# MicroYY/VoxelHashing

Hardware: AMD Instinct MI355X
Metric: depth frames/sec integrate+raycast @640x480, 4 cm voxel; HBM GB/s vs peak (higher is better)
Workload: dtype f32

## Files before the change

### include/vh_api.h

```cpp
#ifndef VH_API_H
#define VH_API_H

#include "vh_types.h"

#ifdef __cplusplus
extern "C" {
#endif

typedef void* vhStream_t;

const char* vh_version(void);
const char* vh_error_string(int code);
const char* vh_last_error_message(void);

int vh_malloc(void** devPtr, size_t bytes);
int vh_free(void* devPtr);
int vh_malloc_host(void** hostPtr, size_t bytes);
int vh_free_host(void* hostPtr);
int vh_memcpy_h2d(void* dst, const void* src, size_t bytes, vhStream_t stream);
int vh_memcpy_d2h(void* dst, const void* src, size_t bytes, vhStream_t stream);
int vh_memset(void* dst, int value, size_t bytes, vhStream_t stream);
int vh_time_next_launch(void* startEvent, void* stopEvent);
int vh_stream_create(vhStream_t* out);
int vh_stream_destroy(vhStream_t stream);
int vh_stream_synchronize(vhStream_t stream);
int vh_device_synchronize(void);

int vh_hash_data_alloc(VhHashData* hd, const VhHashParams* hp);
int vh_hash_data_free(VhHashData* hd);

int vh_reset(const VhHashData* hd, const VhHashParams* hp, vhStream_t stream);
int vh_reset_bucket_mutex(const VhHashData* hd, const VhHashParams* hp, vhStream_t stream);
int vh_alloc(const VhHashData* hd, const VhHashParams* hp, const VhDepthCameraData* cam,
             const VhDepthCameraParams* cp, const uint32_t* d_bitMask, int32_t lockToken, vhStream_t stream);
enum { VH_COMPACT_COUNTER_IS_ZERO = 1 };
int vh_compactify(const VhHashData* hd, const VhHashParams* hp, const VhDepthCameraParams* cp,
                  uint32_t* numOccupied, uint32_t flags, vhStream_t stream);
int vh_integrate(const VhHashData* hd, const VhHashParams* hp, const VhDepthCameraData* cam,
                 const VhDepthCameraParams* cp, vhStream_t stream);
int vh_starve(const VhHashData* hd, const VhHashParams* hp, vhStream_t stream);
int vh_gc_identify(const VhHashData* hd, const VhHashParams* hp, const VhDepthCameraParams* cp, vhStream_t stream);
int vh_gc_free(const VhHashData* hd, const VhHashParams* hp, int32_t lockToken, vhStream_t stream);
int vh_bind_input_depth_color_textures(const VhDepthCameraData* cam);

enum { VH_FUSED_GC = 1, VH_FUSED_STARVE = 2 };
int vh_integrate_fused(const VhHashData* hd, const VhHashParams* hp, const VhDepthCameraData* cam,
                       const VhDepthCameraParams* cp, uint32_t flags, int32_t lockToken, uint32_t* d_countMirror,
                       uint32_t mirrorTag, const void* d_packedFrame, vhStream_t stream);
int vh_alloc_job(VhFrameJob* job, vhStream_t stream);
int vh_compactify_job(VhFrameJob* job, vhStream_t stream);

int vh_render(const VhHashData* hd, const VhHashParams* hp, const VhRayCastData* rd,
              const VhDepthCameraParams* cp, const VhRayCastParams* rp, vhStream_t stream);
int vh_ray_interval_clear(uint32_t* d_tileHeads, uint32_t width, uint32_t height, vhStream_t stream);
int vh_ray_interval_splat(const VhHashData* hd, const VhHashParams* hp, const VhDepthCameraParams* cp, const VhRayCastParams* rp,
                          uint32_t* d_tileHeads, VhTileBlock* d_tileBlocks, uint32_t tileCapacity, uint32_t* d_schedule, uint32_t phase,
                          uint32_t* d_longestList, vhStream_t stream);
size_t vh_render_schedule_bytes(uint32_t width, uint32_t height);
uint32_t vh_render_split_tiles(uint32_t width, uint32_t height);
int vh_render_intervals(const VhHashData* hd, const VhHashParams* hp, const VhRayCastData* rd, const VhDepthCameraParams* cp,
                        const VhRayCastParams* rp, uint32_t* d_tileHeads, const VhTileBlock* d_tileBlocks, uint32_t tileCapacity,
                        uint32_t* d_schedule, uint32_t phase, vhStream_t stream);
int vh_compute_normals(float* d_output4, const float* d_input4, uint32_t width, uint32_t height, vhStream_t stream);
int vh_render_intervals_co(const VhHashData* hd, const VhHashParams* hp, const VhRayCastData* rd, const VhDepthCameraParams* cp,
                           const VhRayCastParams* rp, uint32_t* d_tileHeads, const VhTileBlock* d_tileBlocks, uint32_t tileCapacity,
                           uint32_t* d_schedule, uint32_t phase, VhFrameJob* job, vhStream_t stream);
int vh_compute_normals_co(float* d_output4, const float* d_input4, uint32_t width, uint32_t height, VhFrameJob* job, vhStream_t stream);
int vh_compute_normals_co2(float* d_output4, const float* d_input4, uint32_t width, uint32_t height, VhFrameJob* job,
                           const VhRayCastParams* nextView, uint32_t* d_tileHeads, VhTileBlock* d_tileBlocks, uint32_t tileCapacity,
                           uint32_t* d_schedule, uint32_t phase, uint32_t* d_longestList, vhStream_t stream);

int vh_publish_words(const uint32_t* d_src0, const uint32_t* d_src1, uint32_t* d_mapped, uint32_t tag, vhStream_t stream);

int vh_stream_out_pass1(const VhHashData* hd, const VhHashParams* hp, uint32_t threadsPerPart, uint32_t start,
                        float radius, const float camPos[3], uint32_t* d_outputCounter, VhSDFBlockDesc* d_output,
                        uint32_t outputCapacity, int32_t lockToken, vhStream_t stream);
int vh_stream_out_probe(const VhHashData* hd, const VhHashParams* hp, uint32_t threadsPerPart, uint32_t start, float radius,
                        const float camPos[3], uint32_t* d_counter, uint32_t* d_mapped, uint32_t tag, vhStream_t stream);
int vh_stream_out_pass2(const VhHashData* hd, const VhHashParams* hp, const VhSDFBlockDesc* d_descs,
                        VhVoxel* d_output, uint32_t nSDFBlocks, vhStream_t stream);
int vh_stream_out_device(const VhHashData* hd, const VhHashParams* hp, uint32_t threadsPerPart, uint32_t start, float radius,
                         const float camPos[3], uint32_t* d_outputCounter, VhSDFBlockDesc* d_descs, VhVoxel* d_blocks,
                         uint32_t mostBlocks, int32_t lockToken, uint32_t* d_bitMask, vhStream_t stream);
int vh_publish_count(const uint32_t* d_counter, uint32_t* d_mapped, uint32_t tag, vhStream_t stream);
int vh_stream_in_device(const VhHashData* hd, const VhHashParams* hp, uint32_t n, const VhSDFBlockDesc* d_descs, const VhVoxel* d_blocks,
                        int32_t lockToken, uint32_t* d_failed, uint32_t* d_bitMask, uint32_t chunkBit, uint32_t* d_mapped, uint32_t tag,
                        vhStream_t stream);
int vh_stream_in_pass1(const VhHashData* hd, const VhHashParams* hp, uint32_t n, uint32_t heapCountPrev,
                       const VhSDFBlockDesc* d_descs, int32_t lockToken, vhStream_t stream);
int vh_stream_in_pass1_report(const VhHashData* hd, const VhHashParams* hp, uint32_t n, uint32_t heapCountPrev,
                              const VhSDFBlockDesc* d_descs, int32_t lockToken, uint32_t* d_failed, vhStream_t stream);
int vh_stream_in_pass2(const VhHashData* hd, const VhHashParams* hp, uint32_t n, uint32_t heapCountPrev,
                       const VhSDFBlockDesc* d_descs, const VhVoxel* d_blocks, vhStream_t stream);

int vh_synth_frame(const double* h_spheres, int nSpheres, int inside, const float camToWorld[16],
                   const VhDepthCameraParams* cp, float* d_depth, float* d_color4, vhStream_t stream);
enum { VH_OP_ALLOC = 0, VH_OP_DELETE = 1, VH_OP_INSERT = 2, VH_OP_LOOKUP = 3, VH_OP_NEW_PASS = 4 };
int vh_debug_hash_ops(const VhHashData* hd, const VhHashParams* hp, const int32_t* d_ops, int32_t* d_results,
                      uint32_t n, vhStream_t stream);

int vh_debug_check_fast_math(float divisor, uint32_t modulus, uint32_t n, uint32_t seed, uint32_t* d_mismatches, vhStream_t stream);

int vh_debug_check_refined_division(uint32_t n, uint32_t seed, uint32_t* d_mismatches, vhStream_t stream);
int vh_debug_valu_probe(uint32_t mode, uint32_t wavesPerSimd, uint32_t iters, uint32_t* d_stamps, uint32_t* numWaves, vhStream_t stream);

typedef struct VhSceneRep VhSceneRep;
typedef struct VhRayCast VhRayCast;
typedef struct VhChunkGrid VhChunkGrid;

int vh_scene_rep_create(const VhHashParams* hp, const VhSceneOptions* opt, vhStream_t stream, VhSceneRep** out);
void vh_scene_rep_destroy(VhSceneRep* s);
int vh_scene_rep_integrate(VhSceneRep* s, const float rigidTransform[16], const VhDepthCameraData* cam,
                           const VhDepthCameraParams* cp, const uint32_t* d_bitMask);
int vh_scene_rep_set_last_rigid_transform_and_compactify(VhSceneRep* s, const float rigidTransform[16],
                                                         const VhDepthCameraParams* cp);
int vh_scene_rep_reset(VhSceneRep* s);
int vh_scene_rep_get_hash_data(VhSceneRep* s, VhHashData* out);
int vh_scene_rep_get_hash_params(VhSceneRep* s, VhHashParams* out);
int vh_scene_rep_get_heap_free_count(VhSceneRep* s, uint32_t* out);
int vh_scene_rep_get_num_occupied_blocks(VhSceneRep* s, uint32_t* out);
int vh_scene_rep_debug_hash(VhSceneRep* s, uint32_t report[4]);
int vh_scene_rep_get_state(VhSceneRep* s, uint32_t* out);
int vh_scene_rep_get_timings(VhSceneRep* s, double out[4]);
int vh_scene_rep_set_options(VhSceneRep* s, const VhSceneOptions* opt);

int vh_scene_rep_integrate_ahead(VhSceneRep* s, const float rigidTransform[16], const VhDepthCameraData* cam,
                                 const VhDepthCameraParams* cp, const uint32_t* d_bitMask, VhFrameJob** job);
int vh_scene_rep_integrate_finish(VhSceneRep* s, const VhDepthCameraData* cam, const VhDepthCameraParams* cp);

int vh_raycast_create(const VhRayCastParams* rp, vhStream_t stream, VhRayCast** out);
void vh_raycast_destroy(VhRayCast* r);
int vh_raycast_render(VhRayCast* r, const VhHashData* hd, const VhHashParams* hp,
                      const VhDepthCameraParams* cp, const float lastRigidTransform[16]);
int vh_raycast_render_co(VhRayCast* r, const VhHashData* hd, const VhHashParams* hp,
                         const VhDepthCameraParams* cp, const float lastRigidTransform[16], VhFrameJob* job);
int vh_raycast_get_data(VhRayCast* r, VhRayCastData* out);
int vh_raycast_get_params(VhRayCast* r, VhRayCastParams* out);
int vh_raycast_get_timings(VhRayCast* r, double out[4]);
int vh_raycast_get_event_pair_overhead(VhRayCast* r, double* ms);
int vh_raycast_set_timing(VhRayCast* r, int enabled);
int vh_raycast_set_timing_stride(VhRayCast* r, int enabled, uint32_t stride);
int vh_raycast_set_interval_splatting(VhRayCast* r, int enabled);

int vh_chunk_grid_create(VhSceneRep* s, const float voxelExtents[3], const int32_t gridDimensions[3],
                         const int32_t minGridPos[3], uint32_t initialChunkListSize, int streamingEnabled,
                         uint32_t streamOutParts, VhChunkGrid** out);
void vh_chunk_grid_destroy(VhChunkGrid* g);
int vh_chunk_grid_stream_out_to_cpu_pass0_gpu(VhChunkGrid* g, const float posCamera[3], float radius, int useParts, int multiThreaded);
int vh_chunk_grid_stream_out_to_cpu_pass1_cpu(VhChunkGrid* g, int multiThreaded);
int vh_chunk_grid_stream_in_to_gpu_pass0_cpu(VhChunkGrid* g, const float posCamera[3], float radius, int useParts, int multiThreaded);
int vh_chunk_grid_stream_in_to_gpu_pass1_gpu(VhChunkGrid* g, int multiThreaded);
int vh_chunk_grid_stream_out_to_cpu(VhChunkGrid* g, const float posCamera[3], float radius, int useParts, uint32_t* nStreamedBlocks);
int vh_chunk_grid_stream_in_to_gpu(VhChunkGrid* g, const float posCamera[3], float radius, int useParts, uint32_t* nStreamedBlocks);
int vh_chunk_grid_stream_out_to_cpu_all(VhChunkGrid* g);
int vh_chunk_grid_stream_in_to_gpu_all(VhChunkGrid* g, const float posCamera[3], float radius, int useParts, uint32_t* nStreamedBlocks);
int vh_chunk_grid_get_bit_mask_gpu(VhChunkGrid* g, const uint32_t** d_bitMask);
int vh_chunk_grid_reset(VhChunkGrid* g);
int vh_chunk_grid_debug_check_for_duplicates(VhChunkGrid* g);
int vh_chunk_grid_get_statistics(VhChunkGrid* g, uint32_t out[3]);
int vh_chunk_grid_get_num_failed_inserts(VhChunkGrid* g, uint32_t* out);
int vh_chunk_grid_download_host_blocks(VhChunkGrid* g, VhSDFBlockDesc* descs, VhVoxel* blocks, uint32_t capacity, uint32_t* n);
int vh_chunk_grid_save_to_file(VhChunkGrid* g, const char* filename, const float camPos[3], float radius);
int vh_chunk_grid_load_from_file(VhChunkGrid* g, const char* filename, const float camPos[3], float radius);

typedef struct VhReconstruction VhReconstruction;
void vh_reconstruction_default_options(VhReconstructionOptions* out);
int vh_reconstruction_create(VhSceneRep* scene, VhRayCast* rayCast, VhChunkGrid* chunkGrid ,
                             const VhDepthCameraParams* cp, const VhReconstructionOptions* opt, VhReconstruction** out);
void vh_reconstruction_destroy(VhReconstruction* r);
int vh_reconstruction_run(VhReconstruction* r, const VhSequenceFrame* frames, uint32_t n);
int vh_reconstruction_run_ahead(VhReconstruction* r, const VhSequenceFrame* frames, uint32_t n, const VhSequenceFrame* next);
int vh_reconstruction_synchronize(VhReconstruction* r);
int vh_reconstruction_get_stats(VhReconstruction* r, VhReconstructionStats* out);
int vh_reconstruction_debug_fail_render(VhReconstruction* r, uint32_t nthRenderFromNow);
int vh_reconstruction_reset(VhReconstruction* r);

int vh_convert_color_raw_to_float4(float* d_output4, const uint8_t* d_inputRGBX, uint32_t width, uint32_t height, vhStream_t stream);
int vh_upload_frame(const float* hostDepth, const uint8_t* hostRGBX, float* d_depth, float* d_color4, uint32_t width, uint32_t height, vhStream_t stream);
int vh_resample_float_map(float* d_output, uint32_t outputWidth, uint32_t outputHeight, const float* d_input,
                          uint32_t inputWidth, uint32_t inputHeight, vhStream_t stream);
int vh_resample_float4_map(float* d_output4, uint32_t outputWidth, uint32_t outputHeight, const float* d_input4,
                           uint32_t inputWidth, uint32_t inputHeight, vhStream_t stream);
// ... 157 lines not shown
```

### include/vh_types.h

```cpp
#ifndef VH_TYPES_H
#define VH_TYPES_H

#include <stdint.h>

#ifdef __cplusplus
extern "C" {
#endif

#define VH_SDF_BLOCK_SIZE 8
#define VH_SDF_BLOCK_VOXELS 512
#define VH_HASH_BUCKET_SIZE 10
#define VH_LOCK_ENTRY (-1)
#define VH_FREE_ENTRY (-2)
#define VH_NO_OFFSET 0

typedef struct VhHashEntry {
    int32_t pos[3];
    int32_t ptr;
    uint32_t offset;
    uint32_t _pad[3];
} VhHashEntry;

typedef struct VhVoxel {
    float sdf;
    uint8_t color[3];
    uint8_t weight;
} VhVoxel;

typedef struct VhHashParams {
    float m_rigidTransform[16];
    float m_rigidTransformInverse[16];

    uint32_t m_hashNumBuckets;
    uint32_t m_hashBucketSize;
    uint32_t m_hashMaxCollisionLinkedListSize;
    uint32_t m_numSDFBlocks;

    int32_t m_SDFBlockSize;
    float m_virtualVoxelSize;
    uint32_t m_numOccupiedBlocks;

    float m_maxIntegrationDistance;
    float m_truncScale;
    float m_truncation;
    uint32_t m_integrationWeightSample;
    uint32_t m_integrationWeightMax;

    float m_streamingVoxelExtents[3];
    int32_t m_streamingGridDimensions[3];
    int32_t m_streamingMinGridPos[3];
    uint32_t m_streamingInitialChunkListSize;
    uint32_t m_dummy[2];
} VhHashParams;

typedef struct VhDepthCameraParams {
    float fx, fy, mx, my;
    uint32_t m_imageWidth;
    uint32_t m_imageHeight;
    float m_sensorDepthWorldMin;
    float m_sensorDepthWorldMax;
} VhDepthCameraParams;

typedef struct VhRayCastParams {
    float m_viewMatrix[16];
    float m_viewMatrixInverse[16];
    float m_intrinsics[16];
    float m_intrinsicsInverse[16];

    uint32_t m_width;
    uint32_t m_height;

    uint32_t m_numOccupiedSDFBlocks;
    uint32_t m_maxNumVertices;
    int32_t m_splatMinimum;

    float m_minDepth;
    float m_maxDepth;
    float m_rayIncrement;
    float m_thresSampleDist;
    float m_thresDist;
    uint8_t m_useGradients;
    uint8_t _pad0[3];

    uint32_t dummy0;
} VhRayCastParams;

typedef struct VhHashData {
    uint32_t* d_heap;
    uint32_t* d_heapCounter;
    int32_t* d_hashDecision;
    int32_t* d_hashDecisionPrefix;
    VhHashEntry* d_hash;
    VhHashEntry* d_hashCompactified;
    int32_t* d_hashCompactifiedCounter;
    VhVoxel* d_SDFBlocks;
    int32_t* d_hashBucketMutex;
    uint8_t m_bIsOnGPU;
    uint8_t _pad0[7];
    uint32_t* d_bucketCount;
    uint32_t* d_bucketBits;
    uint32_t* d_state;
} VhHashData;

enum {
    VH_STATE_HEAP_UNDERFLOW = 0,
    VH_STATE_INSERT_FAILED = 1,
    VH_STATE_ALLOC_LOCK_LOST = 2,
    VH_STATE_RIDER_GAVE_UP = 3,
    VH_STATE_WORDS = 16
};

typedef struct VhDepthCameraData {
    const float* d_depthData;
    const float* d_colorData;
} VhDepthCameraData;

typedef struct VhRayCastData {
    float* d_depth;
    float* d_depth4;
    float* d_normals;
    float* d_colors;
} VhRayCastData;

#define VH_TILE_LIST_CAPACITY 64
#define VH_TILE_LIST_CAPACITY_LARGE 128
typedef struct VhTileBlock {
    int32_t pos[3];
    int32_t ptr;
} VhTileBlock;

typedef struct VhSDFBlockDesc {
    int32_t pos[3];
    int32_t ptr;
} VhSDFBlockDesc;

typedef struct VhMarchingCubesParams {
    uint32_t m_boxEnabled;
    float m_minCorner[3];
    uint32_t m_maxNumTriangles;
    float m_maxCorner[3];
    uint32_t m_sdfBlockSize;
    uint32_t m_hashNumBuckets;
    uint32_t m_hashBucketSize;
    float m_threshMarchingCubes;
    float m_threshMarchingCubes2;
    float dummy[3];
} VhMarchingCubesParams;

typedef struct VhVertex {
    float p[3];
    float c[3];
} VhVertex;
typedef struct VhTriangle {
    VhVertex v0, v1, v2;
} VhTriangle;

typedef struct VhMarchingCubesData {
    VhMarchingCubesParams* d_params;
    uint32_t* d_numOccupiedBlocks;
    uint32_t* d_occupiedBlocks;
    uint32_t* d_numTriangles;
    VhTriangle* d_triangles;
    uint8_t m_bIsOnGPU;
} VhMarchingCubesData;

typedef struct VhSceneOptions {
    uint8_t s_offlineProcessing;
    uint8_t s_garbageCollectionEnabled;
    uint8_t s_timingsDetailledEnabled;
    uint8_t s_useReferenceLaunchSequence;
    uint32_t s_garbageCollectionStarve;
    uint32_t s_streamingOutParts;
} VhSceneOptions;

typedef struct VhFrameJob {
    VhHashData hashData;
    VhHashParams hashParams;
    VhDepthCameraData cam;
    VhDepthCameraParams cp;
    const uint32_t* d_bitMask;
    void* d_packedFrame;
    int32_t lockToken;
    uint8_t allocLaunched, compactifyLaunched, pad0[2];
    uint32_t frameNumber;
    uint32_t tableEpoch;
// ... 191 lines not shown
```

### voxelhashing_amd/csrc/vh_device.hpp

```cpp
#pragma once

#include <hip/hip_runtime.h>
#include <stdint.h>

#include "../../include/vh_types.h"

namespace vhd {

struct F3 { float x, y, z; };
struct I3 { int x, y, z; };

#define VHD __device__ __forceinline__

VHD float minf() { return __int_as_float((int)0xff800000u); }
VHD float pinf() { return __int_as_float((int)0x7f800000u); }

VHD F3 mk3(float x, float y, float z) { F3 r; r.x = x; r.y = y; r.z = z; return r; }
VHD I3 mki3(int x, int y, int z) { I3 r; r.x = x; r.y = y; r.z = z; return r; }
VHD float dot3(F3 a, F3 b) { return a.x * b.x + a.y * b.y + a.z * b.z; }

VHD int f2i(float v) { return __float2int_rz(v); }
VHD uint8_t f2uc(float v) { return (uint8_t)__float2int_rz(fminf(fmaxf(v, 0.0f), 255.0f)); }

VHD int signi(float v) { return (0.0f < v) - (v < 0.0f); }
// ... 82 lines not shown
{
    const uint32_t q0 = __umulhi(k.m, n);
    const uint32_t t = ((n - q0) >> 1) + q0;
    const uint32_t q = t >> k.sh;
    return n - q * k.d;
}
VHD uint32_t hash_pos_fast(HashMod k, I3 p)
{
    const uint32_t p0 = 73856093u, p1 = 19349669u, p2 = 83492791u;
    return umod_fast(((uint32_t)p.x * p0) ^ ((uint32_t)p.y * p1) ^ ((uint32_t)p.z * p2), k);
}


VHD F3 depth_to_skeleton(const VhDepthCameraParams& cp, uint32_t ux, uint32_t uy, float depth)
{
    const float x = ((float)ux - cp.mx) / cp.fx;
    const float y = ((float)uy - cp.my) / cp.fy;
    return mk3(depth * x, depth * y, depth);
}
VHD float cam_to_proj_z(const VhDepthCameraParams& cp, float z)
{
    return (z - cp.m_sensorDepthWorldMin) / (cp.m_sensorDepthWorldMax - cp.m_sensorDepthWorldMin);
}
VHD float proj_to_cam_z(const VhDepthCameraParams& cp, float z)
{
    return z * (cp.m_sensorDepthWorldMax - cp.m_sensorDepthWorldMin) + cp.m_sensorDepthWorldMin;
}
VHD bool in_frustum_approx(const VhDepthCameraParams& cp, const float* viewMatrixInverse, F3 pos)
{
    F3 pc = mat_mul_p(viewMatrixInverse, pos);
    float px = pc.x * cp.fx / pc.z + cp.mx;
    float py = pc.y * cp.fy / pc.z + cp.my;
    float wm1 = (float)cp.m_imageWidth - 1.0f, hm1 = (float)cp.m_imageHeight - 1.0f;
    float x = (2.0f * px - wm1) / wm1;
    float y = (hm1 - 2.0f * py) / hm1;
    float z = cam_to_proj_z(cp, pc.z);
    const float s = 0.95f;
    x *= s; y *= s; z *= s;
    return !(x < -1.0f || x > 1.0f || y < -1.0f || y > 1.0f || z < 0.0f || z > 1.0f);
}
VHD bool block_in_frustum(const VhHashParams& hp, const VhDepthCameraParams& cp, I3 blk)
{
    F3 pw = block_to_world(hp.m_virtualVoxelSize, blk);
    float off = hp.m_virtualVoxelSize * 0.5f * ((float)VH_SDF_BLOCK_SIZE - 1.0f);
    pw.x += off; pw.y += off; pw.z += off;
    return in_frustum_approx(cp, hp.m_rigidTransformInverse, pw);
}


VHD int4 load_quad(const VhHashEntry* e) { return *reinterpret_cast<const int4*>(e); }
VHD void store_quad(VhHashEntry* e, int4 q) { *reinterpret_cast<int4*>(e) = q; }
VHD bool quad_matches(int4 q, I3 p) { return q.x == p.x && q.y == p.y && q.z == p.z && q.w != VH_FREE_ENTRY; }

VHD void delete_hash_entry(VhHashEntry* e)
{
    e->offset = 0;
    store_quad(e, make_int4(0, 0, 0, VH_FREE_ENTRY));
}
VHD void copy_entry(VhHashEntry* dst, const VhHashEntry* src)
{
    int4 q = load_quad(src);
    uint32_t o = src->offset;
    dst->offset = o;
    store_quad(dst, q);
}

VHD void bucket_inc(const VhHashData& hd, uint32_t slotIdx)
{
    uint32_t b = slotIdx / VH_HASH_BUCKET_SIZE;
    uint32_t old = atomicAdd(&hd.d_bucketCount[b], 1u);
    if (old == 0u) atomicOr(&hd.d_bucketBits[b >> 5], 1u << (b & 31));
}
VHD void bucket_dec(const VhHashData& hd, uint32_t slotIdx)
{
    uint32_t b = slotIdx / VH_HASH_BUCKET_SIZE;
    uint32_t old = atomicSub(&hd.d_bucketCount[b], 1u);
    if (old == 1u) atomicAnd(&hd.d_bucketBits[b >> 5], ~(1u << (b & 31)));
}
VHD bool bucket_maybe_occupied(const VhHashData& hd, uint32_t h)
{
    return (hd.d_bucketBits[h >> 5] >> (h & 31)) & 1u;
}

VHD uint32_t consume_heap(const VhHashData& hd, uint32_t numSDFBlocks, bool& ok)
{
    uint32_t addr = atomicSub(&hd.d_heapCounter[0], 1u);
    if (addr >= numSDFBlocks) {
        atomicAdd(&hd.d_heapCounter[0], 1u);
        atomicAdd(&hd.d_state[VH_STATE_HEAP_UNDERFLOW], 1u);
        ok = false;
        return 0;
    }
    ok = true;
    return hd.d_heap[addr];
}
VHD void append_heap(const VhHashData& hd, uint32_t blockId)
{
    uint32_t addr = atomicAdd(&hd.d_heapCounter[0], 1u);
    hd.d_heap[addr + 1] = blockId;
}

VHD int lookup_ptr(const VhHashData& hd, const VhHashParams& hp, I3 blk)
{
    const uint32_t ne = hp.m_hashNumBuckets * VH_HASH_BUCKET_SIZE;
    const uint32_t h = hash_pos(hp.m_hashNumBuckets, blk);
    if (!bucket_maybe_occupied(hd, h)) return VH_FREE_ENTRY;
    const uint32_t base = h * VH_HASH_BUCKET_SIZE;
#pragma unroll 1
    for (uint32_t j = 0; j < VH_HASH_BUCKET_SIZE; j++) {
        int4 q = load_quad(&hd.d_hash[base + j]);
        if (quad_matches(q, blk)) return q.w;
    }
    const uint32_t idxLast = base + VH_HASH_BUCKET_SIZE - 1;
    uint32_t i = idxLast;
    uint32_t maxIter = 0;
#pragma unroll 1
    while (maxIter < hp.m_hashMaxCollisionLinkedListSize) {
        int4 q = load_quad(&hd.d_hash[i]);
        if (quad_matches(q, blk)) return q.w;
        if (q.w == VH_FREE_ENTRY && i != idxLast) {
            __builtin_amdgcn_fence(__ATOMIC_ACQUIRE, "agent");
            q = load_quad(&hd.d_hash[i]);
            if (quad_matches(q, blk)) return q.w;
        }
        uint32_t off = hd.d_hash[i].offset;
        if (off == 0) break;
        i = (idxLast + off) % ne;
        maxIter++;
    }
    return VH_FREE_ENTRY;
}

VHD int alloc_block(const VhHashData& hd, const VhHashParams& hp, I3 pos, int32_t lockToken)
{
    const uint32_t ne = hp.m_hashNumBuckets * VH_HASH_BUCKET_SIZE;
    uint32_t h = hash_pos(hp.m_hashNumBuckets, pos);
    const uint32_t base = h * VH_HASH_BUCKET_SIZE;

    int firstEmpty = -1;
    const uint32_t idxLast = base + VH_HASH_BUCKET_SIZE - 1;
    const uint32_t maxLoop = hp.m_hashMaxCollisionLinkedListSize;
    uint32_t i = idxLast;
    uint32_t maxIter = 0;
    if (!bucket_maybe_occupied(hd, h)) {
        firstEmpty = (int)base;
    } else {
        int4 qs[VH_HASH_BUCKET_SIZE];
#pragma unroll
        for (uint32_t j = 0; j < VH_HASH_BUCKET_SIZE; j++) qs[j] = load_quad(&hd.d_hash[base + j]);
        uint32_t off = hd.d_hash[idxLast].offset;
#pragma unroll
        for (uint32_t j = 0; j < VH_HASH_BUCKET_SIZE; j++) {
            if (quad_matches(qs[j], pos)) return 0;
            if (firstEmpty == -1 && qs[j].w == VH_FREE_ENTRY) firstEmpty = (int)(base + j);
        }
#pragma unroll 1
        while (maxIter < maxLoop) {
            if (off == 0) break;
            i = (idxLast + off) % ne;
            maxIter++;
            if (!(maxIter < maxLoop)) break;
            int4 q = load_quad(&hd.d_hash[i]);
            if (quad_matches(q, pos)) return 0;
            off = hd.d_hash[i].offset;
        }
    }

    if (firstEmpty != -1) {
        int prev = atomicExch(&hd.d_hashBucketMutex[h], lockToken);
        if (prev != lockToken) {
            bool ok;
            uint32_t blk = consume_heap(hd, hp.m_numSDFBlocks, ok);
            if (!ok) return 3;
            VhHashEntry* e = &hd.d_hash[firstEmpty];
            e->offset = VH_NO_OFFSET;
            store_quad(e, make_int4(pos.x, pos.y, pos.z, (int)(blk * VH_SDF_BLOCK_VOXELS)));
            bucket_inc(hd, (uint32_t)firstEmpty);
            return 1;
        }
        atomicAdd(&hd.d_state[VH_STATE_ALLOC_LOCK_LOST], 1u);
        return 2;
    }

    int offset = 0;
    maxIter = 0;
#pragma unroll 1
    while (maxIter < maxLoop) {
        offset++;
        i = (idxLast + (uint32_t)offset) % ne;
        if ((offset % VH_HASH_BUCKET_SIZE) == 0) continue;
        int4 q = load_quad(&hd.d_hash[i]);
        if (q.w == VH_FREE_ENTRY) {
            int prev = atomicExch(&hd.d_hashBucketMutex[h], lockToken);
            if (prev != lockToken) {
                uint32_t lastOffset = hd.d_hash[idxLast].offset;
                uint32_t h2 = i / VH_HASH_BUCKET_SIZE;
                prev = atomicExch(&hd.d_hashBucketMutex[h2], lockToken);
                if (prev != lockToken) {
                    bool ok;
                    uint32_t blk = consume_heap(hd, hp.m_numSDFBlocks, ok);
                    if (!ok) return 3;
                    VhHashEntry* e = &hd.d_hash[i];
                    e->offset = lastOffset;
                    store_quad(e, make_int4(pos.x, pos.y, pos.z, (int)(blk * VH_SDF_BLOCK_VOXELS)));
                    __threadfence();
                    hd.d_hash[idxLast].offset = (uint32_t)offset;
                    bucket_inc(hd, i);
                    return 1;
                }
            }
            atomicAdd(&hd.d_state[VH_STATE_ALLOC_LOCK_LOST], 1u);
            return 2;
        }
        maxIter++;
    }
    return 3;
}

VHD bool insert_hash_entry(const VhHashData& hd, const VhHashParams& hp, I3 pos, int ptr, int32_t lockToken)
{
    const uint32_t ne = hp.m_hashNumBuckets * VH_HASH_BUCKET_SIZE;
    const uint32_t h = hash_pos(hp.m_hashNumBuckets, pos);
    const uint32_t base = h * VH_HASH_BUCKET_SIZE;
#pragma unroll 1
    for (uint32_t j = 0; j < VH_HASH_BUCKET_SIZE; j++) {
        VhHashEntry* e = &hd.d_hash[base + j];
        int prev = atomicCAS(&e->ptr, VH_FREE_ENTRY, VH_LOCK_ENTRY);
        if (prev == VH_FREE_ENTRY) {
            e->offset = 0;
            store_quad(e, make_int4(pos.x, pos.y, pos.z, ptr));
            bucket_inc(hd, base + j);
            return true;
        }
    }
    const uint32_t idxLast = base + VH_HASH_BUCKET_SIZE - 1;
    int prevLock = atomicExch(&hd.d_hashBucketMutex[h], lockToken);
    if (prevLock == lockToken) return false;
    uint32_t maxIter = 0;
    int offset = 0;
#pragma unroll 1
    while (maxIter < hp.m_hashMaxCollisionLinkedListSize) {
        offset++;
        uint32_t i = (idxLast + (uint32_t)offset) % ne;
        if ((offset % VH_HASH_BUCKET_SIZE) == 0) continue;
        VhHashEntry* e = &hd.d_hash[i];
        int prev = atomicCAS(&e->ptr, VH_FREE_ENTRY, VH_LOCK_ENTRY);
        if (prev == VH_FREE_ENTRY) {
            e->offset = hd.d_hash[idxLast].offset;
            store_quad(e, make_int4(pos.x, pos.y, pos.z, ptr));
            hd.d_hash[idxLast].offset = (uint32_t)offset;
            bucket_inc(hd, i);
            return true;
        }
        maxIter++;
    }
    return false;
}

VHD bool delete_hash_entry_element(const VhHashData& hd, const VhHashParams& hp, I3 blk, int32_t lockToken)
{
    const uint32_t ne = hp.m_hashNumBuckets * VH_HASH_BUCKET_SIZE;
    const uint32_t h = hash_pos(hp.m_hashNumBuckets, blk);
    const uint32_t base = h * VH_HASH_BUCKET_SIZE;

#pragma unroll 1
    for (uint32_t j = 0; j < VH_HASH_BUCKET_SIZE; j++) {
        const uint32_t i = base + j;
        int4 q = load_quad(&hd.d_hash[i]);
        if (quad_matches(q, blk)) {
            uint32_t off = hd.d_hash[i].offset;
            if (off != 0) {
                int prev = atomicExch(&hd.d_hashBucketMutex[h], lockToken);
                if (prev == lockToken) return false;
                append_heap(hd, (uint32_t)q.w / VH_SDF_BLOCK_VOXELS);
                uint32_t nextIdx = (i + off) % ne;
                copy_entry(&hd.d_hash[i], &hd.d_hash[nextIdx]);
                delete_hash_entry(&hd.d_hash[nextIdx]);
                bucket_dec(hd, nextIdx);
                return true;
            } else {
                append_heap(hd, (uint32_t)q.w / VH_SDF_BLOCK_VOXELS);
                delete_hash_entry(&hd.d_hash[i]);
                bucket_dec(hd, i);
                return true;
            }
        }
    }
    const uint32_t idxLast = base + VH_HASH_BUCKET_SIZE - 1;
    uint32_t prevIdx = idxLast;
    uint32_t i = (idxLast + hd.d_hash[idxLast].offset) % ne;
    uint32_t maxIter = 0;
#pragma unroll 1
    while (maxIter < hp.m_hashMaxCollisionLinkedListSize) {
        int4 q = load_quad(&hd.d_hash[i]);
        uint32_t off = hd.d_hash[i].offset;
        if (quad_matches(q, blk)) {
            int prev = atomicExch(&hd.d_hashBucketMutex[h], lockToken);
            if (prev == lockToken) return false;
            append_heap(hd, (uint32_t)q.w / VH_SDF_BLOCK_VOXELS);
            delete_hash_entry(&hd.d_hash[i]);
            bucket_dec(hd, i);
            hd.d_hash[prevIdx].offset = off;
            return true;
        }
        if (off == 0) return false;
        prevIdx = i;
        i = (idxLast + off) % ne;
        maxIter++;
    }
    return false;
}

VHD bool delete_hash_entry_element_wave(const VhHashData& hd, const VhHashParams& hp, I3 blk, int32_t lockToken, uint32_t lane)
{
    const uint32_t h = hash_pos(hp.m_hashNumBuckets, blk);
    const uint32_t i = h * VH_HASH_BUCKET_SIZE + lane;
    int4 q = make_int4(0, 0, 0, VH_FREE_ENTRY);
    uint32_t off = 0u;
    if (lane < VH_HASH_BUCKET_SIZE) { q = load_quad(&hd.d_hash[i]); off = hd.d_hash[i].offset; }
    const bool match = lane < VH_HASH_BUCKET_SIZE && quad_matches(q, blk);
    const unsigned long long m = __ballot(match);
    bool ok = false;
    if (m == 0ull || __ballot(match && off != 0u) != 0ull) {
        if (lane == 0u) ok = delete_hash_entry_element(hd, hp, blk, lockToken);
    } else if (match) {
        const uint32_t addr = atomicAdd(&hd.d_heapCounter[0], 1u);
        const uint32_t old = atomicSub(&hd.d_bucketCount[h], 1u);
        hd.d_heap[addr + 1] = (uint32_t)q.w / VH_SDF_BLOCK_VOXELS;
        delete_hash_entry(&hd.d_hash[i]);
        if (old == 1u) atomicAnd(&hd.d_bucketBits[h >> 5], ~(1u << (h & 31)));
        ok = true;
    }
    return __ballot(ok) != 0ull;
}


struct Vox {
    float sdf;
    uint32_t cw;
    VHD uint32_t weight() const { return cw >> 24; }
    VHD uint32_t r() const { return cw & 0xffu; }
    VHD uint32_t g() const { return (cw >> 8) & 0xffu; }
    VHD uint32_t b() const { return (cw >> 16) & 0xffu; }
};
VHD Vox unpack_vox(uint2 w) { Vox v; v.sdf = __uint_as_float(w.x); v.cw = w.y; return v; }
VHD uint2 pack_vox(Vox v) { return make_uint2(__float_as_uint(v.sdf), v.cw); }
VHD uint32_t pack_cw(uint32_t r, uint32_t g, uint32_t b, uint32_t w) { return r | (g << 8) | (b << 16) | (w << 24); }

VHD Vox combine_voxel(const VhHashParams& hp, Vox v0, Vox v1)
{
    Vox out;
    const uint32_t a = v0.cw & 0x00ffffffu, c = v1.cw & 0x00ffffffu;
    const uint32_t rgb = (a | c) - (((a ^ c) >> 1) & 0x7f7f7f7fu);
    float w0 = (float)v0.weight(), w1 = (float)v1.weight();
    out.sdf = (v0.sdf * w0 + v1.sdf * w1) / (w0 + w1);
    uint32_t w = min(hp.m_integrationWeightMax, v0.weight() + v1.weight());
    out.cw = rgb | ((w & 0xffu) << 24);
    return out;
}

}
```

### voxelhashing_amd/csrc/vh_host.cpp

```cpp
#include <hip/hip_runtime.h>

#include <array>
#include <climits>
#include <cstring>
#include <string>
#include <unordered_set>
#include <vector>

#include "../../include/vh.hpp"
#include "vh_host_util.hpp"
#include "vh_stage_timer.hpp"

namespace {

inline void check(int code, const char* what)
{
    if (code != 0) throw vh::Error(code, std::string(what) + ": " + vh_error_string(code));
}
inline void checkHip(hipError_t e, const char* what)
{
    if (e != hipSuccess) throw vh::Error(-(int)e, std::string(what) + ": " + hipGetErrorString(e));
}

}
// ... 50 lines not shown
}
int vh_free_host(void* hostPtr)
{
    if (!hostPtr) return VH_ERR_BAD_ARGUMENT;
    VH_HIP(hipHostFree(hostPtr));
    return VH_OK;
}
int vh_memcpy_h2d(void* dst, const void* src, size_t bytes, vhStream_t stream)
{
    if (!dst || !src) return VH_ERR_BAD_ARGUMENT;
    VH_HIP(hipMemcpyAsync(dst, src, bytes, hipMemcpyHostToDevice, (hipStream_t)stream));
    VH_HIP(hipStreamSynchronize((hipStream_t)stream));
    return VH_OK;
}
int vh_memcpy_d2h(void* dst, const void* src, size_t bytes, vhStream_t stream)
{
    if (!dst || !src) return VH_ERR_BAD_ARGUMENT;
    VH_HIP(hipMemcpyAsync(dst, src, bytes, hipMemcpyDeviceToHost, (hipStream_t)stream));
    VH_HIP(hipStreamSynchronize((hipStream_t)stream));
    return VH_OK;
}
int vh_memset(void* dst, int value, size_t bytes, vhStream_t stream)
{
    if (!dst) return VH_ERR_BAD_ARGUMENT;
    VH_HIP(hipMemsetAsync(dst, value, bytes, (hipStream_t)stream));
    return VH_OK;
}
int vh_time_next_launch(void* startEvent, void* stopEvent)
{
    if (!startEvent || !stopEvent) return VH_ERR_BAD_ARGUMENT;
    t_launchStart = (hipEvent_t)startEvent;
    t_launchStop = (hipEvent_t)stopEvent;
    return VH_OK;
}
int vh_stream_create(vhStream_t* out)
{
    if (!out) return VH_ERR_BAD_ARGUMENT;
    hipStream_t s = nullptr;
    VH_HIP(hipStreamCreateWithFlags(&s, hipStreamNonBlocking));
    *out = (vhStream_t)s;
    return VH_OK;
}
int vh_stream_destroy(vhStream_t stream)
{
    if (!stream) return VH_ERR_BAD_ARGUMENT;
    VH_HIP(hipStreamDestroy((hipStream_t)stream));
    return VH_OK;
}
int vh_stream_synchronize(vhStream_t stream)
{
    VH_HIP(hipStreamSynchronize((hipStream_t)stream));
    return VH_OK;
}
int vh_device_synchronize(void)
{
    VH_HIP(hipDeviceSynchronize());
    return VH_OK;
}

int vh_hash_data_alloc(VhHashData* hd, const VhHashParams* hp)
{
    if (!hd || !hp || hp->m_hashNumBuckets == 0 || hp->m_numSDFBlocks == 0) return VH_ERR_BAD_ARGUMENT;
    if (hp->m_hashBucketSize != VH_HASH_BUCKET_SIZE || hp->m_SDFBlockSize != VH_SDF_BLOCK_SIZE) return VH_ERR_BAD_ARGUMENT;
    if ((uint64_t)hp->m_numSDFBlocks * VH_SDF_BLOCK_VOXELS > (uint64_t)INT_MAX) return VH_ERR_BAD_ARGUMENT;
    if ((uint64_t)hp->m_hashNumBuckets * VH_HASH_BUCKET_SIZE > (uint64_t)UINT_MAX / 2) return VH_ERR_BAD_ARGUMENT;
    std::memset(hd, 0, sizeof(*hd));
    const size_t nb = hp->m_hashNumBuckets, ne = nb * VH_HASH_BUCKET_SIZE, nblk = hp->m_numSDFBlocks;
    int err = 0;
#define VH_ALLOC(field, bytes)                                              \
    if (!err) {                                                             \
        hipError_t e_ = hipMalloc((void**)&hd->field, (bytes));             \
        if (e_ != hipSuccess) { hd->field = nullptr; err = -(int)e_; }      \
    }
    VH_ALLOC(d_heap, sizeof(uint32_t) * nblk)
    VH_ALLOC(d_heapCounter, sizeof(uint32_t))
    VH_ALLOC(d_hash, sizeof(VhHashEntry) * ne)
    VH_ALLOC(d_hashDecision, sizeof(int32_t) * ne)
    VH_ALLOC(d_hashDecisionPrefix, sizeof(int32_t) * ne)
    VH_ALLOC(d_hashCompactified, sizeof(VhHashEntry) * ne)
    VH_ALLOC(d_hashCompactifiedCounter, sizeof(int32_t))
    VH_ALLOC(d_SDFBlocks, sizeof(VhVoxel) * nblk * VH_SDF_BLOCK_VOXELS)
    VH_ALLOC(d_hashBucketMutex, sizeof(int32_t) * nb)
    VH_ALLOC(d_bucketCount, sizeof(uint32_t) * nb)
    VH_ALLOC(d_bucketBits, sizeof(uint32_t) * ((nb + 31) / 32))
    VH_ALLOC(d_state, sizeof(uint32_t) * VH_STATE_WORDS)
#undef VH_ALLOC
    if (err) {
        vh_hash_data_free(hd);
        return err;
    }
    hd->m_bIsOnGPU = 1;
    return VH_OK;
}

int vh_hash_data_free(VhHashData* hd)
{
    if (!hd) return VH_ERR_BAD_ARGUMENT;
    void* ptrs[] = { hd->d_heap, hd->d_heapCounter, hd->d_hash, hd->d_hashDecision, hd->d_hashDecisionPrefix,
                     hd->d_hashCompactified, hd->d_hashCompactifiedCounter, hd->d_SDFBlocks, hd->d_hashBucketMutex,
                     hd->d_bucketCount, hd->d_bucketBits, hd->d_state };
    for (void* p : ptrs)
        if (p) (void)hipFree(p);
    std::memset(hd, 0, sizeof(*hd));
    return VH_OK;
}

}


namespace vh {

mat4f mat4f::identity()
{
    mat4f r;
    for (int i = 0; i < 16; i++) r.m[i] = (i % 5 == 0) ? 1.0f : 0.0f;
    return r;
}

mat4f mat4f::getInverse() const
{
    static const signed char T[16][6][4] = {
        { {+1,5,10,15}, {-1,5,11,14}, {-1,9,6,15}, {+1,9,7,14}, {+1,13,6,11}, {-1,13,7,10} },
        { {-1,1,10,15}, {+1,1,11,14}, {+1,9,2,15}, {-1,9,3,14}, {-1,13,2,11}, {+1,13,3,10} },
        { {+1,1,6,15}, {-1,1,7,14}, {-1,5,2,15}, {+1,5,3,14}, {+1,13,2,7}, {-1,13,3,6} },
        { {-1,1,6,11}, {+1,1,7,10}, {+1,5,2,11}, {-1,5,3,10}, {-1,9,2,7}, {+1,9,3,6} },
        { {-1,4,10,15}, {+1,4,11,14}, {+1,8,6,15}, {-1,8,7,14}, {-1,12,6,11}, {+1,12,7,10} },
        { {+1,0,10,15}, {-1,0,11,14}, {-1,8,2,15}, {+1,8,3,14}, {+1,12,2,11}, {-1,12,3,10} },
        { {-1,0,6,15}, {+1,0,7,14}, {+1,4,2,15}, {-1,4,3,14}, {-1,12,2,7}, {+1,12,3,6} },
        { {+1,0,6,11}, {-1,0,7,10}, {-1,4,2,11}, {+1,4,3,10}, {+1,8,2,7}, {-1,8,3,6} },
        { {+1,4,9,15}, {-1,4,11,13}, {-1,8,5,15}, {+1,8,7,13}, {+1,12,5,11}, {-1,12,7,9} },
        { {-1,0,9,15}, {+1,0,11,13}, {+1,8,1,15}, {-1,8,3,13}, {-1,12,1,11}, {+1,12,3,9} },
        { {+1,0,5,15}, {-1,0,7,13}, {-1,4,1,15}, {+1,4,3,13}, {+1,12,1,7}, {-1,12,3,5} },
        { {-1,0,5,11}, {+1,0,7,9}, {+1,4,1,11}, {-1,4,3,9}, {-1,8,1,7}, {+1,8,3,5} },
        { {-1,4,9,14}, {+1,4,10,13}, {+1,8,5,14}, {-1,8,6,13}, {-1,12,5,10}, {+1,12,6,9} },
        { {+1,0,9,14}, {-1,0,10,13}, {-1,8,1,14}, {+1,8,2,13}, {+1,12,1,10}, {-1,12,2,9} },
        { {-1,0,5,14}, {+1,0,6,13}, {+1,4,1,14}, {-1,4,2,13}, {-1,12,1,6}, {+1,12,2,5} },
        { {+1,0,5,10}, {-1,0,6,9}, {-1,4,1,10}, {+1,4,2,9}, {+1,8,1,6}, {-1,8,2,5} },
    };
    float inv[16];
    for (int n = 0; n < 16; n++) {
        float acc = 0.0f;
        for (int t = 0; t < 6; t++) {
            const float p = m[T[n][t][1]] * m[T[n][t][2]] * m[T[n][t][3]];
            if (t == 0) acc = (T[n][t][0] > 0) ? p : -p;
            else acc = (T[n][t][0] > 0) ? acc + p : acc - p;
        }
        inv[n] = acc;
    }
    const float det = m[0] * inv[0] + m[1] * inv[4] + m[2] * inv[8] + m[3] * inv[12];
    const float detr = 1.0f / det;
    mat4f r;
    for (int n = 0; n < 16; n++) r.m[n] = inv[n] * detr;
    return r;
}

mat4f mat4f::operator*(const mat4f& o) const
{
    mat4f r;
    for (int i = 0; i < 4; i++)
        for (int j = 0; j < 4; j++)
            r.m[4 * i + j] = m[4 * i + 0] * o.m[j] + m[4 * i + 1] * o.m[4 + j] + m[4 * i + 2] * o.m[8 + j] + m[4 * i + 3] * o.m[12 + j];
    return r;
}

vec3f mat4f::transformPoint(const vec3f& v) const
{
    vec3f r;
// ... 564 lines not shown
```

### voxelhashing_amd/csrc/vh_kernels.hip

```cpp
#include <hip/hip_runtime.h>

#include <cstring>

#include "../../include/vh_api.h"
#include "vh_device.hpp"
#include "vh_host_util.hpp"

using namespace vhd;

namespace {

constexpr int kWave = 64;

VHD uint32_t lane_id() { return threadIdx.x & (kWave - 1); }
VHD uint64_t lanemask_lt() { return (1ull << lane_id()) - 1ull; }


__global__ __launch_bounds__(256) void k_reset_heap(uint32_t* heap, uint32_t* heapCounter, uint32_t n)
{
    const uint32_t idx = blockIdx.x * blockDim.x + threadIdx.x;
    if (idx == 0) heapCounter[0] = n - 1;
    if (idx < n) heap[idx] = n - idx - 1;
}

__global__ __launch_bounds__(256) void k_reset_hash(VhHashEntry* a, VhHashEntry* b, uint32_t ne)
{
    const uint64_t idx = (uint64_t)blockIdx.x * blockDim.x + threadIdx.x;
    if (idx < 2ull * ne) {
        const int4 v = (idx & 1) ? make_int4(0, 0, 0, 0) : make_int4(0, 0, 0, VH_FREE_ENTRY);
        reinterpret_cast<int4*>(a)[idx] = v;
        reinterpret_cast<int4*>(b)[idx] = v;
    }
}

__global__ __launch_bounds__(256) void k_fill_i32(int32_t* p, int32_t v, uint32_t n)
{
    const uint32_t idx = blockIdx.x * blockDim.x + threadIdx.x;
    if (idx < n) p[idx] = v;
}


VHD bool block_streamed_out(const VhHashParams& hp, I3 blk, const uint32_t* bitMask)
{
    if (!bitMask) return false;
    F3 pw = block_to_world(hp.m_virtualVoxelSize, blk);
    F3 p = mk3(pw.x / hp.m_streamingVoxelExtents[0], pw.y / hp.m_streamingVoxelExtents[1], pw.z / hp.m_streamingVoxelExtents[2]);
    I3 c = mki3(f2i(p.x + (float)signi(p.x) * 0.5f), f2i(p.y + (float)signi(p.y) * 0.5f), f2i(p.z + (float)signi(p.z) * 0.5f));
    I3 q = mki3(c.x - hp.m_streamingMinGridPos[0], c.y - hp.m_streamingMinGridPos[1], c.z - hp.m_streamingMinGridPos[2]);
    uint32_t index = (uint32_t)(q.z * hp.m_streamingGridDimensions[0] * hp.m_streamingGridDimensions[1] +
                                q.y * hp.m_streamingGridDimensions[0] + q.x);
    return (bitMask[index >> 5] & (1u << (index & 31))) != 0u;
}

VHD uint2 pack_pixel(const VhHashParams& hp, const VhDepthCameraParams& cp, float depth, bool hasColor, float4 c)
{
    uint32_t cw = 0u;
    if (hasColor && c.x != minf() && depth != minf() && depth < hp.m_maxIntegrationDistance) {
        const float depthZeroOne = cam_to_proj_z(cp, depth);
        const float weightUpdate = fmaxf((float)hp.m_integrationWeightSample * 1.5f * (1.0f - depthZeroOne), 1.0f);
        cw = pack_cw(f2uc(255.0f * c.x), f2uc(255.0f * c.y), f2uc(255.0f * c.z), f2uc(weightUpdate));
    }
    return make_uint2(__float_as_uint(depth), cw);
}

VHD void alloc_tile(const VhHashData& hd, const VhHashParams& hp, const VhDepthCameraData& cam, const VhDepthCameraParams& cp,
                    const uint32_t* bitMask, int32_t lockToken, HashMod hm, uint2* packed, uint32_t tile)
{
    const uint32_t lane = lane_id();
    const uint32_t W = cp.m_imageWidth, H = cp.m_imageHeight;
    const uint32_t tilesX = (W + 7) / 8, tilesY = (H + 7) / 8;
    if (tile >= tilesX * tilesY) return;
    const uint32_t x = (tile % tilesX) * 8 + (lane & 7), y = (tile / tilesX) * 8 + (lane >> 3);
    const float vs = hp.m_virtualVoxelSize;

    bool active = (x < W) && (y < H);
    float d = active ? cam.d_depthData[y * W + x] : minf();
    if (packed && active) {
        float4 c = make_float4(minf(), minf(), minf(), minf());
        if (cam.d_colorData) c = reinterpret_cast<const float4*>(cam.d_colorData)[y * W + x];
        packed[y * W + x] = pack_pixel(hp, cp, d, cam.d_colorData != nullptr, c);
    }
    if (d == minf() || d == 0.0f) active = false;
    if (d >= hp.m_maxIntegrationDistance) active = false;
    const float t = get_truncation(hp, d);
    const float minDepth = fminf(hp.m_maxIntegrationDistance, d - t);
    const float maxDepth = fminf(hp.m_maxIntegrationDistance, d + t);
    if (minDepth >= maxDepth) active = false;
    if (!__any(active)) return;

    const F3 rayMin = mat_mul_p(hp.m_rigidTransform, depth_to_skeleton(cp, x, y, minDepth));
    const F3 rayMax = mat_mul_p(hp.m_rigidTransform, depth_to_skeleton(cp, x, y, maxDepth));
    const F3 rayDir = normalize3(mk3(rayMax.x - rayMin.x, rayMax.y - rayMin.y, rayMax.z - rayMin.z));

    const float rvs = 1.0f / vs;
    I3 id = vvp_to_block(mki3(world_to_vvp1_rb(rayMin.x, vs, rvs), world_to_vvp1_rb(rayMin.y, vs, rvs), world_to_vvp1_rb(rayMin.z, vs, rvs)));
    const I3 idEnd = vvp_to_block(mki3(world_to_vvp1_rb(rayMax.x, vs, rvs), world_to_vvp1_rb(rayMax.y, vs, rvs), world_to_vvp1_rb(rayMax.z, vs, rvs)));

    const F3 step = mk3((float)signi(rayDir.x), (float)signi(rayDir.y), (float)signi(rayDir.z));
    const I3 cl = mki3(f2i(fmaxf(0.0f, fminf(step.x, 1.0f))), f2i(fmaxf(0.0f, fminf(step.y, 1.0f))), f2i(fmaxf(0.0f, fminf(step.z, 1.0f))));
    F3 boundaryPos = block_to_world(vs, mki3(id.x + cl.x, id.y + cl.y, id.z + cl.z));
    const float half = 0.5f * vs;
    boundaryPos.x -= half; boundaryPos.y -= half; boundaryPos.z -= half;
    F3 tMax = mk3((boundaryPos.x - rayMin.x) / rayDir.x, (boundaryPos.y - rayMin.y) / rayDir.y, (boundaryPos.z - rayMin.z) / rayDir.z);
    F3 tDelta = mk3((step.x * (float)VH_SDF_BLOCK_SIZE * vs) / rayDir.x, (step.y * (float)VH_SDF_BLOCK_SIZE * vs) / rayDir.y,
                    (step.z * (float)VH_SDF_BLOCK_SIZE * vs) / rayDir.z);
    const I3 idBound = mki3(f2i((float)idEnd.x + step.x), f2i((float)idEnd.y + step.y), f2i((float)idEnd.z + step.z));

    if (rayDir.x == 0.0f) { tMax.x = pinf(); tDelta.x = pinf(); }
    if (boundaryPos.x - rayMin.x == 0.0f) { tMax.x = pinf(); tDelta.x = pinf(); }
    if (rayDir.y == 0.0f) { tMax.y = pinf(); tDelta.y = pinf(); }
    if (boundaryPos.y - rayMin.y == 0.0f) { tMax.y = pinf(); tDelta.y = pinf(); }
    if (rayDir.z == 0.0f) { tMax.z = pinf(); tDelta.z = pinf(); }
    if (boundaryPos.z - rayMin.z == 0.0f) { tMax.z = pinf(); tDelta.z = pinf(); }

    uint32_t iter = 0;
    while (__any(active)) {
        bool want = active;
        if (want) {
            const int4 q0 = load_quad(&hd.d_hash[hash_pos_fast(hm, id) * VH_HASH_BUCKET_SIZE]);
            want = !quad_matches(q0, id);
        }
        if (want) want = block_in_frustum(hp, cp, id) && !block_streamed_out(hp, id, bitMask);
        uint64_t pending = __ballot(want);
        bool leads = false;
        while (pending) {
            const int leader = __ffsll((unsigned long long)pending) - 1;
            const int bx = __builtin_amdgcn_readlane(id.x, leader);
            const int by = __builtin_amdgcn_readlane(id.y, leader);
            const int bz = __builtin_amdgcn_readlane(id.z, leader);
            const bool same = want && id.x == bx && id.y == by && id.z == bz;
            pending &= ~__ballot(same);
            leads = leads || (int)lane == leader;
        }
        if (leads) alloc_block(hd, hp, id, lockToken);
        if (active) {
            if (tMax.x < tMax.y && tMax.x < tMax.z) {
                id.x = f2i((float)id.x + step.x);
                if (id.x == idBound.x) active = false;
                tMax.x += tDelta.x;
            } else if (tMax.z < tMax.y) {
                id.z = f2i((float)id.z + step.z);
                if (id.z == idBound.z) active = false;
                tMax.z += tDelta.z;
            } else {
                id.y = f2i((float)id.y + step.y);
                if (id.y == idBound.y) active = false;
                tMax.y += tDelta.y;
            }
            iter++;
            if (iter >= 1024u) active = false;
        }
    }
}

__global__ __launch_bounds__(512) void k_alloc(VhHashData hd, VhHashParams hp, VhDepthCameraData cam,
                                               VhDepthCameraParams cp, const uint32_t* bitMask, int32_t lockToken, HashMod hm, uint2* packed)
{
    if (blockIdx.x == 0 && threadIdx.x == 0) hd.d_hashCompactifiedCounter[0] = 0;
    alloc_tile(hd, hp, cam, cp, bitMask, lockToken, hm, packed, blockIdx.x * (blockDim.x / kWave) + (threadIdx.x / kWave));
}


VHD int cvt_rz(float v)
{
    int r;
    asm("v_cvt_i32_f32 %0, %1" : "=v"(r) : "v"(v));
    return r;
}

constexpr uint32_t kIntegrateTile = 32;
constexpr uint32_t kIntegrateTileRows = 29;
constexpr uint32_t kIntegrateTileStride = 34;


constexpr uint32_t VH_BOX_STAGED = 1u, VH_BOX_CERTIFIED = 2u;
struct BlockBox {
    uint32_t x0, y0, w, h, flags;
};
VHD uint32_t frame_tag(const VhHashParams& hp, const VhDepthCameraParams& cp)
{
    uint32_t t = 0x9E3779B9u;
#pragma unroll
    for (int i = 0; i < 12; i++) t = (t ^ __float_as_uint(hp.m_rigidTransformInverse[i])) * 0x01000193u + (t >> 15);
    const uint32_t more[7] = { __float_as_uint(hp.m_virtualVoxelSize), __float_as_uint(cp.fx), __float_as_uint(cp.fy), __float_as_uint(cp.mx),
                               __float_as_uint(cp.my), cp.m_imageWidth, cp.m_imageHeight };
#pragma unroll
    for (int i = 0; i < 7; i++) t = (t ^ more[i]) * 0x01000193u + (t >> 15);
    return (t & 0x7fffffffu) | 1u;
}
VHD uint32_t rider_tag(uint32_t frameNumber) { return 0x80000000u | frameNumber; }
struct BoxCorners {
    int bx0, bx1, by0, by1;
    float cz;
    bool fine;
};
VHD BoxCorners box_no_corner()
{
    BoxCorners a;
    a.bx0 = 0x7fffffff; a.bx1 = (int)0x80000000; a.by0 = 0x7fffffff; a.by1 = (int)0x80000000;
    a.cz = pinf();
    a.fine = true;
    return a;
}
VHD void box_add_corner(const VhHashParams& hp, const VhDepthCameraParams& cp, int ex, int ey, int ez, uint32_t c, BoxCorners& a)
{
    const I3 pc = mki3(ex * VH_SDF_BLOCK_SIZE + ((c & 1u) ? 7 : 0), ey * VH_SDF_BLOCK_SIZE + ((c & 2u) ? 7 : 0), ez * VH_SDF_BLOCK_SIZE + ((c & 4u) ? 7 : 0));
    const F3 pf = mat_mul_p(hp.m_rigidTransformInverse, vvp_to_world(hp.m_virtualVoxelSize, pc));
    const float rz = __builtin_amdgcn_rcpf(pf.z);
    const int cx = cvt_rz((pf.x * cp.fx * rz + cp.mx) + 0.5f), cy = cvt_rz((pf.y * cp.fy * rz + cp.my) + 0.5f);
    a.bx0 = min(a.bx0, cx); a.bx1 = max(a.bx1, cx);
    a.by0 = min(a.by0, cy); a.by1 = max(a.by1, cy);
    a.cz = fminf(a.cz, pf.z);
    a.fine = a.fine && pf.z >= 0x1p-20f && pf.z <= 0x1p20f && fabsf(pf.x * cp.fx) <= 0x1p60f && fabsf(pf.y * cp.fy) <= 0x1p60f;
}
VHD BlockBox box_of_corners(const VhDepthCameraParams& cp, const BoxCorners& a)
{
    const bool inFront = a.cz > 1e-3f;
    const bool sane = a.bx0 > -(1 << 30) && a.bx1 < (1 << 30) && a.by0 > -(1 << 30) && a.by1 < (1 << 30);
    const int x0i = max(a.bx0 - 1, 0) & ~1, x1i = min(a.bx1 + 1, (int)cp.m_imageWidth - 1);
    const int y0i = max(a.by0 - 1, 0), y1i = min(a.by1 + 1, (int)cp.m_imageHeight - 1);
    const bool staged = inFront && sane && x0i <= x1i && y0i <= y1i && (x1i - x0i) < (int)kIntegrateTile && (y1i - y0i) < (int)kIntegrateTileRows &&
                        (cp.m_imageWidth & 1u) == 0u && cp.m_imageWidth <= 0xffffu && cp.m_imageHeight <= 0xffffu;
    BlockBox b;
    b.x0 = staged ? (uint32_t)x0i : 0u;
    b.y0 = staged ? (uint32_t)y0i : 0u;
    b.w = staged ? (uint32_t)(x1i - x0i + 1) : 0u;
    b.h = staged ? (uint32_t)(y1i - y0i + 1) : 0u;
    b.flags = (staged ? VH_BOX_STAGED : 0u) | (a.fine ? VH_BOX_CERTIFIED : 0u);
    return b;
}
VHD BlockBox block_box(const VhHashParams& hp, const VhDepthCameraParams& cp, int ex, int ey, int ez)
{
    BoxCorners a = box_no_corner();
#pragma unroll
    for (uint32_t c = 0; c < 8u; c++) box_add_corner(hp, cp, ex, ey, ez, c, a);
    return box_of_corners(cp, a);
}
VHD BlockBox block_box_by_eight_lanes(const VhHashParams& hp, const VhDepthCameraParams& cp, int ex, int ey, int ez)
{
    BoxCorners a = box_no_corner();
    box_add_corner(hp, cp, ex, ey, ez, lane_id() & 7u, a);
    int fine = a.fine ? 1 : 0;
#pragma unroll
    for (int o = 1; o < 8; o <<= 1) {
        a.bx0 = min(a.bx0, __shfl_xor(a.bx0, o)); a.bx1 = max(a.bx1, __shfl_xor(a.bx1, o));
        a.by0 = min(a.by0, __shfl_xor(a.by0, o)); a.by1 = max(a.by1, __shfl_xor(a.by1, o));
        a.cz = fminf(a.cz, __shfl_xor(a.cz, o));
        fine &= __shfl_xor(fine, o);
    }
    a.fine = fine != 0;
    return box_of_corners(cp, a);
}
VHD uint4 pack_box(uint32_t offset, const BlockBox& b, uint32_t tag) { return make_uint4(offset, b.x0 | (b.y0 << 16), b.w | (b.h << 8) | (b.flags << 16), tag); }

constexpr uint32_t kCompactQueue = 768;
struct CompactShared {
    int4 q[kCompactQueue];
    uint32_t off[kCompactQueue];
    uint32_t n, base, nBuckets;
    uint16_t buckets[256 * 32];
};
template <bool COHERENT> VHD void list_store(VhHashEntry* o, const int4 q, const uint4 box)
{
    if (COHERENT) {
        uint64_t* const w = reinterpret_cast<uint64_t*>(o);
        __hip_atomic_store(w + 0, (uint64_t)(uint32_t)q.x | ((uint64_t)(uint32_t)q.y << 32), __ATOMIC_RELAXED, __HIP_MEMORY_SCOPE_AGENT);
        __hip_atomic_store(w + 1, (uint64_t)(uint32_t)q.z | ((uint64_t)(uint32_t)q.w << 32), __ATOMIC_RELAXED, __HIP_MEMORY_SCOPE_AGENT);
        __hip_atomic_store(w + 2, (uint64_t)box.x | ((uint64_t)box.y << 32), __ATOMIC_RELAXED, __HIP_MEMORY_SCOPE_AGENT);
        __builtin_amdgcn_fence(__ATOMIC_RELEASE, "workgroup");
        __hip_atomic_store(w + 3, (uint64_t)box.z | ((uint64_t)box.w << 32), __ATOMIC_RELAXED, __HIP_MEMORY_SCOPE_AGENT);
    } else {
        *(reinterpret_cast<uint4*>(o) + 1) = box;
        store_quad(o, q);
    }
}
template <bool COHERENT> VHD int4 list_quad(const VhHashEntry* e)
{
    if (COHERENT) {
        const uint64_t* const w = reinterpret_cast<const uint64_t*>(e);
        const uint64_t a = __hip_atomic_load(w + 0, __ATOMIC_RELAXED, __HIP_MEMORY_SCOPE_AGENT), b = __hip_atomic_load(w + 1, __ATOMIC_RELAXED, __HIP_MEMORY_SCOPE_AGENT);
        return make_int4((int)(uint32_t)a, (int)(uint32_t)(a >> 32), (int)(uint32_t)b, (int)(uint32_t)(b >> 32));
    }
    return load_quad(e);
}
template <bool COHERENT> VHD uint4 list_box(const VhHashEntry* e)
{
    if (COHERENT) {
        const uint64_t* const w = reinterpret_cast<const uint64_t*>(e);
        const uint64_t a = __hip_atomic_load(w + 2, __ATOMIC_RELAXED, __HIP_MEMORY_SCOPE_AGENT), b = __hip_atomic_load(w + 3, __ATOMIC_RELAXED, __HIP_MEMORY_SCOPE_AGENT);
        return make_uint4((uint32_t)a, (uint32_t)(a >> 32), (uint32_t)b, (uint32_t)(b >> 32));
    }
    return *(reinterpret_cast<const uint4*>(e) + 1);
}

template <bool COHERENT = false>
__device__ void compactify_group(const VhHashData& hd, const VhHashParams& hp, const VhDepthCameraParams& cp, uint32_t wordIdx, CompactShared& sh, const uint32_t riderTag = 0u)
{
    const uint32_t nWords = (hp.m_hashNumBuckets + 31) / 32;
    const uint32_t tag = COHERENT ? riderTag : frame_tag(hp, cp);
    const uint32_t lane = lane_id();
#if defined(VH_KNOCKOUT) && VH_KNOCKOUT == 42
    uint32_t phase[6];
    phase[0] = (uint32_t)__builtin_amdgcn_s_memrealtime();
#define VH_COMPACT_PHASE(I) phase[I] = (uint32_t)__builtin_amdgcn_s_memrealtime();
#define VH_COMPACT_PHASES_OUT { __syncthreads(); if (threadIdx.x == 0) { uint4* const at = reinterpret_cast<uint4*>(hd.d_hashCompactified) + (hp.m_hashNumBuckets * VH_HASH_BUCKET_SIZE) / 2u + 8192u + 2u * (wordIdx / 256u); \
        at[0] = make_uint4(phase[0], phase[1], phase[2], 0x5743u); at[1] = make_uint4(phase[3], phase[4], (uint32_t)__builtin_amdgcn_s_memrealtime(), sh.n | (sh.nBuckets << 16)); } }
#else
#define VH_COMPACT_PHASE(I)
#define VH_COMPACT_PHASES_OUT
#endif
    if (threadIdx.x == 0) { sh.n = 0u; sh.nBuckets = 0u; }
    __syncthreads();
    uint32_t bits = (wordIdx < nWords) ? hd.d_bucketBits[wordIdx] : 0u;
    {
        const uint32_t mine = (uint32_t)__popc(bits);
        uint32_t incl = mine;
#pragma unroll
        for (uint32_t d = 1; d < kWave; d <<= 1) {
            const uint32_t t = (uint32_t)__shfl_up((int)incl, d);
            if (lane >= d) incl += t;
        }
        const uint32_t total = (uint32_t)__shfl((int)incl, kWave - 1);
        uint32_t at = 0;
        if (lane == 0 && total != 0u) at = atomicAdd(&sh.nBuckets, total);
        at = (uint32_t)__shfl((int)at, 0) + incl - mine;
        while (bits != 0u) {
            sh.buckets[at++] = (uint16_t)(threadIdx.x * 32u + (uint32_t)(__ffs((int)bits) - 1));
            bits &= bits - 1u;
        }
    }
    __syncthreads();
    VH_COMPACT_PHASE(1)
    const uint32_t nSlots = sh.nBuckets * VH_HASH_BUCKET_SIZE;
    const uint64_t firstBucket = (uint64_t)(wordIdx - threadIdx.x) * 32u;
    constexpr uint32_t kInFlight = 4;
    for (uint32_t s0 = threadIdx.x; s0 < nSlots; s0 += 256u * kInFlight) {
        int4 qs[kInFlight];
        uint32_t offs[kInFlight];
#pragma unroll
        for (uint32_t j = 0; j < kInFlight; j++) {
            const uint32_t slot = s0 + 256u * j;
            qs[j] = make_int4(0, 0, 0, VH_FREE_ENTRY);
            offs[j] = 0;
            if (slot < nSlots) {
                const VhHashEntry* e = &hd.d_hash[(firstBucket + sh.buckets[slot / VH_HASH_BUCKET_SIZE]) * VH_HASH_BUCKET_SIZE + slot % VH_HASH_BUCKET_SIZE];
                qs[j] = load_quad(e);
                offs[j] = e->offset;
            }
        }
#pragma unroll
        for (uint32_t j = 0; j < kInFlight; j++) {
            const int4 q = qs[j];
            const bool keep = q.w != VH_FREE_ENTRY && block_in_frustum(hp, cp, mki3(q.x, q.y, q.z));
            const uint64_t kept = __ballot(keep);
            if (kept == 0ull) continue;
            uint32_t at = 0;
            if (lane == 0) at = atomicAdd(&sh.n, (uint32_t)__popcll(kept));
            at = (uint32_t)__shfl((int)at, 0) + (uint32_t)__popcll(kept & lanemask_lt());
            if (keep) {
                if (at < kCompactQueue) {
                    sh.q[at] = q;
                    sh.off[at] = offs[j];
                } else {
                    VhHashEntry* o = &hd.d_hashCompactified[(uint32_t)atomicAdd(hd.d_hashCompactifiedCounter, 1)];
                    list_store<COHERENT>(o, q, pack_box(offs[j], block_box(hp, cp, q.x, q.y, q.z), tag));
                }
            }
        }
    }
    __syncthreads();
    VH_COMPACT_PHASE(2)
    const uint32_t n = min(sh.n, kCompactQueue);
    if (n == 0u) return;
    uint32_t place = 0;
    if (threadIdx.x == 0) place = (uint32_t)atomicAdd(hd.d_hashCompactifiedCounter, (int)n);
    if (COHERENT) {
        if (threadIdx.x == 0) sh.base = place;
        __syncthreads();
        VH_COMPACT_PHASE(3)
        const uint32_t base = sh.base;
        for (uint32_t i = threadIdx.x; i < n; i += blockDim.x) list_store<true>(&hd.d_hashCompactified[base + i], sh.q[i], make_uint4(sh.off[i], 0u, 0u, tag));
        VH_COMPACT_PHASE(4)
        VH_COMPACT_PHASES_OUT
        return;
    }
    constexpr uint32_t kBoxRounds = 2;
    uint4 boxes[kBoxRounds];
    const uint32_t mine = threadIdx.x >> 3;
#pragma unroll
    for (uint32_t r = 0; r < kBoxRounds; r++) {
        const uint32_t i = min(r * 32u + mine, n - 1u);
        if (r * 32u < n) {
            const int4 q = sh.q[i];
            boxes[r] = pack_box(sh.off[i], block_box_by_eight_lanes(hp, cp, q.x, q.y, q.z), tag);
        }
    }
    if (threadIdx.x == 0) sh.base = place;
    __syncthreads();
    VH_COMPACT_PHASE(3)
    const uint32_t base = sh.base;
#pragma unroll
    for (uint32_t r = 0; r < kBoxRounds; r++) {
        const uint32_t i = r * 32u + mine;
        if (i < n && (threadIdx.x & 7u) == 0u) list_store<COHERENT>(&hd.d_hashCompactified[base + i], sh.q[i], boxes[r]);
    }
    for (uint32_t r = kBoxRounds; r * 32u < n; r++) {
        const uint32_t i = r * 32u + mine;
        const int4 q = sh.q[min(i, n - 1u)];
        const BlockBox b = block_box_by_eight_lanes(hp, cp, q.x, q.y, q.z);
        if (i < n && (threadIdx.x & 7u) == 0u) list_store<COHERENT>(&hd.d_hashCompactified[base + i], q, pack_box(sh.off[i], b, tag));
    }
    VH_COMPACT_PHASE(4)
    VH_COMPACT_PHASES_OUT
}

__global__ __launch_bounds__(256) void k_compactify(VhHashData hd, VhHashParams hp, VhDepthCameraParams cp)
{
    __shared__ CompactShared sh;
    compactify_group(hd, hp, cp, blockIdx.x * blockDim.x + threadIdx.x, sh);
}


VHD Vox integrate_voxel(const VhHashParams& hp, const VhDepthCameraParams& cp, const VhDepthCameraData& cam, I3 pi, Vox stored)
{
    F3 pf = mat_mul_p(hp.m_rigidTransformInverse, vvp_to_world(hp.m_virtualVoxelSize, pi));
    const uint32_t sx = (uint32_t)f2i((pf.x * cp.fx / pf.z + cp.mx) + 0.5f);
    const uint32_t sy = (uint32_t)f2i((pf.y * cp.fy / pf.z + cp.my) + 0.5f);
    if (sx < cp.m_imageWidth && sy < cp.m_imageHeight) {
        const uint32_t pix = sy * cp.m_imageWidth + sx;
        const float depth = cam.d_depthData[pix];
        float cr = minf(), cg = minf(), cb = minf();
        if (cam.d_colorData) {
            const float4 c = reinterpret_cast<const float4*>(cam.d_colorData)[pix];
            cr = c.x; cg = c.y; cb = c.z;
        }
        if (cr != minf() && depth != minf()) {
            if (depth < hp.m_maxIntegrationDistance) {
                const float depthZeroOne = cam_to_proj_z(cp, depth);
                float sdf = depth - pf.z;
                const float truncation = get_truncation(hp, depth);
                if (sdf > -truncation) {
                    if (sdf >= 0.0f) sdf = fminf(truncation, sdf);
                    else sdf = fmaxf(-truncation, sdf);
                    const float weightUpdate = fmaxf((float)hp.m_integrationWeightSample * 1.5f * (1.0f - depthZeroOne), 1.0f);
                    Vox curr;
                    curr.sdf = sdf;
                    if (cam.d_colorData) curr.cw = pack_cw(f2uc(255.0f * cr), f2uc(255.0f * cg), f2uc(255.0f * cb), f2uc(weightUpdate));
                    else curr.cw = pack_cw(0, 255, 0, f2uc(weightUpdate));
                    return combine_voxel(hp, stored, curr);
                }
            }
        }
    }
    return stored;
}

VHD Vox starve_voxel(Vox v)
{
    uint32_t w = v.weight();
    w = (w > 0u) ? w - 1u : 0u;
    v.cw = (v.cw & 0x00ffffffu) | (w << 24);
    return v;
}

VHD void block_min_max(float& minSdf, uint32_t& maxW, float* sMin, uint32_t* sMax)
{
#pragma unroll
    for (int o = 32; o > 0; o >>= 1) {
        minSdf = fminf(minSdf, __shfl_xor(minSdf, o));
        maxW = max(maxW, (uint32_t)__shfl_xor((int)maxW, o));
    }
    const uint32_t wave = threadIdx.x / kWave;
    if (lane_id() == 0) { sMin[wave] = minSdf; sMax[wave] = maxW; }
    __syncthreads();
    float m = sMin[0];
    uint32_t w = sMax[0];
    for (uint32_t i = 1; i < blockDim.x / kWave; i++) { m = fminf(m, sMin[i]); w = max(w, sMax[i]); }
    minSdf = m; maxW = w;
}

VHD float gc_key(Vox v) { return (v.weight() == 0u) ? pinf() : fabsf(v.sdf); }

template <bool FUSED>
__global__ __launch_bounds__(256) void k_integrate(VhHashData hd, VhHashParams hp, VhDepthCameraData cam,
                                                   VhDepthCameraParams cp, uint32_t flags, int32_t lockToken, uint32_t* countMirror)
{
    __shared__ float sMin[4];
    __shared__ uint32_t sMax[4];
    __shared__ int sFreed;

    const uint32_t count = FUSED ? (uint32_t)hd.d_hashCompactifiedCounter[0] : hp.m_numOccupiedBlocks;
    if (FUSED && countMirror && blockIdx.x == 0 && threadIdx.x == 0) *countMirror = count;
    const uint32_t t = threadIdx.x;
    const int lx = (int)((2u * t) & 7u), ly = (int)(((2u * t) & 63u) >> 3), lz = (int)((2u * t) >> 6);

    for (uint32_t b = blockIdx.x; b < count; b += gridDim.x) {
        const int4 q = load_quad(&hd.d_hashCompactified[b]);
        const int ex = __builtin_amdgcn_readfirstlane(q.x), ey = __builtin_amdgcn_readfirstlane(q.y);
        const int ez = __builtin_amdgcn_readfirstlane(q.z), ptr = __builtin_amdgcn_readfirstlane(q.w);

        uint4* vp = reinterpret_cast<uint4*>(&hd.d_SDFBlocks[(uint32_t)ptr]) + t;
        const uint4 raw = *vp;
// ... 439 lines not shown
            const bool decide = (minSdf >= thr) || (maxW == 0u);
            if (lane == 0) hd.d_hashDecision[b] = decide ? 1 : 0;
            if (__builtin_amdgcn_readfirstlane(decide ? 1 : 0) != 0) freed = free_block_cold<KERNARG_OFFSET>(ex, ey, ez, lane);
        }
        if (freed) {
#pragma unroll
            for (int j = 0; j < 4; j++) vp[j * kWave] = make_uint4(0u, 0u, 0u, 0u);
        } else if (!wrote) {
#pragma unroll
            for (int j = 0; j < 4; j++) vp[j * kWave] = raw[j];
        }
        if (!hasNext) break;
        b = bNext;
    }
#if defined(VH_KNOCKOUT) && VH_KNOCKOUT == 9
    if (wFirst == 0u && lane == 0u) {
        const uint64_t c = __builtin_amdgcn_s_memtime() - stampC0, r = __builtin_amdgcn_s_memrealtime() - stampR0;
        hd.d_state[8] = (uint32_t)c; hd.d_state[9] = (uint32_t)r; hd.d_state[10] = (count + nActive - 1u) / nActive; hd.d_state[11] = nActive;
    }
    if (lane == 0u) {
        const uint32_t hwid = __builtin_amdgcn_s_getreg((31 << 11) | 4), xcc = __builtin_amdgcn_s_getreg((31 << 11) | 20);
        reinterpret_cast<uint4*>(hd.d_hashCompactified)[nEntries / 2u + 3u * wFirst] =
            make_uint4((uint32_t)stampR0, (uint32_t)__builtin_amdgcn_s_memrealtime(), hwid, xcc);
        reinterpret_cast<uint4*>(hd.d_hashCompactified)[nEntries / 2u + 3u * wFirst + 1u] = make_uint4(stamps[0], stamps[1], stamps[2], stamps[3]);
        reinterpret_cast<uint4*>(hd.d_hashCompactified)[nEntries / 2u + 3u * wFirst + 2u] = make_uint4(stamps[4], stamps[5], 0u, 0u);
    }
#endif
}

template <bool PACKED>
__global__ __launch_bounds__(256)
void k_integrate_fused(FusedArgs args)
{
    __shared__ FusedShared<PACKED> sh;
    integrate_fused_body<PACKED, 0u>(args, blockIdx.x, gridDim.x, sh);
}

__global__ __launch_bounds__(256) void k_starve(VhHashData hd, VhHashParams hp)
{
    const uint32_t b = blockIdx.x;
    if (b >= hp.m_numOccupiedBlocks) return;
    const int ptr = __builtin_amdgcn_readfirstlane(load_quad(&hd.d_hashCompactified[b]).w);
    uint4* vp = reinterpret_cast<uint4*>(&hd.d_SDFBlocks[(uint32_t)ptr]) + threadIdx.x;
    uint4 raw = *vp;
    Vox v0 = starve_voxel(unpack_vox(make_uint2(raw.x, raw.y))), v1 = starve_voxel(unpack_vox(make_uint2(raw.z, raw.w)));
    raw.y = v0.cw; raw.w = v1.cw;
    *vp = raw;
}

__global__ __launch_bounds__(256) void k_gc_identify(VhHashData hd, VhHashParams hp, VhDepthCameraParams cp)
{
    __shared__ float sMin[4];
    __shared__ uint32_t sMax[4];
    const uint32_t b = blockIdx.x;
    if (b >= hp.m_numOccupiedBlocks) return;
    const int ptr = __builtin_amdgcn_readfirstlane(load_quad(&hd.d_hashCompactified[b]).w);
    const uint4 raw = *(reinterpret_cast<const uint4*>(&hd.d_SDFBlocks[(uint32_t)ptr]) + threadIdx.x);
    const Vox v0 = unpack_vox(make_uint2(raw.x, raw.y)), v1 = unpack_vox(make_uint2(raw.z, raw.w));
    float minSdf = fminf(gc_key(v0), gc_key(v1));
    uint32_t maxW = max(v0.weight(), v1.weight());
    block_min_max(minSdf, maxW, sMin, sMax);
    if (threadIdx.x == 0) {
        const float thr = get_truncation(hp, cp.m_sensorDepthWorldMax);
        hd.d_hashDecision[b] = ((minSdf >= thr) || (maxW == 0u)) ? 1 : 0;
    }
}

__global__ __launch_bounds__(256) void k_gc_free(VhHashData hd, VhHashParams hp, int32_t lockToken)
{
    __shared__ int sFreed;
    const uint32_t b = blockIdx.x;
    if (b >= hp.m_numOccupiedBlocks) return;
    if (hd.d_hashDecision[b] == 0) return;
    const int4 q = load_quad(&hd.d_hashCompactified[b]);
    if (threadIdx.x == 0) sFreed = delete_hash_entry_element(hd, hp, mki3(q.x, q.y, q.z), lockToken) ? 1 : 0;
    __syncthreads();
    if (sFreed) {
        const int ptr = __builtin_amdgcn_readfirstlane(q.w);
        *(reinterpret_cast<uint4*>(&hd.d_SDFBlocks[(uint32_t)ptr]) + threadIdx.x) = make_uint4(0u, 0u, 0u, 0u);
    }
}


constexpr uint32_t kSplatWordsPerGroup = 32;
constexpr uint32_t kSplatQueue = 128;

VHD void divmod_small(uint32_t i, uint32_t nx, float rnx, uint32_t& q, uint32_t& r)
{
    q = (uint32_t)((float)i * rnx);
    int rem = (int)i - (int)(q * nx);
    if (rem < 0) { q--; rem += (int)nx; }
    if (rem >= (int)nx) { q++; rem -= (int)nx; }
    r = (uint32_t)rem;
}

constexpr uint32_t kCostSample = 6;
constexpr uint32_t kCostClasses = 32;
constexpr uint32_t kCostClassWidth = 8;
#ifndef VH_SPLIT_TILES
#define VH_SPLIT_TILES 256
#endif
constexpr uint32_t kSplitTiles = VH_SPLIT_TILES;
constexpr uint32_t kSplitMinTiles = 1024;
__host__ __device__ inline uint32_t split_tiles(uint32_t nTiles)
{
#ifndef VH_SPLIT_DIV
#define VH_SPLIT_DIV 16
#endif
    const uint32_t n = (nTiles / VH_SPLIT_DIV) & ~1u;
    return nTiles >= kSplitMinTiles ? (n < kSplitTiles ? n : kSplitTiles) : 0u;
}

constexpr uint32_t kSchedGroups = 8;
__host__ __device__ inline uint32_t sched_groups(uint32_t nTiles) { return nTiles >= kSplitMinTiles ? kSchedGroups : 1u; }

__device__ void schedule_tiles(uint32_t* sched, uint32_t* feedback, uint32_t nTiles, uint32_t phase, uint32_t numCUs, uint32_t part, uint32_t parts,
                               uint32_t* sCount )
{
    const uint32_t* cls = sched + 4;
    uint2* slots = reinterpret_cast<uint2*>(sched + 4 + 4u * ((nTiles + 3u) / 4u));
    const uint32_t nSplit = split_tiles(nTiles);
    if (threadIdx.x == 0 && part == 0u) {
        sched[0] = phase;
        if (feedback) *feedback = sched[1];
        sched[1] = 0u;
    }
    constexpr uint32_t kSub = 8, kBins = kCostClasses * kSub;
    static_assert(kBins == 4u * kWave, "the scan below gives four bins to each lane of one wave");
    for (uint32_t i = threadIdx.x; i < 2u * kBins; i += blockDim.x) sCount[i] = 0u;
    __syncthreads();
    const uint32_t sub = threadIdx.x % kSub;
    constexpr uint32_t kBatch = 5;
    const uint32_t nQuads = (nTiles + 3u) / 4u;
    const uint4* cls4 = reinterpret_cast<const uint4*>(cls);
    const uint32_t myQuads = part < nQuads ? (nQuads - part + parts - 1u) / parts : 0u;
    uint32_t nShare[kSchedGroups];
#pragma unroll
    for (uint32_t w = 0; w < kSchedGroups; w++) {
        const uint32_t nq = (w < parts && w < nQuads) ? (nQuads - w + parts - 1u) / parts : 0u;
        nShare[w] = 4u * nq - ((nq != 0u && (nQuads - 1u) % parts == w) ? 4u * nQuads - nTiles : 0u);
    }
    for (uint32_t q0 = threadIdx.x; q0 < myQuads; q0 += blockDim.x * kBatch) {
        uint4 c[kBatch];
#pragma unroll
        for (uint32_t j = 0; j < kBatch; j++) {
            const uint32_t q = q0 + j * blockDim.x;
            c[j] = q < myQuads ? cls4[q * parts + part] : make_uint4(0u, 0u, 0u, 0u);
        }
#pragma unroll
        for (uint32_t j = 0; j < kBatch; j++) {
            const uint32_t t = ((q0 + j * blockDim.x) * parts + part) * 4u;
            if (t + 0u < nTiles) atomicAdd(&sCount[min(c[j].x, kCostClasses - 1u) * kSub + sub], 1u);
            if (t + 1u < nTiles) atomicAdd(&sCount[min(c[j].y, kCostClasses - 1u) * kSub + sub], 1u);
            if (t + 2u < nTiles) atomicAdd(&sCount[min(c[j].z, kCostClasses - 1u) * kSub + sub], 1u);
            if (t + 3u < nTiles) atomicAdd(&sCount[min(c[j].w, kCostClasses - 1u) * kSub + sub], 1u);
        }
    }
    __syncthreads();
    if (threadIdx.x < kWave) {
        const uint32_t lane = threadIdx.x;
        uint32_t n[4], mine = 0u;
#pragma unroll
        for (uint32_t j = 0; j < 4u; j++) { n[j] = sCount[kBins - 1u - (lane * 4u + j)]; mine += n[j]; }
        uint32_t incl = mine;
#pragma unroll
        for (int off = 1; off < (int)kWave; off <<= 1) {
            const uint32_t up = (uint32_t)__shfl_up((int)incl, off);
            if ((int)lane >= off) incl += up;
        }
        uint32_t start = incl - mine;
#pragma unroll
        for (uint32_t j = 0; j < 4u; j++) { sCount[kBins + kBins - 1u - (lane * 4u + j)] = start; start += n[j]; }
    }
    __syncthreads();
    const uint32_t nGroups = (nTiles + nSplit + 3u) / 4u, fullRows = nGroups / numCUs;
    for (uint32_t q0 = threadIdx.x; q0 < myQuads; q0 += blockDim.x * kBatch) {
        uint4 c[kBatch];
#pragma unroll
        for (uint32_t j = 0; j < kBatch; j++) {
            const uint32_t q = q0 + j * blockDim.x;
            c[j] = q < myQuads ? cls4[q * parts + part] : make_uint4(0u, 0u, 0u, 0u);
        }
#pragma unroll
        for (uint32_t j = 0; j < kBatch; j++) {
            const uint32_t cc[4] = { c[j].x, c[j].y, c[j].z, c[j].w };
#pragma unroll
            for (uint32_t k = 0; k < 4u; k++) {
                const uint32_t t = ((q0 + j * blockDim.x) * parts + part) * 4u + k;
                if (t < nTiles) {
                    const uint32_t mine = atomicAdd(&sCount[kBins + min(cc[k], kCostClasses - 1u) * kSub + sub], 1u);
                    uint32_t i = 0u;
#pragma unroll
                    for (uint32_t w = 0; w < kSchedGroups; w++) i += min(mine, nShare[w]) + ((w < part && nShare[w] > mine) ? 1u : 0u);
                    if (i < nSplit) {
                        const uint32_t at = (i / 2u) * 4u + (i & 1u) * 2u;
                        slots[at] = make_uint2(t | (1u << 24), phase);
                        slots[at + 1u] = make_uint2(t | (2u << 24), phase);
                    } else {
                        const uint32_t j = i + nSplit;
                        uint32_t g = j / 4u;
                        const uint32_t row = g / numCUs, col = g % numCUs;
                        if ((row & 1u) && row < fullRows && row * numCUs >= nSplit / 2u) g = row * numCUs + (numCUs - 1u - col);
                        slots[g * 4u + (j & 3u)] = make_uint2(t, phase);
                    }
                }
            }
        }
    }
}

struct SplatShared {
    uint32_t sBuckets[kSplatWordsPerGroup * 32];
    int4 sBlocks[kSplatQueue];
    uint32_t sNumBuckets, sNumBlocks;
};

__device__ void interval_splat_group(const VhHashData& hd, const VhHashParams& hp, const VhDepthCameraParams& cp, const VhRayCastParams& rp,
                                     uint4* heads, int4* lists, uint32_t cap, uint32_t* sched, uint32_t phase, uint32_t numCUs,
                                     uint32_t nSplatGroups, uint32_t* feedback, uint32_t group, SplatShared& sh)
{
    uint32_t (&sBuckets)[kSplatWordsPerGroup * 32] = sh.sBuckets;
    int4 (&sBlocks)[kSplatQueue] = sh.sBlocks;
    uint32_t& sNumBuckets = sh.sNumBuckets;
    uint32_t& sNumBlocks = sh.sNumBlocks;
    const uint32_t nWords = (hp.m_hashNumBuckets + 31) / 32;
    const uint32_t lane = lane_id(), wave = threadIdx.x / kWave;
    const int tilesX = (int)((rp.m_width + 7) / 8), tilesY = (int)((rp.m_height + 7) / 8);
    const float vs = hp.m_virtualVoxelSize;
    const float growLo = (rp.m_useGradients ? 1.75f : 1.25f) * vs, growHi = (rp.m_useGradients ? 0.75f : 0.25f) * vs;

    if (group >= nSplatGroups) {
        schedule_tiles(sched, feedback, (uint32_t)(tilesX * tilesY), phase, numCUs, group - nSplatGroups, sched_groups((uint32_t)(tilesX * tilesY)), sBuckets);
        return;
    }
    if (threadIdx.x == 0) { sNumBuckets = 0u; sNumBlocks = 0u; }
    __syncthreads();
    if (threadIdx.x < kSplatWordsPerGroup) {
        const uint32_t wordIdx = group * kSplatWordsPerGroup + threadIdx.x;
        uint32_t bits = wordIdx < nWords ? hd.d_bucketBits[wordIdx] : 0u;
        while (bits) {
            const uint32_t bucket = wordIdx * 32u + (uint32_t)(__ffs((int)bits) - 1);
            bits &= bits - 1u;
            sBuckets[atomicAdd(&sNumBuckets, 1u)] = bucket;
        }
    }
    __syncthreads();
    const uint32_t nBuckets = sNumBuckets;
    for (uint32_t b0 = 0; b0 < nBuckets; b0 += 12u) {
        const uint32_t bi = b0 + threadIdx.x / 16u, sl = threadIdx.x % 16u;
        if (threadIdx.x < 12u * 16u && bi < nBuckets && sl < VH_HASH_BUCKET_SIZE) {
            const int4 q = load_quad(&hd.d_hash[(uint64_t)sBuckets[bi] * VH_HASH_BUCKET_SIZE + sl]);
            if (q.w != VH_FREE_ENTRY) sBlocks[atomicAdd(&sNumBlocks, 1u)] = q;
        }
        __syncthreads();
        const uint32_t nBlocks = sNumBlocks;
        for (uint32_t k = wave; k < nBlocks; k += 256 / kWave) {
            const int4 q = sBlocks[k];
            const int bx = q.x, by = q.y, bz = q.z, ptr = q.w;
            const float lox = (float)(bx * VH_SDF_BLOCK_SIZE) * vs - growLo, hix = (float)(bx * VH_SDF_BLOCK_SIZE + VH_SDF_BLOCK_SIZE) * vs + growHi;
            const float loy = (float)(by * VH_SDF_BLOCK_SIZE) * vs - growLo, hiy = (float)(by * VH_SDF_BLOCK_SIZE + VH_SDF_BLOCK_SIZE) * vs + growHi;
            const float loz = (float)(bz * VH_SDF_BLOCK_SIZE) * vs - growLo, hiz = (float)(bz * VH_SDF_BLOCK_SIZE + VH_SDF_BLOCK_SIZE) * vs + growHi;
            float zmin = pinf(), zmax = minf(), xmin = pinf(), xmax = minf(), ymin = pinf(), ymax = minf();
#pragma unroll
            for (int c = 0; c < 8; c++) {
                const F3 pc = mat_mul_p(rp.m_viewMatrix, mk3((c & 1) ? hix : lox, (c & 2) ? hiy : loy, (c & 4) ? hiz : loz));
                zmin = fminf(zmin, pc.z); zmax = fmaxf(zmax, pc.z);
                const float iz = 1.0f / fmaxf(pc.z, 1e-6f);
                const float sx = pc.x * cp.fx * iz + cp.mx, sy = pc.y * cp.fy * iz + cp.my;
                xmin = fminf(xmin, sx); xmax = fmaxf(xmax, sx);
                ymin = fminf(ymin, sy); ymax = fmaxf(ymax, sy);
            }
            if (!(zmax > 0.0f)) continue;
            int tx0 = 0, ty0 = 0, tx1 = tilesX - 1, ty1 = tilesY - 1;
            if (zmin > 0.05f) {
                const float slop = 1.0f + 1e-3f * fmaxf(fmaxf(fabsf(xmin), fabsf(xmax)), fmaxf(fabsf(ymin), fabsf(ymax)));
                tx0 = (int)fminf(fmaxf(floorf((xmin - slop) * 0.125f), 0.0f), (float)tilesX);
                ty0 = (int)fminf(fmaxf(floorf((ymin - slop) * 0.125f), 0.0f), (float)tilesY);
                tx1 = (int)fminf(fmaxf(floorf((xmax + slop) * 0.125f), -1.0f), (float)(tilesX - 1));
                ty1 = (int)fminf(fmaxf(floorf((ymax + slop) * 0.125f), -1.0f), (float)(tilesY - 1));
            }
            if (tx1 < tx0 || ty1 < ty0) continue;
            const float zs = 1e-3f * fabsf(zmax) + 0.5f * vs;
            const uint32_t lo = __float_as_uint(fmaxf(zmin - zs, 0.0f)), hi = __float_as_uint(fmaxf(zmax + zs, 0.0f));
            const uint32_t nx = (uint32_t)(tx1 - tx0 + 1), n = nx * (uint32_t)(ty1 - ty0 + 1);
            const float rnx = 1.0f / (float)nx;
            constexpr uint32_t kInFlight = 4;
            for (uint32_t base = 0; base < n; base += kInFlight * kWave) {
                uint32_t t[kInFlight], slot[kInFlight];
#pragma unroll
                for (uint32_t j = 0; j < kInFlight; j++) {
                    const uint32_t i = base + j * kWave + lane;
                    uint32_t qy, qx;
                    divmod_small(i, nx, rnx, qy, qx);
                    t[j] = (uint32_t)(ty0 + (int)qy) * (uint32_t)tilesX + (uint32_t)(tx0 + (int)qx);
                    slot[j] = 0xffffffffu;
                    if (i < n) {
                        slot[j] = atomicAdd(&heads[t[j]].z, 1u);
                    }
                }
#pragma unroll
                for (uint32_t j = 0; j < kInFlight; j++) {
                    if (slot[j] < cap) {
                        lists[(size_t)t[j] * cap + slot[j]] = make_int4(bx, by, bz, ptr);
                    } else if (slot[j] != 0xffffffffu) {
                        atomicMin(&heads[t[j]].x, lo);
                        atomicMax(&heads[t[j]].y, hi);
                    }
                }
            }
        }
        __syncthreads();
        if (threadIdx.x == 0) sNumBlocks = 0u;
        __syncthreads();
    }
}

__global__ __launch_bounds__(256) void k_interval_splat(VhHashData hd, VhHashParams hp, VhDepthCameraParams cp,
                                                        VhRayCastParams rp, uint4* heads, int4* lists, uint32_t cap,
                                                        uint32_t* sched, uint32_t phase, uint32_t numCUs, uint32_t nSplatGroups, uint32_t* feedback)
{
    __shared__ SplatShared sh;
    interval_splat_group(hd, hp, cp, rp, heads, lists, cap, sched, phase, numCUs, nSplatGroups, feedback, blockIdx.x, sh);
}

__global__ __launch_bounds__(256) void k_interval_clear(uint4* heads, uint32_t n)
{
    const uint32_t i = blockIdx.x * blockDim.x + threadIdx.x;
    if (i < n) heads[i] = make_uint4(0x7f800000u, 0u, 0u, 0u);
}


struct BlockCache {
    int bx0, by0, bz0, p0;
    int bx1, by1, bz1, p1;
    bool v0, v1;
};

VHD void cache_init(BlockCache& bc)
{
    bc.v0 = bc.v1 = false;
    bc.bx0 = bc.by0 = bc.bz0 = bc.bx1 = bc.by1 = bc.bz1 = 0;
    bc.p0 = bc.p1 = VH_FREE_ENTRY;
}

VHD int cached_lookup(const VhHashData& hd, const VhHashParams& hp, HashMod hm, BlockCache& bc, int bx, int by, int bz)
{
    if (bc.v0 && bc.bx0 == bx && bc.by0 == by && bc.bz0 == bz) return bc.p0;
    if (bc.v1 && bc.bx1 == bx && bc.by1 == by && bc.bz1 == bz) return bc.p1;
    const uint32_t h = hash_pos_fast(hm, mki3(bx, by, bz));
    const uint32_t word = hd.d_bucketBits[h >> 5];
    const int4 q = load_quad(&hd.d_hash[h * VH_HASH_BUCKET_SIZE]);
    int p;
    if (quad_matches(q, mki3(bx, by, bz))) p = q.w;
    else if (!((word >> (h & 31)) & 1u)) p = VH_FREE_ENTRY;
    else p = lookup_ptr(hd, hp, mki3(bx, by, bz));
    bc.bx1 = bc.bx0; bc.by1 = bc.by0; bc.bz1 = bc.bz0; bc.p1 = bc.p0; bc.v1 = bc.v0;
    bc.bx0 = bx; bc.by0 = by; bc.bz0 = bz; bc.p0 = p; bc.v0 = true;
    return p;
}

constexpr int kPtrUnknown = -3;

struct HashLookup {
    const VhHashData& hd;
    const VhHashParams& hp;
    HashMod hm;
    BlockCache bc;
    VHD int find(int bx, int by, int bz) { return cached_lookup(hd, hp, hm, bc, bx, by, bz); }
    VHD bool first_tap(int bx, int by, int bz, int& handle)
    {
        handle = kPtrUnknown;
        return bucket_maybe_occupied(hd, hash_pos_fast(hm, mki3(bx, by, bz)));
    }
    VHD bool resolve(int, int bxa, int bya, int bza, int bxb, int byb, int bzb, uint32_t straddle, int (&p)[8])
    {
        const int p0 = find(bxa, bya, bza);
        if (p0 == VH_FREE_ENTRY) return false;
#pragma unroll
        for (int j = 0; j < 8; j++) p[j] = p0;
        if (straddle) {
            uint32_t need = 0xfeu;
#pragma unroll
            for (uint32_t j = 1; j < 8u; j++)
                if ((j & straddle) == 0u) need &= ~(1u << j);
#pragma unroll 1
            while (need) {
                const uint32_t k = (uint32_t)__ffs((int)need) - 1u;
                const int pk = find((k & 1u) ? bxb : bxa, (k & 2u) ? byb : bya, (k & 4u) ? bzb : bza);
                if (pk == VH_FREE_ENTRY) return false;
                const uint32_t km = k & straddle;
                uint32_t same = 0u;
#pragma unroll
                for (uint32_t j = 1; j < 8u; j++) {
                    const bool eq = (j & straddle) == km;
                    p[j] = eq ? pk : p[j];
                    same |= (eq ? 1u : 0u) << j;
// ... 733 lines not shown
}
#undef VH_WAVE_STAMP
#undef VH_STAT_DECL
#undef VH_STAT_ARGS
#undef VH_STAT_STORE

struct CoAlloc {
    VhHashData hd;
    VhHashParams hp;
    VhDepthCameraData cam;
    VhDepthCameraParams cp;
    const uint32_t* bitMask;
    uint2* packed;
    HashMod hm;
    int32_t lockToken;
    uint32_t firstGroup;
};

VHD bool co_alloc(const CoAlloc& job)
{
    if (job.firstGroup == 0u || blockIdx.x < job.firstGroup) return false;
    const uint32_t g = blockIdx.x - job.firstGroup;
    if (g == 0u && threadIdx.x == 0) job.hd.d_hashCompactifiedCounter[0] = 0;
    alloc_tile(job.hd, job.hp, job.cam, job.cp, job.bitMask, job.lockToken, job.hm, job.packed, g * (256u / kWave) + (threadIdx.x / kWave));
    return true;
}

#ifndef VH_RENDER_WAVES
#define VH_RENDER_WAVES 6
#endif
template <bool GRADIENTS>
__global__ __launch_bounds__(256) __attribute__((amdgpu_waves_per_eu(VH_RENDER_WAVES, VH_RENDER_WAVES)))
void k_render(VhHashData hd, VhHashParams hp, VhRayCastData rd, VhDepthCameraParams cp, VhRayCastParams rp,
              uint4* heads, const int4* lists, uint32_t cap, uint32_t* sched, uint32_t phase, CoAlloc job)
{
    __shared__ int tileTab[256 / kWave][2u * VH_TILE_LIST_CAPACITY * kTileSlotWords];
    if (co_alloc(job)) return;
    render_tile<GRADIENTS, VH_TILE_LIST_CAPACITY>(hd, hp, rd, cp, rp, heads, lists, cap, sched, phase, tileTab);
}

template <bool GRADIENTS>
__global__ __launch_bounds__(256)
void k_render_large(VhHashData hd, VhHashParams hp, VhRayCastData rd, VhDepthCameraParams cp, VhRayCastParams rp,
                    uint4* heads, const int4* lists, uint32_t cap, uint32_t* sched, uint32_t phase, CoAlloc job)
{
    __shared__ int tileTab[256 / kWave][2u * VH_TILE_LIST_CAPACITY_LARGE * kTileSlotWords];
    if (co_alloc(job)) return;
    render_tile<GRADIENTS, VH_TILE_LIST_CAPACITY_LARGE>(hd, hp, rd, cp, rp, heads, lists, cap, sched, phase, tileTab);
}

struct CoCompactify {
    VhHashData hd;
    VhHashParams hp;
    VhDepthCameraParams cp;
    uint32_t groups;
};

struct CoSplat {
    VhRayCastParams rp;
    VhDepthCameraParams cp;
    uint4* heads;
    int4* lists;
    uint32_t* sched;
    uint32_t* feedback;
    uint32_t cap, phase, numCUs, nSplatGroups;
    uint32_t groups;
};

struct CoIntegrate {
    FusedArgs args;
    uint32_t* done;
    uint32_t listExpected, listClassExpected;
    uint32_t riderTag;
    uint32_t first;
    uint32_t groups;
};
struct NormalsKernargs {
    float4* out; const float4* in; uint32_t width, height; CoCompactify job; CoSplat splat; CoIntegrate integ;
};
constexpr uint32_t kRiderFewGroups = 128;
VHD void rider_done(const CoIntegrate& integ, const uint32_t i, const uint32_t n)
{
    if (integ.groups == 0u) return;
    __builtin_amdgcn_fence(__ATOMIC_RELEASE, "workgroup");
    __syncthreads();
    if (threadIdx.x < kWave) {
        uint32_t* const words = integ.done;
        const uint32_t padded = (n + VH_RIDER_DONE_COUNTERS - 1u) / VH_RIDER_DONE_COUNTERS * VH_RIDER_DONE_COUNTERS;
        const uint32_t add = (i + VH_RIDER_DONE_COUNTERS >= n && i + VH_RIDER_DONE_COUNTERS < padded) ? 2u : 1u;
        uint32_t last = 0;
        if (threadIdx.x == 0) {
            if (n <= kRiderFewGroups) {
                last = __hip_atomic_fetch_add(&words[2u * VH_RIDER_DONE_COUNTERS * 32u], 1u, __ATOMIC_RELAXED, __HIP_MEMORY_SCOPE_AGENT) + 1u == integ.listExpected ? 1u : 0u;
            } else {
                const uint32_t before = __hip_atomic_fetch_add(&words[(VH_RIDER_DONE_COUNTERS + i % VH_RIDER_DONE_COUNTERS) * 32u], add, __ATOMIC_RELAXED, __HIP_MEMORY_SCOPE_AGENT);
                if (before + add == integ.listClassExpected)
                    last = __hip_atomic_fetch_add(&words[2u * VH_RIDER_DONE_COUNTERS * 32u], 1u, __ATOMIC_RELAXED, __HIP_MEMORY_SCOPE_AGENT) + 1u == integ.listExpected ? 1u : 0u;
            }
        }
        last = (uint32_t)__shfl((int)last, 0);
        if (last && threadIdx.x < (uint32_t)VH_RIDER_DONE_COUNTERS)
            __hip_atomic_store(&words[threadIdx.x * 32u], integ.listExpected, __ATOMIC_RELAXED, __HIP_MEMORY_SCOPE_AGENT);
    }
}

struct PassRiderShared {
    FusedShared<false> fused;
    int4 q;
    uint32_t have, count;
};
template <uint32_t KERNARG_OFFSET>
VHD void pass_rider_group(const CoIntegrate& integ, const uint32_t group, PassRiderShared& sh)
{
    const FusedArgs& args = integ.args;
    const VhHashEntry* const list = args.hd.d_hashCompactified;
    const uint32_t nEntries = args.hp.m_hashNumBuckets * VH_HASH_BUCKET_SIZE;
    const float thr = get_truncation(args.hp, args.cp.m_sensorDepthWorldMax);
    if (threadIdx.x < kWave) {
        uint32_t have = 0u;
        if (group < nEntries) {
            const uint32_t* const flag = integ.done + (blockIdx.x % VH_RIDER_DONE_COUNTERS) * 32u;
            const uint64_t* const tagWord = reinterpret_cast<const uint64_t*>(&list[group]) + 3;
            for (uint32_t polls = 0; polls < (1u << 22); polls++) {
                const uint64_t w = __hip_atomic_load(tagWord, __ATOMIC_RELAXED, __HIP_MEMORY_SCOPE_AGENT);
                const uint32_t f = __hip_atomic_load(flag, __ATOMIC_RELAXED, __HIP_MEMORY_SCOPE_AGENT);
                if ((uint32_t)(w >> 32) == integ.riderTag) { have = 1u; break; }
                if ((int32_t)(f - integ.listExpected) >= 0) break;
                __builtin_amdgcn_s_sleep(2);
            }
        }
        int4 q = make_int4(0, 0, 0, 0);
        if (have) q = list_quad<true>(&list[group]);
        if (threadIdx.x == 0) { sh.q = q; sh.have = have; }
    }
    __syncthreads();
    const bool early = sh.have != 0u;
    if (early) integrate_block_by_workgroup<true, KERNARG_OFFSET>(args, sh.fused, sh.q, group, thr);
    if (threadIdx.x < kWave) {
        uint32_t count = 0u;
        if (rider_wait(integ.done, integ.listExpected)) count = (uint32_t)__hip_atomic_load(args.hd.d_hashCompactifiedCounter, __ATOMIC_RELAXED, __HIP_MEMORY_SCOPE_AGENT);
        else if (threadIdx.x == 0) atomicAdd(&args.hd.d_state[VH_STATE_RIDER_GAVE_UP], 1u);
        if (threadIdx.x == 0) sh.count = count;
    }
    __syncthreads();
    const uint32_t count = sh.count;
    if (args.countMirror && group == 0u && threadIdx.x == 0) *reinterpret_cast<uint2*>(args.countMirror) = make_uint2(count, args.mirrorTag);
    for (uint32_t b = group; b < count; b += integ.groups) {
        if (b == group && early) continue;
        __syncthreads();
        integrate_block_by_workgroup<true, KERNARG_OFFSET>(args, sh.fused, list_quad<true>(&list[b]), b, thr);
    }
}

__global__ __launch_bounds__(256) void k_compute_normals(float4* out, const float4* in, uint32_t width, uint32_t height, CoCompactify job, CoSplat splat, CoIntegrate integ)
{
    __shared__ union RiderShared { SplatShared splat; CompactShared compact; PassRiderShared pass; } shared;
    SplatShared& sh = shared.splat;
    uint32_t g = blockIdx.x;
    if (integ.groups != 0u && g >= integ.first) {
        static_assert(kRiderFewGroups >= VH_RIDER_DONE_COUNTERS && VH_RIDER_DONE_COUNTERS <= kWave, "one lane per flag");
#if defined(VH_KNOCKOUT) && VH_KNOCKOUT == 42
        const uint32_t riderStamp0 = (uint32_t)__builtin_amdgcn_s_memrealtime();
        uint4* const riderStampAt = reinterpret_cast<uint4*>(job.hd.d_hashCompactified) + (job.hp.m_hashNumBuckets * VH_HASH_BUCKET_SIZE) / 2u + blockIdx.x;
#endif
        pass_rider_group<(uint32_t)(offsetof(NormalsKernargs, integ) + offsetof(CoIntegrate, args))>(integ, g - integ.first, shared.pass);
#if defined(VH_KNOCKOUT) && VH_KNOCKOUT == 42
        __syncthreads();
        if (threadIdx.x == 0) *riderStampAt = make_uint4(riderStamp0, (uint32_t)__builtin_amdgcn_s_memrealtime(), 5u, 0x5742u);
#endif
        return;
    }
#if defined(VH_KNOCKOUT) && VH_KNOCKOUT == 42
    const uint32_t stamp0 = (uint32_t)__builtin_amdgcn_s_memrealtime();
    uint4* const stampAt = reinterpret_cast<uint4*>(job.hd.d_hashCompactified) + (job.hp.m_hashNumBuckets * VH_HASH_BUCKET_SIZE) / 2u + blockIdx.x;
#define VH_GROUP_STAMP(KIND) { __syncthreads(); if (threadIdx.x == 0) *stampAt = make_uint4(stamp0, (uint32_t)__builtin_amdgcn_s_memrealtime(), (KIND), 0x5742u); }
#else
#define VH_GROUP_STAMP(KIND)
#endif
#if defined(VH_KNOCKOUT) && VH_KNOCKOUT >= 31 && VH_KNOCKOUT <= 34
    {
        const uint32_t nSchedK = splat.groups - splat.nSplatGroups;
        const bool isSched = g < nSchedK, isCompact = !isSched && g - nSchedK < job.groups, isSplat = !isSched && !isCompact && g < splat.groups + job.groups;
        if (VH_KNOCKOUT == 31 && isSched) return;
        if (VH_KNOCKOUT == 32 && (isSched || isSplat)) return;
        if (VH_KNOCKOUT == 33 && isCompact) return;
        if (VH_KNOCKOUT == 34 && !isSched && !isCompact && !isSplat) return;
    }
#endif
    const uint32_t nSched = splat.groups - splat.nSplatGroups;
    if (g >= nSched && g - nSched < job.groups) {
        g -= nSched;
        if (integ.groups != 0u) compactify_group<true>(job.hd, job.hp, job.cp, g * blockDim.x + threadIdx.x, shared.compact, integ.riderTag);
        else compactify_group<false>(job.hd, job.hp, job.cp, g * blockDim.x + threadIdx.x, shared.compact);
        VH_GROUP_STAMP(3u)
        rider_done(integ, g, job.groups);
        return;
    }
    if (g >= nSched) g -= job.groups;
    if (g < splat.groups) {
        const uint32_t group = g < nSched ? splat.nSplatGroups + g : g - nSched;
        interval_splat_group(job.hd, job.hp, splat.cp, splat.rp, splat.heads, splat.lists, splat.cap, splat.sched, splat.phase, splat.numCUs,
                             splat.nSplatGroups, splat.feedback, group, sh);
        VH_GROUP_STAMP(group >= splat.nSplatGroups ? 1u : 2u)
        return;
    }
    g -= splat.groups;
    const uint32_t idx = g * blockDim.x + threadIdx.x;
#if defined(VH_KNOCKOUT) && VH_KNOCKOUT == 42
    if (job.groups != 0u && idx < width * height) {
#else
    if (idx >= width * height) return;
    {
#endif
    const uint32_t x = idx % width, y = idx / width;
    const float mi = minf();
    float4 o = make_float4(mi, mi, mi, mi);
    if (x > 0 && x < width - 1 && y > 0 && y < height - 1) {
        const float4 CC = in[idx], PC = in[idx + width], CP = in[idx + 1], MC = in[idx - width], CM = in[idx - 1];
        if (CC.x != mi && PC.x != mi && CP.x != mi && MC.x != mi && CM.x != mi) {
            const F3 a = mk3(PC.x - MC.x, PC.y - MC.y, PC.z - MC.z), b = mk3(CP.x - CM.x, CP.y - CM.y, CP.z - CM.z);
            const F3 n = mk3(a.y * b.z - a.z * b.y, a.z * b.x - a.x * b.z, a.x * b.y - a.y * b.x);
            const float l = sqrtf(dot3(n, n));
            if (l > 0.0f) o = make_float4(n.x / -l, n.y / -l, n.z / -l, 1.0f);
        }
    }
    out[idx] = o;
    }
#if defined(VH_KNOCKOUT) && VH_KNOCKOUT == 42
    if (job.groups != 0u) VH_GROUP_STAMP(4u)
#endif
}
#undef VH_GROUP_STAMP


namespace mc_tables {
#define VH_MC_QUAL __device__ const
#include "../../include/vh_mc_tables.h"
#undef VH_MC_QUAL
}

VHD int lookup_ptr_wide(const VhHashData& hd, const VhHashParams& hp, I3 blk)
{
    const uint32_t ne = hp.m_hashNumBuckets * VH_HASH_BUCKET_SIZE;
    const uint32_t h = hash_pos(hp.m_hashNumBuckets, blk);
    if (!bucket_maybe_occupied(hd, h)) return VH_FREE_ENTRY;
    const uint32_t base = h * VH_HASH_BUCKET_SIZE, idxLast = base + VH_HASH_BUCKET_SIZE - 1;
    int4 qs[VH_HASH_BUCKET_SIZE];
#pragma unroll
    for (uint32_t j = 0; j < VH_HASH_BUCKET_SIZE; j++) qs[j] = load_quad(&hd.d_hash[base + j]);
    uint32_t off = hd.d_hash[idxLast].offset;
#pragma unroll
    for (uint32_t j = 0; j < VH_HASH_BUCKET_SIZE; j++)
        if (quad_matches(qs[j], blk)) return qs[j].w;
    uint32_t maxIter = 0;
#pragma unroll 1
    while (maxIter < hp.m_hashMaxCollisionLinkedListSize) {
        if (off == 0) break;
        const uint32_t i = (idxLast + off) % ne;
        const int4 q = load_quad(&hd.d_hash[i]);
        if (quad_matches(q, blk)) return q.w;
        off = hd.d_hash[i].offset;
        maxIter++;
    }
    return VH_FREE_ENTRY;
}

__global__ void k_mc_reset(VhMarchingCubesData d)
{
    if (threadIdx.x == 0 && blockIdx.x == 0) { d.d_numTriangles[0] = 0u; d.d_numOccupiedBlocks[0] = 0u; }
}

__global__ __launch_bounds__(256) void k_mc_pass1(VhHashData hd, VhHashParams hp, VhMarchingCubesData d)
{
    const uint32_t nWords = (hp.m_hashNumBuckets + 31) / 32;
    const uint32_t wordIdx = blockIdx.x * blockDim.x + threadIdx.x;
    uint32_t bits = (wordIdx < nWords) ? hd.d_bucketBits[wordIdx] : 0u;
// ... 906 lines not shown
        if (absDI <= prm.colorThres && sqrtf(gu * gu + gv * gv) > prm.colorGradientMin) {
            const float wC = fmaxf(0.0f, 1.0f - absDI / prm.colorThres);
            const float iz = 1.0f / pp.z, wSq = pp.z * pp.z;
            const float d0 = gu * iz, d1 = gv * iz, d2 = gu * (-pp.x / wSq) + gv * (-pp.y / wSq);
            const F3 g = mk3(d0 * prm.fx, d1 * prm.fy, d0 * prm.mx + d1 * prm.my + d2);
            const float J[6] = { g.x * phiA.x + g.y * phiA.y + g.z * phiA.z, g.x * phiB.x + g.y * phiB.y + g.z * phiB.z,
                                 g.x * phiG.x + g.y * phiG.y + g.z * phiG.z, g.x, g.y, g.z };
            rgbd_add_row(acc, J, dI, prm.weightColor * wC);
        }
    }
    const uint32_t lane = lane_id();
#pragma unroll
    for (int off = 32; off > 0; off >>= 1) {
#pragma unroll
        for (uint32_t k = 0; k < kIcpTerms; k++) {
            const float other = __shfl_down(acc[k], off);
            if ((int)lane < off) acc[k] += other;
        }
    }
    if (lane == 0u) {
#pragma unroll
        for (uint32_t k = 0; k < kIcpTerms; k++) partials[(size_t)blockIdx.x * kIcpTerms + k] = acc[k];
    }
}

__global__ __launch_bounds__(64) void k_icp_rgbd_solve(VhIcpStateRGBD* st, const float* partials, uint32_t nPartials, float angleThres, float distThres, float earlyOut)
{
    __shared__ float sTerms[kIcpTerms];
    VhIcpState& s = st->icp;
    if (s.lost || s.done) return;
    const uint32_t t = threadIdx.x;
    if (t < kIcpTerms) sTerms[t] = icp_sum_term(partials, nPartials, t);
    __syncthreads();
    if (t != 0u) return;
    double A[6][6], b[6];
    const bool nonzero = icp_system_from_terms(sTerms, A, b);
    s.sumRegError = sTerms[27];
    s.sumRegWeight = sTerms[28];
    s.numCorr = (uint32_t)sTerms[29];
    s.iterations += 1u;
    if (!nonzero) { s.lost = 1u; return; }
    double xs[6];
    s.matrixCondition = icp_solve_6x6(A, b, xs);
    float x[6];
    for (int k = 0; k < 3; k++) x[k] = st->angles[k] + (float)xs[k];
    for (int k = 0; k < 3; k++) x[3 + k] = st->translation[k] + (float)xs[3 + k];
    const float cz = cosf(x[0]), sz = sinf(x[0]), cy = cosf(x[1]), sy = sinf(x[1]), cx = cosf(x[2]), sx = sinf(x[2]);
    const float R[9] = { cz * cy, cz * sy * sx - sz * cx, cz * sy * cx + sz * sx,
                         sz * cy, sz * sy * sx + cz * cx, sz * sy * cx - cz * sx,
                         -sy, cy * sx, cy * cx };
    const float angle = angle_axis_angle(R);
    const float tnorm = sqrtf(x[3] * x[3] + x[4] * x[4] + x[5] * x[5]);
    if (!(angle <= angleThres) || !(tnorm <= distThres)) { s.lost = 1u; return; }
    const float M[16] = { R[0], R[1], R[2], x[3], R[3], R[4], R[5], x[4], R[6], R[7], R[8], x[5], 0.0f, 0.0f, 0.0f, 1.0f };
    for (int k = 0; k < 16; k++) s.delta[k] = M[k];
    rgbd_linearisation_point(st, M);
    if (fabsf(s.lastError - s.sumRegError) < earlyOut) s.done = 1u;
    s.lastError = s.sumRegError;
}


__global__ __launch_bounds__(64) void k_stream_out_pass1(VhHashData hd, VhHashParams hp, uint32_t start, float radius,
                                                         float cx, float cy, float cz, uint32_t* outCounter,
                                                         VhSDFBlockDesc* out, uint32_t capacity, int32_t lockToken)
{
    const uint32_t ne = hp.m_hashNumBuckets * VH_HASH_BUCKET_SIZE;
    const uint32_t idx = blockIdx.x * blockDim.x + threadIdx.x + start;
    if (idx >= ne) return;
    VhHashEntry* e = &hd.d_hash[idx];
    const int4 q = load_quad(e);
    const uint32_t off = e->offset;
    const I3 pos = mki3(q.x, q.y, q.z);
    const F3 pw = block_to_world(hp.m_virtualVoxelSize, pos);
    const F3 df = mk3(pw.x - cx, pw.y - cy, pw.z - cz);
    const float d = sqrtf(dot3(df, df));
    if (q.w != VH_FREE_ENTRY && d >= radius) {
        bool emit = false;
        if (off != 0u || hash_pos(hp.m_hashNumBuckets, pos) != idx / VH_HASH_BUCKET_SIZE) {
            emit = delete_hash_entry_element(hd, hp, pos, lockToken);
        } else {
            append_heap(hd, (uint32_t)q.w / VH_SDF_BLOCK_VOXELS);
            delete_hash_entry(e);
            bucket_dec(hd, idx);
            emit = true;
        }
        if (emit) {
            const uint32_t addr = atomicAdd(outCounter, 1u);
            if (addr < capacity) {
                VhSDFBlockDesc dsc;
                dsc.pos[0] = q.x; dsc.pos[1] = q.y; dsc.pos[2] = q.z; dsc.ptr = q.w;
                out[addr] = dsc;
            }
        }
    }
}

VHD uint32_t chunk_bit_of_block(const VhHashParams& hp, I3 blk)
{
    const F3 pw = block_to_world(hp.m_virtualVoxelSize, blk);
    const F3 p = mk3(pw.x / hp.m_streamingVoxelExtents[0], pw.y / hp.m_streamingVoxelExtents[1], pw.z / hp.m_streamingVoxelExtents[2]);
    const I3 c = mki3(f2i(p.x + (float)signi(p.x) * 0.5f), f2i(p.y + (float)signi(p.y) * 0.5f), f2i(p.z + (float)signi(p.z) * 0.5f));
    const int qx = c.x - hp.m_streamingMinGridPos[0], qy = c.y - hp.m_streamingMinGridPos[1], qz = c.z - hp.m_streamingMinGridPos[2];
    if (qx < 0 || qy < 0 || qz < 0 || qx >= hp.m_streamingGridDimensions[0] || qy >= hp.m_streamingGridDimensions[1] || qz >= hp.m_streamingGridDimensions[2])
        return 0xffffffffu;
    return (uint32_t)(qz * hp.m_streamingGridDimensions[0] * hp.m_streamingGridDimensions[1] + qy * hp.m_streamingGridDimensions[0] + qx);
}

__global__ __launch_bounds__(64) void k_stream_out_pass1_bits(VhHashData hd, VhHashParams hp, uint32_t start, float radius,
                                                              float cx, float cy, float cz, uint32_t* outCounter,
                                                              VhSDFBlockDesc* out, uint32_t capacity, int32_t lockToken, uint32_t* bitMask)
{
    const uint32_t ne = hp.m_hashNumBuckets * VH_HASH_BUCKET_SIZE;
    const uint32_t idx = blockIdx.x * blockDim.x + threadIdx.x + start;
    if (idx >= ne) return;
    VhHashEntry* e = &hd.d_hash[idx];
    const int4 q = load_quad(e);
    const uint32_t off = e->offset;
    const I3 pos = mki3(q.x, q.y, q.z);
    const F3 pw = block_to_world(hp.m_virtualVoxelSize, pos);
    const F3 df = mk3(pw.x - cx, pw.y - cy, pw.z - cz);
    const float d = sqrtf(dot3(df, df));
    if (q.w != VH_FREE_ENTRY && d >= radius) {
        bool emit = false;
        if (off != 0u || hash_pos(hp.m_hashNumBuckets, pos) != idx / VH_HASH_BUCKET_SIZE) {
            emit = delete_hash_entry_element(hd, hp, pos, lockToken);
        } else {
            append_heap(hd, (uint32_t)q.w / VH_SDF_BLOCK_VOXELS);
            delete_hash_entry(e);
            bucket_dec(hd, idx);
            emit = true;
        }
        if (emit) {
            const uint32_t addr = atomicAdd(outCounter, 1u);
            if (addr < capacity) {
                VhSDFBlockDesc dsc;
                dsc.pos[0] = q.x; dsc.pos[1] = q.y; dsc.pos[2] = q.z; dsc.ptr = q.w;
                out[addr] = dsc;
                const uint32_t bit = chunk_bit_of_block(hp, pos);
                if (bitMask && bit != 0xffffffffu) atomicOr(&bitMask[bit >> 5], 1u << (bit & 31u));
            }
        }
    }
}

__global__ __launch_bounds__(256) void k_stream_out_probe(VhHashData hd, VhHashParams hp, uint32_t start, uint32_t n, float radius,
                                                          float cx, float cy, float cz, uint32_t* counter)
{
    const uint32_t ne = hp.m_hashNumBuckets * VH_HASH_BUCKET_SIZE;
    const uint32_t t = blockIdx.x * blockDim.x + threadIdx.x, idx = t + start;
    bool would = false;
    if (t < n && idx < ne) {
        const int4 q = load_quad(&hd.d_hash[idx]);
        const F3 pw = block_to_world(hp.m_virtualVoxelSize, mki3(q.x, q.y, q.z));
        const F3 df = mk3(pw.x - cx, pw.y - cy, pw.z - cz);
        would = q.w != VH_FREE_ENTRY && sqrtf(dot3(df, df)) >= radius;
    }
    const unsigned long long m = __ballot(would);
    if (m != 0ull && lane_id() == 0u) atomicAdd(counter, (uint32_t)__popcll(m));
}

__global__ void k_publish_and_clear(uint32_t* src, uint32_t* mapped, uint32_t tag)
{
    mapped[0] = *src;
    mapped[1] = 0u;
    *src = 0u;
    __atomic_thread_fence(__ATOMIC_RELEASE);
    __hip_atomic_store(&mapped[2], tag, __ATOMIC_RELEASE, __HIP_MEMORY_SCOPE_SYSTEM);
}

__global__ __launch_bounds__(256) void k_stream_out_pass2(VhHashData hd, const VhSDFBlockDesc* descs, VhVoxel* out, uint32_t n)
{
    const uint32_t b = blockIdx.x;
    if (b >= n) return;
    const int ptr = __builtin_amdgcn_readfirstlane(descs[b].ptr);
    uint4* src = reinterpret_cast<uint4*>(&hd.d_SDFBlocks[(uint32_t)ptr]) + threadIdx.x;
    reinterpret_cast<uint4*>(out)[(size_t)b * 256 + threadIdx.x] = *src;
    *src = make_uint4(0u, 0u, 0u, 0u);
}

__global__ __launch_bounds__(256) void k_stream_out_pass2_counted(VhHashData hd, const VhSDFBlockDesc* descs, VhVoxel* out, const uint32_t* counter, uint32_t capacity)
{
    const uint32_t b = blockIdx.x, n = min(*counter, capacity);
    if (b >= n) return;
    const int ptr = __builtin_amdgcn_readfirstlane(descs[b].ptr);
    uint4* src = reinterpret_cast<uint4*>(&hd.d_SDFBlocks[(uint32_t)ptr]) + threadIdx.x;
    reinterpret_cast<uint4*>(out)[(size_t)b * 256 + threadIdx.x] = *src;
    *src = make_uint4(0u, 0u, 0u, 0u);
}

__global__ void k_publish_count(const uint32_t* counter, uint32_t* mapped, uint32_t tag)
{
    mapped[0] = *counter;
    mapped[1] = 0u;
    __atomic_thread_fence(__ATOMIC_RELEASE);
    __hip_atomic_store(&mapped[2], tag, __ATOMIC_RELEASE, __HIP_MEMORY_SCOPE_SYSTEM);
}

__global__ __launch_bounds__(64) void k_stream_in_pass1_dev(VhHashData hd, VhHashParams hp, uint32_t n, const VhSDFBlockDesc* descs, int32_t lockToken,
                                                            uint32_t* failed, uint32_t* bitMask, uint32_t chunkBit)
{
    const uint32_t i = blockIdx.x * blockDim.x + threadIdx.x;
    if (i >= n) return;
    const uint32_t heapCountPrev = hd.d_heapCounter[0];
    if (n > heapCountPrev + 1u) return;
    if (i == 0u && bitMask && chunkBit != 0xffffffffu) atomicAnd(&bitMask[chunkBit >> 5], ~(1u << (chunkBit & 31u)));
    const uint32_t ptr = hd.d_heap[heapCountPrev - i] * VH_SDF_BLOCK_VOXELS;
    const VhSDFBlockDesc dsc = descs[i];
    if (!insert_hash_entry(hd, hp, mki3(dsc.pos[0], dsc.pos[1], dsc.pos[2]), (int)ptr, lockToken)) {
        atomicAdd(&hd.d_state[VH_STATE_INSERT_FAILED], 1u);
        failed[1u + atomicAdd(&failed[0], 1u)] = i;
    }
}
__global__ __launch_bounds__(256) void k_stream_in_pass2_dev(VhHashData hd, uint32_t n, const VhVoxel* blocks)
{
    const uint32_t b = blockIdx.x;
    if (b >= n) return;
    const uint32_t heapCountPrev = hd.d_heapCounter[0];
    if (n > heapCountPrev + 1u) return;
    const uint32_t ptr = hd.d_heap[heapCountPrev - b] * VH_SDF_BLOCK_VOXELS;
    *(reinterpret_cast<uint4*>(&hd.d_SDFBlocks[ptr]) + threadIdx.x) = reinterpret_cast<const uint4*>(blocks)[(size_t)b * 256 + threadIdx.x];
}
__global__ void k_stream_in_commit(VhHashData hd, uint32_t n, const uint32_t* failed, uint32_t* mapped, uint32_t tag)
{
    const uint32_t heapCountPrev = hd.d_heapCounter[0];
    const bool exhausted = n > heapCountPrev + 1u;
    if (!exhausted) hd.d_heapCounter[0] = heapCountPrev - n;
    else atomicAdd(&hd.d_state[VH_STATE_HEAP_UNDERFLOW], 1u);
    mapped[0] = failed[0];
    mapped[1] = heapCountPrev;
    mapped[3] = exhausted ? 1u : 0u;
    __atomic_thread_fence(__ATOMIC_RELEASE);
    __hip_atomic_store(&mapped[2], tag, __ATOMIC_RELEASE, __HIP_MEMORY_SCOPE_SYSTEM);
}

__global__ __launch_bounds__(64) void k_stream_in_pass1(VhHashData hd, VhHashParams hp, uint32_t n, uint32_t heapCountPrev,
                                                        const VhSDFBlockDesc* descs, int32_t lockToken, uint32_t* failed)
{
    const uint32_t i = blockIdx.x * blockDim.x + threadIdx.x;
    if (i >= n) return;
    const uint32_t ptr = hd.d_heap[heapCountPrev - i] * VH_SDF_BLOCK_VOXELS;
    const VhSDFBlockDesc dsc = descs[i];
    if (!insert_hash_entry(hd, hp, mki3(dsc.pos[0], dsc.pos[1], dsc.pos[2]), (int)ptr, lockToken)) {
        atomicAdd(&hd.d_state[VH_STATE_INSERT_FAILED], 1u);
        if (failed) failed[1u + atomicAdd(&failed[0], 1u)] = i;
    }
}

__global__ __launch_bounds__(256) void k_stream_in_pass2(VhHashData hd, uint32_t n, uint32_t heapCountPrev, const VhVoxel* blocks)
{
    const uint32_t b = blockIdx.x;
    if (b >= n) return;
    const uint32_t ptr = hd.d_heap[heapCountPrev - b] * VH_SDF_BLOCK_VOXELS;
    *(reinterpret_cast<uint4*>(&hd.d_SDFBlocks[ptr]) + threadIdx.x) = reinterpret_cast<const uint4*>(blocks)[(size_t)b * 256 + threadIdx.x];
}


struct SynthArgs {
    double spheres[4 * 8];
    int nSpheres;
    int inside;
    float T[16];
};

__global__ __launch_bounds__(256) void k_synth(SynthArgs a, VhDepthCameraParams cp, float* depth, float4* color)
{
    const uint32_t idx = blockIdx.x * blockDim.x + threadIdx.x;
    if (idx >= cp.m_imageWidth * cp.m_imageHeight) return;
    const uint32_t u = idx % cp.m_imageWidth, v = idx / cp.m_imageWidth;
    const double ox = (double)a.T[3], oy = (double)a.T[7], oz = (double)a.T[11];
    const double dx = ((double)u - (double)cp.mx) / (double)cp.fx;
    const double dy = ((double)v - (double)cp.my) / (double)cp.fy;
    const double wx = (double)a.T[0] * dx + (double)a.T[1] * dy + (double)a.T[2];
    const double wy = (double)a.T[4] * dx + (double)a.T[5] * dy + (double)a.T[6];
    const double wz = (double)a.T[8] * dx + (double)a.T[9] * dy + (double)a.T[10];
    const double aa = wx * wx + wy * wy + wz * wz;
    double bestT = 0.0;
    int best = -1;
    for (int s = 0; s < a.nSpheres; s++) {
        const double cx = a.spheres[4 * s + 0], cy = a.spheres[4 * s + 1], cz = a.spheres[4 * s + 2], r = a.spheres[4 * s + 3];
        const double ocx = ox - cx, ocy = oy - cy, ocz = oz - cz;
        const double b = ocx * wx + ocy * wy + ocz * wz;
        const double c = ocx * ocx + ocy * ocy + ocz * ocz - r * r;
        const double disc = b * b - aa * c;
        if (disc < 0.0) continue;
        const double sq = sqrt(disc);
        const double t = a.inside ? (-b + sq) / aa : (-b - sq) / aa;
        if (t > 0.0 && (best < 0 || t < bestT)) { bestT = t; best = s; }
    }
    const float mi = minf();
    if (best < 0) {
        depth[idx] = mi;
        color[idx] = make_float4(mi, mi, mi, mi);
    } else {
        const double cx = a.spheres[4 * best + 0], cy = a.spheres[4 * best + 1], cz = a.spheres[4 * best + 2], r = a.spheres[4 * best + 3];
        const double px = ox + bestT * wx, py = oy + bestT * wy, pz = oz + bestT * wz;
        double nx = (px - cx) / r, ny = (py - cy) / r, nz = (pz - cz) / r;
        if (a.inside) { nx = -nx; ny = -ny; nz = -nz; }
        depth[idx] = (float)bestT;
        color[idx] = make_float4((float)(0.5 + 0.5 * nx), (float)(0.5 + 0.5 * ny), (float)(0.5 + 0.5 * nz), 1.0f);
    }
}

__global__ void k_debug_hash_ops(VhHashData hd, VhHashParams hp, const int32_t* ops, int32_t* results, uint32_t n)
{
    if (blockIdx.x != 0 || threadIdx.x != 0) return;
    int32_t token = 1;
    for (uint32_t i = 0; i < n; i++) {
        const int32_t op = ops[5 * i + 0];
        const I3 p = mki3(ops[5 * i + 1], ops[5 * i + 2], ops[5 * i + 3]);
        const int32_t arg = ops[5 * i + 4];
        int32_t r = 0;
        switch (op) {
        case VH_OP_ALLOC: r = alloc_block(hd, hp, p, token); break;
        case VH_OP_DELETE: r = delete_hash_entry_element(hd, hp, p, token) ? 1 : 0; break;
        case VH_OP_INSERT: r = insert_hash_entry(hd, hp, p, arg, token) ? 1 : 0; break;
        case VH_OP_LOOKUP: r = lookup_ptr(hd, hp, p); break;
        case VH_OP_NEW_PASS: token++; break;
        default: break;
        }
        __builtin_amdgcn_fence(__ATOMIC_ACQ_REL, "agent");
        results[i] = r;
    }
}

__global__ __launch_bounds__(256) void k_check_fast_math(float b, HashMod hm, uint32_t n, uint32_t seed, uint32_t* mismatches)
{
    const uint32_t i = blockIdx.x * blockDim.x + threadIdx.x;
    if (i >= n) return;
    uint32_t s = (i + 1u) * 2654435761u ^ seed;
    s ^= s >> 15; s *= 2246822519u; s ^= s >> 13; s *= 3266489917u; s ^= s >> 16;
    uint32_t u = s * 747796405u + 2891336453u;
    float a;
    if ((i & 7u) == 7u) {
        a = __uint_as_float(u);
        const uint32_t ex = (u >> 23) & 0xffu;
        if (ex == 0xffu || ex < 0x10u || ex > 0xe8u) a = (float)(int)u * 1.0e-6f;
    } else {
        a = ((float)(int)u) * (1.0f / 2147483648.0f) * (((i >> 3) & 1u) ? 400.0f : 8.0f);
    }
    const float rb = 1.0f / b;
    const float q0 = a / b, q1 = div_exact(a, b, rb);
    if (__float_as_uint(q0) != __float_as_uint(q1) && !(q0 == 0.0f && q1 == 0.0f)) atomicAdd(&mismatches[0], 1u);
    if ((s % hm.d) != umod_fast(s, hm)) atomicAdd(&mismatches[1], 1u);
    if ((u % hm.d) != umod_fast(u, hm)) atomicAdd(&mismatches[1], 1u);
    if (i < 64u) {
        const uint32_t e = 0xffffffffu - i;
        if ((e % hm.d) != umod_fast(e, hm)) atomicAdd(&mismatches[1], 1u);
        if ((i % hm.d) != umod_fast(i, hm)) atomicAdd(&mismatches[1], 1u);
    }
}

__global__ __launch_bounds__(256) void k_check_refined_division(uint32_t n, uint32_t seed, uint32_t* mismatches)
{
    const uint32_t i = blockIdx.x * blockDim.x + threadIdx.x;
    if (i >= n) return;
    uint32_t s = (i + 1u) * 2654435761u ^ seed;
    s ^= s >> 15; s *= 2246822519u; s ^= s >> 13; s *= 3266489917u; s ^= s >> 16;
    const uint32_t u = s * 747796405u + 2891336453u, t = u * 2654435761u + 40503u;
    const uint32_t dExp = 127u - 20u + (s >> 8) % 41u, nExpP = 127u - 100u + (u >> 8) % 161u, nExpB = 127u - 100u + (t >> 8) % 190u;
    float d = __uint_as_float((dExp << 23) | (s & 0x7fffffu));
    if (dExp == 127u + 20u) d = 0x1p20f;
    float nP = __uint_as_float((u & 0x80000000u) | (nExpP << 23) | (u & 0x7fffffu));
    if (nExpP == 127u + 60u) nP = copysignf(0x1p60f, nP);
    if ((i & 1023u) == 0u) nP = (i & 1024u) ? 0.0f : -0.0f;
    if ((i & 1023u) == 1u) { d = 1.0f + (float)(i >> 10) * 0x1p-23f; nP = __uint_as_float(0x3fffffffu - (s & 0xffu)); }
    const float dB = (float)(1u + (s >> 3) % 510u);
    const float nB = __uint_as_float((t & 0x80000000u) | (nExpB << 23) | (t & 0x7fffffu));
    const f32x2 dd = (f32x2){ d, dB }, nn = (f32x2){ nP, nB };
    const f32x2 q = div_refined2(nn, dd, rcp_refined2(dd));
    const float wantP = nP / d, wantB = nB / dB;
    if (__float_as_uint(q.x) != __float_as_uint(wantP) && !(wantP == 0.0f && q.x == 0.0f)) atomicAdd(&mismatches[0], 1u);
    if (__float_as_uint(q.y) != __float_as_uint(wantB)) atomicAdd(&mismatches[1], 1u);
}

inline uint32_t cdiv(uint64_t a, uint64_t b) { return (uint32_t)((a + b - 1) / b); }

inline HashMod make_hash_mod(uint32_t d)
{
    HashMod k;
    k.d = d;
    uint32_t l = 0;
    while ((1ull << l) < (uint64_t)d) l++;
    k.m = (uint32_t)((((1ull << 32) * ((1ull << l) - (uint64_t)d)) / d) + 1ull);
    k.sh = l - 1;
    return k;
}

}


extern "C" {

int vh_reset(const VhHashData* hd, const VhHashParams* hp, vhStream_t stream)
{
    if (!hd || !hp || !hd->d_hash) return VH_ERR_BAD_ARGUMENT;
    hipStream_t s = (hipStream_t)stream;
    const uint32_t nb = hp->m_hashNumBuckets, ne = nb * VH_HASH_BUCKET_SIZE, nblk = hp->m_numSDFBlocks;
    VH_HIP(hipMemsetAsync(hd->d_SDFBlocks, 0, sizeof(VhVoxel) * (size_t)nblk * VH_SDF_BLOCK_VOXELS, s));
    VH_HIP(hipMemsetAsync(hd->d_bucketCount, 0, sizeof(uint32_t) * nb, s));
    VH_HIP(hipMemsetAsync(hd->d_bucketBits, 0, sizeof(uint32_t) * ((nb + 31) / 32), s));
    VH_HIP(hipMemsetAsync(hd->d_state, 0, sizeof(uint32_t) * VH_STATE_WORDS, s));
    VH_HIP(hipMemsetAsync(hd->d_hashDecision, 0, sizeof(int32_t) * ne, s));
    VH_HIP(hipMemsetAsync(hd->d_hashCompactifiedCounter, 0, sizeof(int32_t), s));
    k_reset_heap<<<cdiv(nblk, 256), 256, 0, s>>>(hd->d_heap, hd->d_heapCounter, nblk);
    k_reset_hash<<<cdiv(2ull * ne, 256), 256, 0, s>>>(hd->d_hash, hd->d_hashCompactified, ne);
    k_fill_i32<<<cdiv(nb, 256), 256, 0, s>>>(hd->d_hashBucketMutex, VH_FREE_ENTRY, nb);
    return vh_last_launch_error();
}

int vh_reset_bucket_mutex(const VhHashData* hd, const VhHashParams* hp, vhStream_t stream)
{
    if (!hd || !hp) return VH_ERR_BAD_ARGUMENT;
    k_fill_i32<<<cdiv(hp->m_hashNumBuckets, 256), 256, 0, (hipStream_t)stream>>>(hd->d_hashBucketMutex, VH_FREE_ENTRY, hp->m_hashNumBuckets);
    return vh_last_launch_error();
}

int vh_alloc(const VhHashData* hd, const VhHashParams* hp, const VhDepthCameraData* cam,
             const VhDepthCameraParams* cp, const uint32_t* d_bitMask, int32_t lockToken, vhStream_t stream)
{
    if (!hd || !hp || !cam || !cp || !cam->d_depthData) return VH_ERR_BAD_ARGUMENT;
    const uint32_t tiles = cdiv(cp->m_imageWidth, 8) * cdiv(cp->m_imageHeight, 8);
    if (tiles == 0) return VH_OK;
    if (hp->m_hashNumBuckets < 2) return VH_ERR_BAD_ARGUMENT;
    k_alloc<<<cdiv(tiles, 8), 512, 0, (hipStream_t)stream>>>(*hd, *hp, *cam, *cp, d_bitMask, lockToken, make_hash_mod(hp->m_hashNumBuckets), nullptr);
    return vh_last_launch_error();
}

int vh_alloc_job(VhFrameJob* job, vhStream_t stream)
{
    if (!job || !job->cam.d_depthData || !job->hashData.d_hash) return VH_ERR_BAD_ARGUMENT;
    const uint32_t tiles = cdiv(job->cp.m_imageWidth, 8) * cdiv(job->cp.m_imageHeight, 8);
    if (job->hashParams.m_hashNumBuckets < 2) return VH_ERR_BAD_ARGUMENT;
    job->allocLaunched = 1;
    if (tiles == 0) return VH_OK;
    k_alloc<<<cdiv(tiles, 8), 512, 0, (hipStream_t)stream>>>(job->hashData, job->hashParams, job->cam, job->cp, job->d_bitMask, job->lockToken,
                                                             make_hash_mod(job->hashParams.m_hashNumBuckets), reinterpret_cast<uint2*>(job->d_packedFrame));
    return vh_last_launch_error();
}

int vh_compactify_job(VhFrameJob* job, vhStream_t stream)
{
    if (!job || !job->hashData.d_hash) return VH_ERR_BAD_ARGUMENT;
    job->compactifyLaunched = 1;
    const uint32_t nWords = (job->hashParams.m_hashNumBuckets + 31) / 32;
    k_compactify<<<cdiv(nWords, 256), 256, 0, (hipStream_t)stream>>>(job->hashData, job->hashParams, job->cp);
    return vh_last_launch_error();
}

int vh_compactify(const VhHashData* hd, const VhHashParams* hp, const VhDepthCameraParams* cp,
                  uint32_t* numOccupied, uint32_t flags, vhStream_t stream)
{
    if (!hd || !hp || !cp) return VH_ERR_BAD_ARGUMENT;
    hipStream_t s = (hipStream_t)stream;
    if (!(flags & VH_COMPACT_COUNTER_IS_ZERO)) VH_HIP(hipMemsetAsync(hd->d_hashCompactifiedCounter, 0, sizeof(int32_t), s));
    const uint32_t nWords = (hp->m_hashNumBuckets + 31) / 32;
    k_compactify<<<cdiv(nWords, 256), 256, 0, s>>>(*hd, *hp, *cp);
    int err = vh_last_launch_error();
    if (err) return err;
    if (numOccupied) {
        VH_HIP(hipMemcpyAsync(numOccupied, hd->d_hashCompactifiedCounter, sizeof(uint32_t), hipMemcpyDeviceToHost, s));
        VH_HIP(hipStreamSynchronize(s));
    }
    return VH_OK;
}

int vh_integrate(const VhHashData* hd, const VhHashParams* hp, const VhDepthCameraData* cam,
                 const VhDepthCameraParams* cp, vhStream_t stream)
{
    if (!hd || !hp || !cam || !cp || !cam->d_depthData) return VH_ERR_BAD_ARGUMENT;
    if (hp->m_numOccupiedBlocks == 0) return VH_OK;
    k_integrate<false><<<hp->m_numOccupiedBlocks, 256, 0, (hipStream_t)stream>>>(*hd, *hp, *cam, *cp, 0u, VH_LOCK_ENTRY, nullptr);
    return vh_last_launch_error();
}

static uint32_t device_num_cus();

int vh_integrate_fused(const VhHashData* hd, const VhHashParams* hp, const VhDepthCameraData* cam,
                       const VhDepthCameraParams* cp, uint32_t flags, int32_t lockToken, uint32_t* d_countMirror, uint32_t mirrorTag,
                       const void* d_packedFrame, vhStream_t stream)
{
    if (!hd || !hp || !cam || !cp || !cam->d_depthData) return VH_ERR_BAD_ARGUMENT;
    if (cp->m_imageWidth > 0xffffu || cp->m_imageHeight > 0xffffu) return VH_ERR_BAD_ARGUMENT;
    const uint32_t want = cdiv(hp->m_numSDFBlocks, 4), most = device_num_cus() * 8u;
    const uint32_t grid = want < most ? want : most;
    const uint2* packed = reinterpret_cast<const uint2*>(d_packedFrame);
    FusedArgs args;
    args.hd = *hd; args.hp = *hp; args.cam = *cam; args.cp = *cp;
    args.flags = flags; args.lockToken = lockToken; args.countMirror = d_countMirror; args.mirrorTag = mirrorTag;
    args.packed = reinterpret_cast<const uint2*>(packed);
    if (packed) VH_LAUNCH_TIMED(k_integrate_fused<true>, grid, 256, (hipStream_t)stream, args);
    else VH_LAUNCH_TIMED(k_integrate_fused<false>, grid, 256, (hipStream_t)stream, args);
    return vh_last_launch_error();
}

int vh_starve(const VhHashData* hd, const VhHashParams* hp, vhStream_t stream)
{
    if (!hd || !hp) return VH_ERR_BAD_ARGUMENT;
    if (hp->m_numOccupiedBlocks == 0) return VH_OK;
    k_starve<<<hp->m_numOccupiedBlocks, 256, 0, (hipStream_t)stream>>>(*hd, *hp);
    return vh_last_launch_error();
}

int vh_gc_identify(const VhHashData* hd, const VhHashParams* hp, const VhDepthCameraParams* cp, vhStream_t stream)
{
    if (!hd || !hp || !cp) return VH_ERR_BAD_ARGUMENT;
    if (hp->m_numOccupiedBlocks == 0) return VH_OK;
    k_gc_identify<<<hp->m_numOccupiedBlocks, 256, 0, (hipStream_t)stream>>>(*hd, *hp, *cp);
    return vh_last_launch_error();
}

int vh_gc_free(const VhHashData* hd, const VhHashParams* hp, int32_t lockToken, vhStream_t stream)
{
    if (!hd || !hp) return VH_ERR_BAD_ARGUMENT;
    if (hp->m_numOccupiedBlocks == 0) return VH_OK;
    k_gc_free<<<hp->m_numOccupiedBlocks, 256, 0, (hipStream_t)stream>>>(*hd, *hp, lockToken);
    return vh_last_launch_error();
}

int vh_bind_input_depth_color_textures(const VhDepthCameraData* cam)
{
    (void)cam;
    return VH_OK;
}

int vh_render(const VhHashData* hd, const VhHashParams* hp, const VhRayCastData* rd,
              const VhDepthCameraParams* cp, const VhRayCastParams* rp, vhStream_t stream)
{
    if (!hd || !hp || !rd || !cp || !rp || !rd->d_depth) return VH_ERR_BAD_ARGUMENT;
    const uint32_t tiles = cdiv(rp->m_width, 8) * cdiv(rp->m_height, 8);
    if (tiles == 0) return VH_OK;
    if (hp->m_hashNumBuckets < 2) return VH_ERR_BAD_ARGUMENT;
    const HashMod hm = make_hash_mod(hp->m_hashNumBuckets);
    if (rp->m_useGradients) k_render_hash<true><<<cdiv(tiles, 4), 256, 0, (hipStream_t)stream>>>(*hd, *hp, *rd, *cp, *rp, hm);
    else k_render_hash<false><<<cdiv(tiles, 4), 256, 0, (hipStream_t)stream>>>(*hd, *hp, *rd, *cp, *rp, hm);
    return vh_last_launch_error();
}

static uint32_t device_num_cus()
{
    static int numCUs = 0;
    if (numCUs == 0) {
        int dev = 0;
        if (hipGetDevice(&dev) != hipSuccess || hipDeviceGetAttribute(&numCUs, hipDeviceAttributeMultiprocessorCount, dev) != hipSuccess || numCUs <= 0)
            numCUs = 256;
    }
    return (uint32_t)numCUs;
}

size_t vh_render_schedule_bytes(uint32_t width, uint32_t height)
{
    const size_t tiles = (size_t)cdiv(width, 8) * cdiv(height, 8);
    return (4u + 4u * ((tiles + 3u) / 4u) + 2u * 4u * ((tiles + kSplitTiles + 3u) / 4u)) * sizeof(uint32_t);
}

uint32_t vh_render_split_tiles(uint32_t width, uint32_t height) { return split_tiles(cdiv(width, 8) * cdiv(height, 8)); }

int vh_render_intervals_co(const VhHashData* hd, const VhHashParams* hp, const VhRayCastData* rd, const VhDepthCameraParams* cp,
                           const VhRayCastParams* rp, uint32_t* d_tileHeads, const VhTileBlock* d_tileBlocks, uint32_t tileCapacity,
                           uint32_t* d_schedule, uint32_t phase, VhFrameJob* fj, vhStream_t stream)
{
    if (!hd || !hp || !rd || !cp || !rp || !rd->d_depth || !d_tileHeads) return VH_ERR_BAD_ARGUMENT;
    const uint32_t tiles = cdiv(rp->m_width, 8) * cdiv(rp->m_height, 8);
    if (tiles == 0) return VH_OK;
    uint4* h = reinterpret_cast<uint4*>(d_tileHeads);
    const int4* l = reinterpret_cast<const int4*>(d_tileBlocks);
    const uint32_t cap = d_tileBlocks ? tileCapacity : 0u;
    const bool large = cap > (uint32_t)VH_TILE_LIST_CAPACITY;
    uint32_t groups = cdiv(tiles + (d_schedule ? split_tiles(tiles) : 0u), 4);
    CoAlloc job;
    std::memset(&job, 0, sizeof(job));
    if (fj && !fj->allocLaunched && fj->cam.d_depthData && fj->hashData.d_hash && fj->hashParams.m_hashNumBuckets >= 2) {
        const uint32_t allocTiles = cdiv(fj->cp.m_imageWidth, 8) * cdiv(fj->cp.m_imageHeight, 8);
        job.hd = fj->hashData; job.hp = fj->hashParams; job.cam = fj->cam; job.cp = fj->cp;
        job.bitMask = fj->d_bitMask;
        job.packed = reinterpret_cast<uint2*>(fj->d_packedFrame);
        job.hm = make_hash_mod(fj->hashParams.m_hashNumBuckets);
        job.lockToken = fj->lockToken;
        job.firstGroup = groups;
        groups += cdiv(allocTiles, 4);
        fj->allocLaunched = 1;
    }
    const dim3 grid(groups);
    hipStream_t st = (hipStream_t)stream;
    if (rp->m_useGradients) {
        if (large) VH_LAUNCH_TIMED(k_render_large<true>, grid, 256, st, *hd, *hp, *rd, *cp, *rp, h, l, cap, d_schedule, phase, job);
        else VH_LAUNCH_TIMED(k_render<true>, grid, 256, st, *hd, *hp, *rd, *cp, *rp, h, l, cap, d_schedule, phase, job);
    } else {
        if (large) VH_LAUNCH_TIMED(k_render_large<false>, grid, 256, st, *hd, *hp, *rd, *cp, *rp, h, l, cap, d_schedule, phase, job);
        else VH_LAUNCH_TIMED(k_render<false>, grid, 256, st, *hd, *hp, *rd, *cp, *rp, h, l, cap, d_schedule, phase, job);
    }
    return vh_last_launch_error();
}

int vh_render_intervals(const VhHashData* hd, const VhHashParams* hp, const VhRayCastData* rd, const VhDepthCameraParams* cp,
                        const VhRayCastParams* rp, uint32_t* d_tileHeads, const VhTileBlock* d_tileBlocks, uint32_t tileCapacity,
                        uint32_t* d_schedule, uint32_t phase, vhStream_t stream)
{
    return vh_render_intervals_co(hd, hp, rd, cp, rp, d_tileHeads, d_tileBlocks, tileCapacity, d_schedule, phase, nullptr, stream);
}

int vh_ray_interval_clear(uint32_t* d_tileHeads, uint32_t width, uint32_t height, vhStream_t stream)
{
    if (!d_tileHeads) return VH_ERR_BAD_ARGUMENT;
    const uint32_t tiles = cdiv(width, 8) * cdiv(height, 8);
    if (tiles == 0) return VH_OK;
    k_interval_clear<<<cdiv(tiles, 256), 256, 0, (hipStream_t)stream>>>(reinterpret_cast<uint4*>(d_tileHeads), tiles);
    return vh_last_launch_error();
}

int vh_ray_interval_splat(const VhHashData* hd, const VhHashParams* hp, const VhDepthCameraParams* cp, const VhRayCastParams* rp,
                          uint32_t* d_tileHeads, VhTileBlock* d_tileBlocks, uint32_t tileCapacity, uint32_t* d_schedule, uint32_t phase,
                          uint32_t* d_longestList, vhStream_t stream)
{
    if (!hd || !hp || !cp || !rp || !d_tileHeads) return VH_ERR_BAD_ARGUMENT;
    if (rp->m_width == 0 || rp->m_height == 0) return VH_OK;
    const uint32_t numCUs = d_schedule ? device_num_cus() : 256u;
    const uint32_t nWords = (hp->m_hashNumBuckets + 31) / 32;
    const uint32_t groups = cdiv(nWords, kSplatWordsPerGroup);
    const uint32_t nSched = d_schedule ? sched_groups(cdiv(rp->m_width, 8) * cdiv(rp->m_height, 8)) : 0u;
    k_interval_splat<<<groups + nSched, 256, 0, (hipStream_t)stream>>>(*hd, *hp, *cp, *rp, reinterpret_cast<uint4*>(d_tileHeads),
                                                                                 reinterpret_cast<int4*>(d_tileBlocks), d_tileBlocks ? tileCapacity : 0u,
                                                                                 d_schedule, phase, numCUs, groups, d_longestList);
    return vh_last_launch_error();
}

int vh_compute_normals_co2(float* d_output4, const float* d_input4, uint32_t width, uint32_t height, VhFrameJob* fj,
                           const VhRayCastParams* nextView, uint32_t* d_tileHeads, VhTileBlock* d_tileBlocks, uint32_t tileCapacity,
                           uint32_t* d_schedule, uint32_t phase, uint32_t* d_longestList, vhStream_t stream)
{
    if (!d_output4 || !d_input4) return VH_ERR_BAD_ARGUMENT;
    if (width * height == 0) return VH_OK;
    uint32_t groups = cdiv((uint64_t)width * height, 256);
    CoCompactify job;
    std::memset(&job, 0, sizeof(job));
    CoSplat sp;
    std::memset(&sp, 0, sizeof(sp));
    if (fj && fj->allocLaunched && !fj->compactifyLaunched && fj->hashData.d_hash) {
        job.hd = fj->hashData; job.hp = fj->hashParams; job.cp = fj->cp;
        job.groups = cdiv((fj->hashParams.m_hashNumBuckets + 31) / 32, 256);
        groups += job.groups;
        fj->compactifyLaunched = 1;
        if (nextView && d_tileHeads && nextView->m_width != 0 && nextView->m_height != 0) {
            sp.rp = *nextView; sp.cp = fj->cp;
            sp.heads = reinterpret_cast<uint4*>(d_tileHeads);
            sp.lists = reinterpret_cast<int4*>(d_tileBlocks);
            sp.sched = d_schedule; sp.feedback = d_longestList;
            sp.cap = d_tileBlocks ? tileCapacity : 0u;
            sp.phase = phase;
            sp.numCUs = d_schedule ? device_num_cus() : 256u;
            sp.nSplatGroups = cdiv((fj->hashParams.m_hashNumBuckets + 31) / 32, kSplatWordsPerGroup);
            sp.groups = sp.nSplatGroups + (d_schedule ? sched_groups(cdiv(nextView->m_width, 8) * cdiv(nextView->m_height, 8)) : 0u);
            groups += sp.groups;
        }
    }
    CoIntegrate integ;
    std::memset(&integ, 0, sizeof(integ));
    if (fj && job.groups != 0u &&
        fj->fusedPrepared && !fj->fusedLaunched && fj->d_riderDone && fj->d_packedFrame && fj->cam.d_depthData &&
        fj->cp.m_imageWidth <= 0xffffu && fj->cp.m_imageHeight <= 0xffffu) {
        integ.args.hd = fj->hashData; integ.args.hp = fj->hashParams; integ.args.cam = fj->cam; integ.args.cp = fj->cp;
        integ.args.flags = fj->fusedFlags; integ.args.lockToken = fj->fusedLockToken;
        integ.args.countMirror = fj->d_countMirror; integ.args.mirrorTag = fj->mirrorTag;
        integ.args.packed = reinterpret_cast<const uint2*>(fj->d_packedFrame);
        integ.done = fj->d_riderDone;
        integ.riderTag = 0x80000000u | fj->mirrorTag;
        if (job.groups <= kRiderFewGroups) {
            fj->listDoneTotal += job.groups;
        } else {
            fj->listClassTotal += cdiv(job.groups, VH_RIDER_DONE_COUNTERS);
            fj->listDoneTotal += VH_RIDER_DONE_COUNTERS;
        }
        integ.listExpected = fj->listDoneTotal;
        integ.listClassExpected = fj->listClassTotal;
        integ.first = groups;
        const uint32_t want = cdiv(fj->hashParams.m_numSDFBlocks, 4), most = device_num_cus() * 8u;
        integ.groups = want < most ? want : most;
        groups += integ.groups;
        fj->fusedLaunched = 1;
    }
    VH_LAUNCH_TIMED(k_compute_normals, groups, 256, (hipStream_t)stream, reinterpret_cast<float4*>(d_output4), reinterpret_cast<const float4*>(d_input4), width, height, job, sp, integ);
    return vh_last_launch_error();
}

int vh_compute_normals_co(float* d_output4, const float* d_input4, uint32_t width, uint32_t height, VhFrameJob* fj, vhStream_t stream)
{
    return vh_compute_normals_co2(d_output4, d_input4, width, height, fj, nullptr, nullptr, nullptr, 0u, nullptr, 0u, nullptr, stream);
}

int vh_compute_normals(float* d_output4, const float* d_input4, uint32_t width, uint32_t height, vhStream_t stream)
{
    return vh_compute_normals_co(d_output4, d_input4, width, height, nullptr, stream);
}

int vh_reset_marching_cubes(const VhMarchingCubesData* data, vhStream_t stream)
{
    if (!data || !data->d_numTriangles || !data->d_numOccupiedBlocks) return VH_ERR_BAD_ARGUMENT;
    k_mc_reset<<<1, 64, 0, (hipStream_t)stream>>>(*data);
    return vh_last_launch_error();
}

int vh_extract_iso_surface_pass1(const VhHashData* hd, const VhHashParams* hp, const VhMarchingCubesData* data, vhStream_t stream)
{
    if (!hd || !hp || !data || !data->d_occupiedBlocks) return VH_ERR_BAD_ARGUMENT;
    const uint32_t nWords = (hp->m_hashNumBuckets + 31) / 32;
    k_mc_pass1<<<cdiv(nWords, 256), 256, 0, (hipStream_t)stream>>>(*hd, *hp, *data);
    return vh_last_launch_error();
}

int vh_extract_iso_surface_pass2(const VhHashData* hd, const VhHashParams* hp, const VhMarchingCubesData* data,
                                 uint32_t numOccupiedBlocks, vhStream_t stream)
{
    if (!hd || !hp || !data || !data->d_params || !data->d_triangles) return VH_ERR_BAD_ARGUMENT;
    if (numOccupiedBlocks == 0) return VH_OK;
    k_mc_pass2<<<numOccupiedBlocks, 512, 0, (hipStream_t)stream>>>(*hd, *hp, *data, numOccupiedBlocks);
    return vh_last_launch_error();
}

#define VH_IMG_LAUNCH(n) cdiv((uint32_t)(n), 256u), 256, 0, (hipStream_t)stream

int vh_convert_color_raw_to_float4(float* d_output4, const uint8_t* d_inputRGBX, uint32_t width, uint32_t height, vhStream_t stream)
{
    if (!d_output4 || !d_inputRGBX) return VH_ERR_BAD_ARGUMENT;
    if (width * height == 0) return VH_OK;
    k_convert_color_raw_to_float4<<<VH_IMG_LAUNCH(width * height)>>>(reinterpret_cast<float4*>(d_output4), reinterpret_cast<const uint32_t*>(d_inputRGBX), width * height);
    return vh_last_launch_error();
}
int vh_upload_frame(const float* hostDepth, const uint8_t* hostRGBX, float* d_depth, float* d_color4, uint32_t width, uint32_t height, vhStream_t stream)
{
    if (!hostDepth || !d_depth || (hostRGBX && !d_color4)) return VH_ERR_BAD_ARGUMENT;
    const uint32_t n = width * height;
    if (n == 0) return VH_OK;
    if (n % 4u) return VH_ERR_BAD_ARGUMENT;
    const uint32_t nQuads = n / 4u;
// ... 328 lines not shown
```

### voxelhashing_amd/lib.py

```python
import ctypes as C
import os

import numpy as np

from . import vhtypes as T

_HERE = os.path.dirname(os.path.abspath(__file__))
LIB_PATH = os.environ.get("VH_LIB_PATH") or os.path.join(_HERE, "libvoxelhashing_amd.so")
_LIB = None

P = C.POINTER
_F16 = P(C.c_float)
_VP = C.c_void_p

PROTOTYPES = {
    "vh_version": (C.c_char_p, []),
    "vh_error_string": (C.c_char_p, [C.c_int]),
    "vh_last_error_message": (C.c_char_p, []),
    "vh_malloc": (C.c_int, [P(_VP), C.c_size_t]),
    "vh_free": (C.c_int, [_VP]),
    "vh_malloc_host": (C.c_int, [P(_VP), C.c_size_t]),
    "vh_free_host": (C.c_int, [_VP]),
    "vh_memcpy_h2d": (C.c_int, [_VP, _VP, C.c_size_t, _VP]),
    "vh_memcpy_d2h": (C.c_int, [_VP, _VP, C.c_size_t, _VP]),
    "vh_memset": (C.c_int, [_VP, C.c_int, C.c_size_t, _VP]),
    "vh_time_next_launch": (C.c_int, [_VP, _VP]),
    "vh_stream_create": (C.c_int, [P(_VP)]),
    "vh_stream_destroy": (C.c_int, [_VP]),
    "vh_stream_synchronize": (C.c_int, [_VP]),
    "vh_device_synchronize": (C.c_int, []),
    "vh_hash_data_alloc": (C.c_int, [P(T.HashData), P(T.HashParams)]),
    "vh_hash_data_free": (C.c_int, [P(T.HashData)]),
    "vh_reset": (C.c_int, [P(T.HashData), P(T.HashParams), _VP]),
    "vh_reset_bucket_mutex": (C.c_int, [P(T.HashData), P(T.HashParams), _VP]),
    "vh_alloc": (C.c_int, [P(T.HashData), P(T.HashParams), P(T.DepthCameraData), P(T.DepthCameraParams), _VP, C.c_int32, _VP]),
    "vh_compactify": (C.c_int, [P(T.HashData), P(T.HashParams), P(T.DepthCameraParams), P(C.c_uint32), C.c_uint32, _VP]),
    "vh_integrate": (C.c_int, [P(T.HashData), P(T.HashParams), P(T.DepthCameraData), P(T.DepthCameraParams), _VP]),
    "vh_starve": (C.c_int, [P(T.HashData), P(T.HashParams), _VP]),
    "vh_gc_identify": (C.c_int, [P(T.HashData), P(T.HashParams), P(T.DepthCameraParams), _VP]),
    "vh_gc_free": (C.c_int, [P(T.HashData), P(T.HashParams), C.c_int32, _VP]),
    "vh_bind_input_depth_color_textures": (C.c_int, [P(T.DepthCameraData)]),
    "vh_integrate_fused": (C.c_int, [P(T.HashData), P(T.HashParams), P(T.DepthCameraData), P(T.DepthCameraParams), C.c_uint32, C.c_int32, _VP, C.c_uint32, _VP, _VP]),
    "vh_alloc_job": (C.c_int, [P(T.FrameJob), _VP]),
    "vh_compactify_job": (C.c_int, [P(T.FrameJob), _VP]),
    "vh_render": (C.c_int, [P(T.HashData), P(T.HashParams), P(T.RayCastData), P(T.DepthCameraParams), P(T.RayCastParams), _VP]),
    "vh_ray_interval_clear": (C.c_int, [_VP, C.c_uint32, C.c_uint32, _VP]),
    "vh_ray_interval_splat": (C.c_int, [P(T.HashData), P(T.HashParams), P(T.DepthCameraParams), P(T.RayCastParams), _VP, _VP, C.c_uint32, _VP, C.c_uint32, _VP, _VP]),
    "vh_render_intervals": (C.c_int, [P(T.HashData), P(T.HashParams), P(T.RayCastData), P(T.DepthCameraParams), P(T.RayCastParams), _VP, _VP, C.c_uint32, _VP, C.c_uint32, _VP]),
    "vh_render_schedule_bytes": (C.c_size_t, [C.c_uint32, C.c_uint32]),
    "vh_render_split_tiles": (C.c_uint32, [C.c_uint32, C.c_uint32]),
    "vh_compute_normals": (C.c_int, [_VP, _VP, C.c_uint32, C.c_uint32, _VP]),
    "vh_render_intervals_co": (C.c_int, [P(T.HashData), P(T.HashParams), P(T.RayCastData), P(T.DepthCameraParams), P(T.RayCastParams), _VP, _VP, C.c_uint32, _VP, C.c_uint32, P(T.FrameJob), _VP]),
    "vh_compute_normals_co": (C.c_int, [_VP, _VP, C.c_uint32, C.c_uint32, P(T.FrameJob), _VP]),
    "vh_compute_normals_co2": (C.c_int, [_VP, _VP, C.c_uint32, C.c_uint32, P(T.FrameJob), P(T.RayCastParams), _VP, _VP, C.c_uint32, _VP, C.c_uint32, _VP, _VP]),
    "vh_stream_out_pass1": (C.c_int, [P(T.HashData), P(T.HashParams), C.c_uint32, C.c_uint32, C.c_float, _F16, _VP, _VP, C.c_uint32, C.c_int32, _VP]),
    "vh_stream_out_pass2": (C.c_int, [P(T.HashData), P(T.HashParams), _VP, _VP, C.c_uint32, _VP]),
    "vh_stream_out_device": (C.c_int, [P(T.HashData), P(T.HashParams), C.c_uint32, C.c_uint32, C.c_float, _F16, _VP, _VP, _VP, C.c_uint32, C.c_int32, _VP, _VP]),
    "vh_publish_count": (C.c_int, [_VP, _VP, C.c_uint32, _VP]),
    "vh_stream_in_device": (C.c_int, [P(T.HashData), P(T.HashParams), C.c_uint32, _VP, _VP, C.c_int32, _VP, _VP, C.c_uint32, _VP, C.c_uint32, _VP]),
    "vh_stream_in_pass1": (C.c_int, [P(T.HashData), P(T.HashParams), C.c_uint32, C.c_uint32, _VP, C.c_int32, _VP]),
    "vh_stream_in_pass1_report": (C.c_int, [P(T.HashData), P(T.HashParams), C.c_uint32, C.c_uint32, _VP, C.c_int32, _VP, _VP]),
    "vh_stream_in_pass2": (C.c_int, [P(T.HashData), P(T.HashParams), C.c_uint32, C.c_uint32, _VP, _VP, _VP]),
    "vh_synth_frame": (C.c_int, [_VP, C.c_int, C.c_int, _F16, P(T.DepthCameraParams), _VP, _VP, _VP]),
    "vh_debug_hash_ops": (C.c_int, [P(T.HashData), P(T.HashParams), _VP, _VP, C.c_uint32, _VP]),
    "vh_debug_check_fast_math": (C.c_int, [C.c_float, C.c_uint32, C.c_uint32, C.c_uint32, _VP, _VP]),
    "vh_debug_valu_probe": (C.c_int, [C.c_uint32, C.c_uint32, C.c_uint32, _VP, P(C.c_uint32), _VP]),
    "vh_debug_check_refined_division": (C.c_int, [C.c_uint32, C.c_uint32, _VP, _VP]),
    "vh_publish_words": (C.c_int, [_VP, _VP, _VP, C.c_uint32, _VP]),
    "vh_stream_out_probe": (C.c_int, [_VP, _VP, C.c_uint32, C.c_uint32, C.c_float, _VP, _VP, _VP, C.c_uint32, _VP]),
    "vh_scene_rep_create": (C.c_int, [P(T.HashParams), P(T.SceneOptions), _VP, P(_VP)]),
    "vh_scene_rep_destroy": (None, [_VP]),
    "vh_scene_rep_integrate": (C.c_int, [_VP, _F16, P(T.DepthCameraData), P(T.DepthCameraParams), _VP]),
    "vh_scene_rep_set_last_rigid_transform_and_compactify": (C.c_int, [_VP, _F16, P(T.DepthCameraParams)]),
    "vh_scene_rep_reset": (C.c_int, [_VP]),
    "vh_scene_rep_get_hash_data": (C.c_int, [_VP, P(T.HashData)]),
    "vh_scene_rep_get_hash_params": (C.c_int, [_VP, P(T.HashParams)]),
    "vh_scene_rep_get_heap_free_count": (C.c_int, [_VP, P(C.c_uint32)]),
    "vh_scene_rep_get_num_occupied_blocks": (C.c_int, [_VP, P(C.c_uint32)]),
    "vh_scene_rep_debug_hash": (C.c_int, [_VP, P(C.c_uint32)]),
    "vh_scene_rep_get_state": (C.c_int, [_VP, P(C.c_uint32)]),
    "vh_scene_rep_get_timings": (C.c_int, [_VP, P(C.c_double)]),
    "vh_scene_rep_set_options": (C.c_int, [_VP, P(T.SceneOptions)]),
    "vh_scene_rep_integrate_ahead": (C.c_int, [_VP, _F16, P(T.DepthCameraData), P(T.DepthCameraParams), _VP, P(P(T.FrameJob))]),
    "vh_scene_rep_integrate_finish": (C.c_int, [_VP, P(T.DepthCameraData), P(T.DepthCameraParams)]),
    "vh_raycast_create": (C.c_int, [P(T.RayCastParams), _VP, P(_VP)]),
    "vh_raycast_destroy": (None, [_VP]),
    "vh_raycast_render": (C.c_int, [_VP, P(T.HashData), P(T.HashParams), P(T.DepthCameraParams), _F16]),
    "vh_raycast_render_co": (C.c_int, [_VP, P(T.HashData), P(T.HashParams), P(T.DepthCameraParams), _F16, P(T.FrameJob)]),
    "vh_raycast_get_data": (C.c_int, [_VP, P(T.RayCastData)]),
    "vh_raycast_get_params": (C.c_int, [_VP, P(T.RayCastParams)]),
    "vh_raycast_get_timings": (C.c_int, [_VP, P(C.c_double)]),
    "vh_raycast_get_event_pair_overhead": (C.c_int, [_VP, P(C.c_double)]),
    "vh_raycast_set_timing": (C.c_int, [_VP, C.c_int]),
    "vh_raycast_set_timing_stride": (C.c_int, [_VP, C.c_int, C.c_uint32]),
    "vh_raycast_set_interval_splatting": (C.c_int, [_VP, C.c_int]),
    "vh_reconstruction_default_options": (None, [P(T.ReconstructionOptions)]),
    "vh_reconstruction_create": (C.c_int, [_VP, _VP, _VP, P(T.DepthCameraParams), P(T.ReconstructionOptions), P(_VP)]),
    "vh_reconstruction_destroy": (None, [_VP]),
    "vh_reconstruction_run": (C.c_int, [_VP, P(T.SequenceFrame), C.c_uint32]),
    "vh_reconstruction_run_ahead": (C.c_int, [_VP, P(T.SequenceFrame), C.c_uint32, P(T.SequenceFrame)]),
    "vh_reconstruction_synchronize": (C.c_int, [_VP]),
    "vh_reconstruction_debug_fail_render": (C.c_int, [_VP, C.c_uint32]),
    "vh_reconstruction_get_stats": (C.c_int, [_VP, P(T.ReconstructionStats)]),
    "vh_reconstruction_reset": (C.c_int, [_VP]),
    "vh_convert_color_raw_to_float4": (C.c_int, [_VP, _VP, C.c_uint32, C.c_uint32, _VP]),
    "vh_upload_frame": (C.c_int, [_VP, _VP, _VP, _VP, C.c_uint32, C.c_uint32, _VP]),
    "vh_resample_float_map": (C.c_int, [_VP, C.c_uint32, C.c_uint32, _VP, C.c_uint32, C.c_uint32, _VP]),
    "vh_resample_float4_map": (C.c_int, [_VP, C.c_uint32, C.c_uint32, _VP, C.c_uint32, C.c_uint32, _VP]),
    "vh_copy_float_map": (C.c_int, [_VP, _VP, C.c_uint32, C.c_uint32, _VP]),
    "vh_copy_float4_map": (C.c_int, [_VP, _VP, C.c_uint32, C.c_uint32, _VP]),
    "vh_set_invalid_float_map": (C.c_int, [_VP, C.c_uint32, C.c_uint32, _VP]),
    "vh_convert_color_to_intensity_float": (C.c_int, [_VP, _VP, C.c_uint32, C.c_uint32, _VP]),
    "vh_convert_depth_float_to_camera_space_float4": (C.c_int, [_VP, _VP, P(T.DepthCameraParams), C.c_uint32, C.c_uint32, _VP]),
    "vh_gauss_filter_float_map": (C.c_int, [_VP, _VP, C.c_float, C.c_float, C.c_uint32, C.c_uint32, _VP]),
    "vh_gauss_filter_float4_map": (C.c_int, [_VP, _VP, C.c_float, C.c_float, C.c_uint32, C.c_uint32, _VP]),
    "vh_bilateral_filter_float_map": (C.c_int, [_VP, _VP, C.c_float, C.c_float, C.c_uint32, C.c_uint32, _VP]),
    "vh_erode_depth_map": (C.c_int, [_VP, _VP, C.c_int32, C.c_uint32, C.c_uint32, C.c_float, C.c_float, _VP]),
# ... 228 lines not shown
```

Measured before the change: 20900.

## Compactify from a dense per-block table instead of scanning hash bucket bitmaps

Adds a dense table indexed by SDF block id that holds each allocated block's position and hash slot, plus a high-water mark. Every alloc, insert and delete path keeps the table in sync. Compactify now walks only the table up to that mark, instead of scanning bucket bitmaps and then hash slots. The grid size becomes the minimum of the bucket-based and block-based counts. Hash offsets are fetched lazily, only for kept entries. This cuts scan traffic over a large, sparse hash table, at the cost of extra table writes and a wave-level atomicMax on every allocation, plus an extra gather of offsets.

Result: no change. 20930 (median of 3 runs) (+0.2%).

```diff
diff --git a/include/vh_api.h b/include/vh_api.h
--- a/include/vh_api.h
+++ b/include/vh_api.h
@@ -30,6 +30,7 @@
 int vh_hash_data_free(VhHashData* hd);
 
 int vh_reset(const VhHashData* hd, const VhHashParams* hp, vhStream_t stream);
+int vh_block_table_rebuild(const VhHashData* hd, const VhHashParams* hp, vhStream_t stream);
 int vh_reset_bucket_mutex(const VhHashData* hd, const VhHashParams* hp, vhStream_t stream);
 int vh_alloc(const VhHashData* hd, const VhHashParams* hp, const VhDepthCameraData* cam,
              const VhDepthCameraParams* cp, const uint32_t* d_bitMask, int32_t lockToken, vhStream_t stream);
@@ -98,6 +99,7 @@
 enum { VH_OP_ALLOC = 0, VH_OP_DELETE = 1, VH_OP_INSERT = 2, VH_OP_LOOKUP = 3, VH_OP_NEW_PASS = 4 };
 int vh_debug_hash_ops(const VhHashData* hd, const VhHashParams* hp, const int32_t* d_ops, int32_t* d_results,
                       uint32_t n, vhStream_t stream);
+int vh_debug_block_table(const VhHashData* hd, const VhHashParams* hp, int32_t* h_table, uint32_t* h_end, vhStream_t stream);
 
 int vh_debug_check_fast_math(float divisor, uint32_t modulus, uint32_t n, uint32_t seed, uint32_t* d_mismatches, vhStream_t stream);
 
diff --git a/include/vh_types.h b/include/vh_types.h
--- a/include/vh_types.h
+++ b/include/vh_types.h
@@ -101,6 +101,11 @@
     uint32_t* d_bucketBits;
     uint32_t* d_state;
 } VhHashData;
+
+#define VH_BUCKET_BITS_WORDS(nb) ((((uint64_t)(nb) + 31u) / 32u + 63u) / 64u * 64u)
+#define VH_BLOCK_TABLE_END_WORD(nb) VH_BUCKET_BITS_WORDS(nb)
+#define VH_BLOCK_TABLE_WORD(nb) (VH_BUCKET_BITS_WORDS(nb) + 64u)
+#define VH_BUCKET_BITS_BYTES(nb, nblk) (4u * VH_BLOCK_TABLE_WORD(nb) + 16u * (uint64_t)(nblk))
 
 enum {
     VH_STATE_HEAP_UNDERFLOW = 0,
diff --git a/voxelhashing_amd/csrc/vh_device.hpp b/voxelhashing_amd/csrc/vh_device.hpp
--- a/voxelhashing_amd/csrc/vh_device.hpp
+++ b/voxelhashing_amd/csrc/vh_device.hpp
@@ -188,6 +188,34 @@
     return (hd.d_bucketBits[h >> 5] >> (h & 31)) & 1u;
 }
 
+VHD uint32_t* block_table_end(const VhHashData& hd, const VhHashParams& hp) { return hd.d_bucketBits + VH_BLOCK_TABLE_END_WORD(hp.m_hashNumBuckets); }
+VHD int4* block_table(const VhHashData& hd, const VhHashParams& hp)
+{
+    return reinterpret_cast<int4*>(hd.d_bucketBits + VH_BLOCK_TABLE_WORD(hp.m_hashNumBuckets));
+}
+VHD void table_set(const VhHashData& hd, const VhHashParams& hp, int ptr, I3 pos, uint32_t slot)
+{
+    const uint32_t id = (uint32_t)ptr / VH_SDF_BLOCK_VOXELS;
+    if (id < hp.m_numSDFBlocks) block_table(hd, hp)[id] = make_int4(pos.x, pos.y, pos.z, (int)slot);
+}
+VHD void table_clear(const VhHashData& hd, const VhHashParams& hp, int ptr)
+{
+    const uint32_t id = (uint32_t)ptr / VH_SDF_BLOCK_VOXELS;
+    if (id < hp.m_numSDFBlocks) block_table(hd, hp)[id] = make_int4(0, 0, 0, VH_FREE_ENTRY);
+}
+VHD void table_raise(const VhHashData& hd, const VhHashParams& hp, uint32_t end)
+{
+    uint64_t m = __ballot(end != 0u);
+    if (m == 0ull) return;
+    uint32_t top = 0u;
+    while (m != 0ull) {
+        const int l = __ffsll((unsigned long long)m) - 1;
+        top = max(top, (uint32_t)__builtin_amdgcn_readlane((int)end, l));
+        m &= m - 1ull;
+    }
+    if ((int)(threadIdx.x & 63u) == __ffsll((unsigned long long)__ballot(true)) - 1) atomicMax(block_table_end(hd, hp), top);
+}
+
 VHD uint32_t consume_heap(const VhHashData& hd, uint32_t numSDFBlocks, bool& ok)
 {
     uint32_t addr = atomicSub(&hd.d_heapCounter[0], 1u);
@@ -237,7 +265,7 @@
     return VH_FREE_ENTRY;
 }
 
-VHD int alloc_block(const VhHashData& hd, const VhHashParams& hp, I3 pos, int32_t lockToken)
+VHD int alloc_block(const VhHashData& hd, const VhHashParams& hp, I3 pos, int32_t lockToken, uint32_t& end)
 {
     const uint32_t ne = hp.m_hashNumBuckets * VH_HASH_BUCKET_SIZE;
     uint32_t h = hash_pos(hp.m_hashNumBuckets, pos);
@@ -282,6 +310,8 @@
             e->offset = VH_NO_OFFSET;
             store_quad(e, make_int4(pos.x, pos.y, pos.z, (int)(blk * VH_SDF_BLOCK_VOXELS)));
             bucket_inc(hd, (uint32_t)firstEmpty);
+            table_set(hd, hp, (int)(blk * VH_SDF_BLOCK_VOXELS), pos, (uint32_t)firstEmpty);
+            end = blk + 1u;
             return 1;
         }
         atomicAdd(&hd.d_state[VH_STATE_ALLOC_LOCK_LOST], 1u);
@@ -312,6 +342,8 @@
                     __threadfence();
                     hd.d_hash[idxLast].offset = (uint32_t)offset;
                     bucket_inc(hd, i);
+                    table_set(hd, hp, (int)(blk * VH_SDF_BLOCK_VOXELS), pos, i);
+                    end = blk + 1u;
                     return 1;
                 }
             }
@@ -336,6 +368,7 @@
             e->offset = 0;
             store_quad(e, make_int4(pos.x, pos.y, pos.z, ptr));
             bucket_inc(hd, base + j);
+            table_set(hd, hp, ptr, pos, base + j);
             return true;
         }
     }
@@ -356,6 +389,7 @@
             store_quad(e, make_int4(pos.x, pos.y, pos.z, ptr));
             hd.d_hash[idxLast].offset = (uint32_t)offset;
             bucket_inc(hd, i);
+            table_set(hd, hp, ptr, pos, i);
             return true;
         }
         maxIter++;
@@ -380,14 +414,18 @@
                 if (prev == lockToken) return false;
                 append_heap(hd, (uint32_t)q.w / VH_SDF_BLOCK_VOXELS);
                 uint32_t nextIdx = (i + off) % ne;
+                const int4 moved = load_quad(&hd.d_hash[nextIdx]);
                 copy_entry(&hd.d_hash[i], &hd.d_hash[nextIdx]);
                 delete_hash_entry(&hd.d_hash[nextIdx]);
                 bucket_dec(hd, nextIdx);
+                table_clear(hd, hp, q.w);
+                table_set(hd, hp, moved.w, mki3(moved.x, moved.y, moved.z), i);
                 return true;
             } else {
                 append_heap(hd, (uint32_t)q.w / VH_SDF_BLOCK_VOXELS);
                 delete_hash_entry(&hd.d_hash[i]);
                 bucket_dec(hd, i);
+                table_clear(hd, hp, q.w);
                 return true;
             }
         }
@@ -406,6 +444,7 @@
             append_heap(hd, (uint32_t)q.w / VH_SDF_BLOCK_VOXELS);
             delete_hash_entry(&hd.d_hash[i]);
             bucket_dec(hd, i);
+            table_clear(hd, hp, q.w);
             hd.d_hash[prevIdx].offset = off;
             return true;
         }
@@ -434,6 +473,7 @@
         const uint32_t old = atomicSub(&hd.d_bucketCount[h], 1u);
         hd.d_heap[addr + 1] = (uint32_t)q.w / VH_SDF_BLOCK_VOXELS;
         delete_hash_entry(&hd.d_hash[i]);
+        table_clear(hd, hp, q.w);
         if (old == 1u) atomicAnd(&hd.d_bucketBits[h >> 5], ~(1u << (h & 31)));
         ok = true;
     }
diff --git a/voxelhashing_amd/csrc/vh_host.cpp b/voxelhashing_amd/csrc/vh_host.cpp
--- a/voxelhashing_amd/csrc/vh_host.cpp
+++ b/voxelhashing_amd/csrc/vh_host.cpp
@@ -156,7 +156,7 @@
     VH_ALLOC(d_SDFBlocks, sizeof(VhVoxel) * nblk * VH_SDF_BLOCK_VOXELS)
     VH_ALLOC(d_hashBucketMutex, sizeof(int32_t) * nb)
     VH_ALLOC(d_bucketCount, sizeof(uint32_t) * nb)
-    VH_ALLOC(d_bucketBits, sizeof(uint32_t) * ((nb + 31) / 32))
+    VH_ALLOC(d_bucketBits, VH_BUCKET_BITS_BYTES(nb, nblk))
     VH_ALLOC(d_state, sizeof(uint32_t) * VH_STATE_WORDS)
 #undef VH_ALLOC
     if (err) {
diff --git a/voxelhashing_amd/csrc/vh_kernels.hip b/voxelhashing_amd/csrc/vh_kernels.hip
--- a/voxelhashing_amd/csrc/vh_kernels.hip
+++ b/voxelhashing_amd/csrc/vh_kernels.hip
@@ -31,6 +31,26 @@
         reinterpret_cast<int4*>(a)[idx] = v;
         reinterpret_cast<int4*>(b)[idx] = v;
     }
+}
+
+__global__ __launch_bounds__(256) void k_block_table_clear(VhHashData hd, VhHashParams hp)
+{
+    const uint32_t i = blockIdx.x * blockDim.x + threadIdx.x;
+    if (i == 0u) *block_table_end(hd, hp) = 0u;
+    if (i < hp.m_numSDFBlocks) block_table(hd, hp)[i] = make_int4(0, 0, 0, VH_FREE_ENTRY);
+}
+__global__ __launch_bounds__(256) void k_block_table_from_hash(VhHashData hd, VhHashParams hp)
+{
+    const uint32_t i = blockIdx.x * blockDim.x + threadIdx.x;
+    uint32_t end = 0u;
+    if (i < hp.m_hashNumBuckets * VH_HASH_BUCKET_SIZE) {
+        const int4 q = load_quad(&hd.d_hash[i]);
+        if (q.w >= 0 && (uint32_t)q.w / VH_SDF_BLOCK_VOXELS < hp.m_numSDFBlocks) {
+            table_set(hd, hp, q.w, mki3(q.x, q.y, q.z), i);
+            end = (uint32_t)q.w / VH_SDF_BLOCK_VOXELS + 1u;
+        }
+    }
+    table_raise(hd, hp, end);
 }
 
 __global__ __launch_bounds__(256) void k_fill_i32(int32_t* p, int32_t v, uint32_t n)
@@ -132,7 +152,9 @@
             pending &= ~__ballot(same);
             leads = leads || (int)lane == leader;
         }
-        if (leads) alloc_block(hd, hp, id, lockToken);
+        uint32_t end = 0u;
+        if (leads) alloc_block(hd, hp, id, lockToken, end);
+        table_raise(hd, hp, end);
         if (active) {
             if (tMax.x < tMax.y && tMax.x < tMax.z) {
                 id.x = f2i((float)id.x + step.x);
@@ -257,9 +279,15 @@
 struct CompactShared {
     int4 q[kCompactQueue];
     uint32_t off[kCompactQueue];
-    uint32_t n, base, nBuckets;
-    uint16_t buckets[256 * 32];
+    uint32_t n, base;
 };
+__host__ __device__ inline uint32_t compact_groups(uint32_t numBuckets, uint32_t numSDFBlocks)
+{
+    const uint32_t byBuckets = (uint32_t)(((uint64_t)numBuckets + 32u * 256u - 1u) / (32u * 256u));
+    const uint32_t byBlocks = (numSDFBlocks + 255u) / 256u;
+    return byBuckets < byBlocks ? byBuckets : byBlocks;
+}
+
 template <bool COHERENT> VHD void list_store(VhHashEntry* o, const int4 q, const uint4 box)
 {
     if (COHERENT) {
@@ -267,7 +295,7 @@
         __hip_atomic_store(w + 0, (uint64_t)(uint32_t)q.x | ((uint64_t)(uint32_t)q.y << 32), __ATOMIC_RELAXED, __HIP_MEMORY_SCOPE_AGENT);
         __hip_atomic_store(w + 1, (uint64_t)(uint32_t)q.z | ((uint64_t)(uint32_t)q.w << 32), __ATOMIC_RELAXED, __HIP_MEMORY_SCOPE_AGENT);
         __hip_atomic_store(w + 2, (uint64_t)box.x | ((uint64_t)box.y << 32), __ATOMIC_RELAXED, __HIP_MEMORY_SCOPE_AGENT);
-        __builtin_amdgcn_fence(__ATOMIC_RELEASE, "workgroup");
+        asm volatile("s_waitcnt vmcnt(0)" ::: "memory");
         __hip_atomic_store(w + 3, (uint64_t)box.z | ((uint64_t)box.w << 32), __ATOMIC_RELAXED, __HIP_MEMORY_SCOPE_AGENT);
     } else {
         *(reinterpret_cast<uint4*>(o) + 1) = box;
@@ -294,79 +322,54 @@
 }
 
 template <bool COHERENT = false>
-__device__ void compactify_group(const VhHashData& hd, const VhHashParams& hp, const VhDepthCameraParams& cp, uint32_t wordIdx, CompactShared& sh, const uint32_t riderTag = 0u)
-{
-    const uint32_t nWords = (hp.m_hashNumBuckets + 31) / 32;
+__device__ void compactify_group(const VhHashData& hd, const VhHashParams& hp, const VhDepthCameraParams& cp, const uint32_t group, const uint32_t nGroups,
+                                 CompactShared& sh, const uint32_t riderTag = 0u)
+{
     const uint32_t tag = COHERENT ? riderTag : frame_tag(hp, cp);
     const uint32_t lane = lane_id();
+    const uint32_t ne = hp.m_hashNumBuckets * VH_HASH_BUCKET_SIZE, nIds = hp.m_numSDFBlocks;
+    const int4* const table = block_table(hd, hp);
 #if defined(VH_KNOCKOUT) && VH_KNOCKOUT == 42
     uint32_t phase[6];
     phase[0] = (uint32_t)__builtin_amdgcn_s_memrealtime();
 #define VH_COMPACT_PHASE(I) phase[I] = (uint32_t)__builtin_amdgcn_s_memrealtime();
-#define VH_COMPACT_PHASES_OUT { __syncthreads(); if (threadIdx.x == 0) { uint4* const at = reinterpret_cast<uint4*>(hd.d_hashCompactified) + (hp.m_hashNumBuckets * VH_HASH_BUCKET_SIZE) / 2u + 8192u + 2u * (wordIdx / 256u); \
-        at[0] = make_uint4(phase[0], phase[1], phase[2], 0x5743u); at[1] = make_uint4(phase[3], phase[4], (uint32_t)__builtin_amdgcn_s_memrealtime(), sh.n | (sh.nBuckets << 16)); } }
+#define VH_COMPACT_PHASES_OUT { __syncthreads(); if (threadIdx.x == 0) { uint4* const at = reinterpret_cast<uint4*>(hd.d_hashCompactified) + (hp.m_hashNumBuckets * VH_HASH_BUCKET_SIZE) / 2u + 8192u + 2u * group; \
+        at[0] = make_uint4(phase[0], phase[1], phase[2], 0x5743u); at[1] = make_uint4(phase[3], phase[4], (uint32_t)__builtin_amdgcn_s_memrealtime(), sh.n | (min(end, 0xffffu) << 16)); } }
 #else
 #define VH_COMPACT_PHASE(I)
 #define VH_COMPACT_PHASES_OUT
 #endif
-    if (threadIdx.x == 0) { sh.n = 0u; sh.nBuckets = 0u; }
-    __syncthreads();
-    uint32_t bits = (wordIdx < nWords) ? hd.d_bucketBits[wordIdx] : 0u;
-    {
-        const uint32_t mine = (uint32_t)__popc(bits);
-        uint32_t incl = mine;
-#pragma unroll
-        for (uint32_t d = 1; d < kWave; d <<= 1) {
-            const uint32_t t = (uint32_t)__shfl_up((int)incl, d);
-            if (lane >= d) incl += t;
-        }
-        const uint32_t total = (uint32_t)__shfl((int)incl, kWave - 1);
-        uint32_t at = 0;
-        if (lane == 0 && total != 0u) at = atomicAdd(&sh.nBuckets, total);
-        at = (uint32_t)__shfl((int)at, 0) + incl - mine;
-        while (bits != 0u) {
-            sh.buckets[at++] = (uint16_t)(threadIdx.x * 32u + (uint32_t)(__ffs((int)bits) - 1));
-            bits &= bits - 1u;
-        }
-    }
+    if (threadIdx.x == 0) sh.n = 0u;
+    const uint32_t run = group + nGroups * (threadIdx.x >> 2);
+    uint32_t base = 0u;
+    uint32_t id = run * 4u + (threadIdx.x & 3u);
+    int4 e = id < nIds ? table[id] : make_int4(0, 0, 0, VH_FREE_ENTRY);
+    const uint32_t end = __builtin_amdgcn_readfirstlane(__hip_atomic_load(block_table_end(hd, hp), __ATOMIC_RELAXED, __HIP_MEMORY_SCOPE_AGENT));
     __syncthreads();
     VH_COMPACT_PHASE(1)
-    const uint32_t nSlots = sh.nBuckets * VH_HASH_BUCKET_SIZE;
-    const uint64_t firstBucket = (uint64_t)(wordIdx - threadIdx.x) * 32u;
-    constexpr uint32_t kInFlight = 4;
-    for (uint32_t s0 = threadIdx.x; s0 < nSlots; s0 += 256u * kInFlight) {
-        int4 qs[kInFlight];
-        uint32_t offs[kInFlight];
-#pragma unroll
-        for (uint32_t j = 0; j < kInFlight; j++) {
-            const uint32_t slot = s0 + 256u * j;
-            qs[j] = make_int4(0, 0, 0, VH_FREE_ENTRY);
-            offs[j] = 0;
-            if (slot < nSlots) {
-                const VhHashEntry* e = &hd.d_hash[(firstBucket + sh.buckets[slot / VH_HASH_BUCKET_SIZE]) * VH_HASH_BUCKET_SIZE + slot % VH_HASH_BUCKET_SIZE];
-                qs[j] = load_quad(e);
-                offs[j] = e->offset;
-            }
-        }
-#pragma unroll
-        for (uint32_t j = 0; j < kInFlight; j++) {
-            const int4 q = qs[j];
-            const bool keep = q.w != VH_FREE_ENTRY && block_in_frustum(hp, cp, mki3(q.x, q.y, q.z));
-            const uint64_t kept = __ballot(keep);
-            if (kept == 0ull) continue;
+    while (true) {
+        const bool keep = e.w != VH_FREE_ENTRY && block_in_frustum(hp, cp, mki3(e.x, e.y, e.z));
+        const uint64_t kept = __ballot(keep);
+        if (kept != 0ull) {
             uint32_t at = 0;
             if (lane == 0) at = atomicAdd(&sh.n, (uint32_t)__popcll(kept));
             at = (uint32_t)__shfl((int)at, 0) + (uint32_t)__popcll(kept & lanemask_lt());
             if (keep) {
+                const int4 q = make_int4(e.x, e.y, e.z, (int)(id * VH_SDF_BLOCK_VOXELS));
                 if (at < kCompactQueue) {
                     sh.q[at] = q;
-                    sh.off[at] = offs[j];
+                    sh.off[at] = (uint32_t)e.w;
                 } else {
+                    const uint32_t off = (uint32_t)e.w < ne ? hd.d_hash[e.w].offset : 0u;
                     VhHashEntry* o = &hd.d_hashCompactified[(uint32_t)atomicAdd(hd.d_hashCompactifiedCounter, 1)];
-                    list_store<COHERENT>(o, q, pack_box(offs[j], block_box(hp, cp, q.x, q.y, q.z), tag));
+                    list_store<COHERENT>(o, q, pack_box(off, block_box(hp, cp, q.x, q.y, q.z), tag));
                 }
             }
         }
+        base += nGroups * 256u;
+        if (base >= end) break;
+        id = base + run * 4u + (threadIdx.x & 3u);
+        e = id < nIds ? table[id] : make_int4(0, 0, 0, VH_FREE_ENTRY);
     }
     __syncthreads();
     VH_COMPACT_PHASE(2)
@@ -379,36 +382,50 @@
         __syncthreads();
         VH_COMPACT_PHASE(3)
         const uint32_t base = sh.base;
-        for (uint32_t i = threadIdx.x; i < n; i += blockDim.x) list_store<true>(&hd.d_hashCompactified[base + i], sh.q[i], make_uint4(sh.off[i], 0u, 0u, tag));
+        for (uint32_t i = threadIdx.x; i < n; i += blockDim.x) list_store<true>(&hd.d_hashCompactified[base + i], sh.q[i], make_uint4(0u, 0u, 0u, tag));
         VH_COMPACT_PHASE(4)
         VH_COMPACT_PHASES_OUT
         return;
     }
+    constexpr uint32_t kOffRounds = kCompactQueue / 256u;
+    uint32_t offs[kOffRounds];
+#pragma unroll
+    for (uint32_t r = 0; r < kOffRounds; r++) {
+        const uint32_t i = r * 256u + threadIdx.x;
+        offs[r] = 0u;
+        if (i < n) {
+            const uint32_t slot = sh.off[i];
+            if (slot < ne) offs[r] = hd.d_hash[slot].offset;
+        }
+    }
     constexpr uint32_t kBoxRounds = 2;
-    uint4 boxes[kBoxRounds];
+    BlockBox boxes[kBoxRounds];
     const uint32_t mine = threadIdx.x >> 3;
 #pragma unroll
     for (uint32_t r = 0; r < kBoxRounds; r++) {
         const uint32_t i = min(r * 32u + mine, n - 1u);
         if (r * 32u < n) {
             const int4 q = sh.q[i];
-            boxes[r] = pack_box(sh.off[i], block_box_by_eight_lanes(hp, cp, q.x, q.y, q.z), tag);
-        }
-    }
+            boxes[r] = block_box_by_eight_lanes(hp, cp, q.x, q.y, q.z);
+        }
+    }
+#pragma unroll
+    for (uint32_t r = 0; r < kOffRounds; r++)
+        if (r * 256u + threadIdx.x < n) sh.off[r * 256u + threadIdx.x] = offs[r];
     if (threadIdx.x == 0) sh.base = place;
     __syncthreads();
     VH_COMPACT_PHASE(3)
-    const uint32_t base = sh.base;
+    const uint32_t base0 = sh.base;
 #pragma unroll
     for (uint32_t r = 0; r < kBoxRounds; r++) {
         const uint32_t i = r * 32u + mine;
-        if (i < n && (threadIdx.x & 7u) == 0u) list_store<COHERENT>(&hd.d_hashCompactified[base + i], sh.q[i], boxes[r]);
+        if (i < n && (threadIdx.x & 7u) == 0u) list_store<COHERENT>(&hd.d_hashCompactified[base0 + i], sh.q[i], pack_box(sh.off[i], boxes[r], tag));
     }
     for (uint32_t r = kBoxRounds; r * 32u < n; r++) {
         const uint32_t i = r * 32u + mine;
         const int4 q = sh.q[min(i, n - 1u)];
         const BlockBox b = block_box_by_eight_lanes(hp, cp, q.x, q.y, q.z);
-        if (i < n && (threadIdx.x & 7u) == 0u) list_store<COHERENT>(&hd.d_hashCompactified[base + i], q, pack_box(sh.off[i], b, tag));
+        if (i < n && (threadIdx.x & 7u) == 0u) list_store<COHERENT>(&hd.d_hashCompactified[base0 + i], q, pack_box(sh.off[i], b, tag));
     }
     VH_COMPACT_PHASE(4)
     VH_COMPACT_PHASES_OUT
@@ -417,7 +434,7 @@
 __global__ __launch_bounds__(256) void k_compactify(VhHashData hd, VhHashParams hp, VhDepthCameraParams cp)
 {
     __shared__ CompactShared sh;
-    compactify_group(hd, hp, cp, blockIdx.x * blockDim.x + threadIdx.x, sh);
+    compactify_group(hd, hp, cp, blockIdx.x, gridDim.x, sh);
 }
 
 
@@ -1023,8 +1040,8 @@
 }
 
 
-constexpr uint32_t kSplatWordsPerGroup = 32;
-constexpr uint32_t kSplatQueue = 128;
+constexpr uint32_t kSplatLanes = 4;
+__host__ __device__ inline uint32_t splat_groups(uint32_t numBuckets) { return (uint32_t)(((uint64_t)numBuckets + 32u * 32u - 1u) / (32u * 32u)); }
 
 VHD void divmod_small(uint32_t i, uint32_t nx, float rnx, uint32_t& q, uint32_t& r)
 {
@@ -1151,53 +1168,35 @@
 }
 
 struct SplatShared {
-    uint32_t sBuckets[kSplatWordsPerGroup * 32];
-    int4 sBlocks[kSplatQueue];
-    uint32_t sNumBuckets, sNumBlocks;
+    uint32_t sSched[1024];
 };
 
 __device__ void interval_splat_group(const VhHashData& hd, const VhHashParams& hp, const VhDepthCameraParams& cp, const VhRayCastParams& rp,
                                      uint4* heads, int4* lists, uint32_t cap, uint32_t* sched, uint32_t phase, uint32_t numCUs,
                                      uint32_t nSplatGroups, uint32_t* feedback, uint32_t group, SplatShared& sh)
 {
-    uint32_t (&sBuckets)[kSplatWordsPerGroup * 32] = sh.sBuckets;
-    int4 (&sBlocks)[kSplatQueue] = sh.sBlocks;
-    uint32_t& sNumBuckets = sh.sNumBuckets;
-    uint32_t& sNumBlocks = sh.sNumBlocks;
-    const uint32_t nWords = (hp.m_hashNumBuckets + 31) / 32;
     const uint32_t lane = lane_id(), wave = threadIdx.x / kWave;
     const int tilesX = (int)((rp.m_width + 7) / 8), tilesY = (int)((rp.m_height + 7) / 8);
     const float vs = hp.m_virtualVoxelSize;
     const float growLo = (rp.m_useGradients ? 1.75f : 1.25f) * vs, growHi = (rp.m_useGradients ? 0.75f : 0.25f) * vs;
 
     if (group >= nSplatGroups) {
-        schedule_tiles(sched, feedback, (uint32_t)(tilesX * tilesY), phase, numCUs, group - nSplatGroups, sched_groups((uint32_t)(tilesX * tilesY)), sBuckets);
+        schedule_tiles(sched, feedback, (uint32_t)(tilesX * tilesY), phase, numCUs, group - nSplatGroups, sched_groups((uint32_t)(tilesX * tilesY)), sh.sSched);
         return;
     }
-    if (threadIdx.x == 0) { sNumBuckets = 0u; sNumBlocks = 0u; }
-    __syncthreads();
-    if (threadIdx.x < kSplatWordsPerGroup) {
-        const uint32_t wordIdx = group * kSplatWordsPerGroup + threadIdx.x;
-        uint32_t bits = wordIdx < nWords ? hd.d_bucketBits[wordIdx] : 0u;
-        while (bits) {
-            const uint32_t bucket = wordIdx * 32u + (uint32_t)(__ffs((int)bits) - 1);
-            bits &= bits - 1u;
-            sBuckets[atomicAdd(&sNumBuckets, 1u)] = bucket;
-        }
-    }
-    __syncthreads();
-    const uint32_t nBuckets = sNumBuckets;
-    for (uint32_t b0 = 0; b0 < nBuckets; b0 += 12u) {
-        const uint32_t bi = b0 + threadIdx.x / 16u, sl = threadIdx.x % 16u;
-        if (threadIdx.x < 12u * 16u && bi < nBuckets && sl < VH_HASH_BUCKET_SIZE) {
-            const int4 q = load_quad(&hd.d_hash[(uint64_t)sBuckets[bi] * VH_HASH_BUCKET_SIZE + sl]);
-            if (q.w != VH_FREE_ENTRY) sBlocks[atomicAdd(&sNumBlocks, 1u)] = q;
-        }
-        __syncthreads();
-        const uint32_t nBlocks = sNumBlocks;
-        for (uint32_t k = wave; k < nBlocks; k += 256 / kWave) {
-            const int4 q = sBlocks[k];
-            const int bx = q.x, by = q.y, bz = q.z, ptr = q.w;
+    const uint32_t nWaves = nSplatGroups * (256u / kWave), nIds = hp.m_numSDFBlocks;
+    const int4* const table = block_table(hd, hp);
+    uint32_t first = group * (256u / kWave) + wave;
+    uint32_t id = first + lane * nWaves;
+    int4 e = (lane < kSplatLanes && id < nIds) ? table[id] : make_int4(0, 0, 0, VH_FREE_ENTRY);
+    const uint32_t end = __builtin_amdgcn_readfirstlane(__hip_atomic_load(block_table_end(hd, hp), __ATOMIC_RELAXED, __HIP_MEMORY_SCOPE_AGENT));
+    while (true) {
+        uint64_t live = __ballot(e.w != VH_FREE_ENTRY);
+        while (live != 0ull) {
+            const int l = __ffsll((unsigned long long)live) - 1;
+            live &= live - 1ull;
+            const int bx = __builtin_amdgcn_readlane(e.x, l), by = __builtin_amdgcn_readlane(e.y, l), bz = __builtin_amdgcn_readlane(e.z, l);
+            const int ptr = (int)((first + (uint32_t)l * nWaves) * VH_SDF_BLOCK_VOXELS);
             const float lox = (float)(bx * VH_SDF_BLOCK_SIZE) * vs - growLo, hix = (float)(bx * VH_SDF_BLOCK_SIZE + VH_SDF_BLOCK_SIZE) * vs + growHi;
             const float loy = (float)(by * VH_SDF_BLOCK_SIZE) * vs - growLo, hiy = (float)(by * VH_SDF_BLOCK_SIZE + VH_SDF_BLOCK_SIZE) * vs + growHi;
             const float loz = (float)(bz * VH_SDF_BLOCK_SIZE) * vs - growLo, hiz = (float)(bz * VH_SDF_BLOCK_SIZE + VH_SDF_BLOCK_SIZE) * vs + growHi;
@@ -1250,9 +1249,10 @@
                 }
             }
         }
-        __syncthreads();
-        if (threadIdx.x == 0) sNumBlocks = 0u;
-        __syncthreads();
+        first += kSplatLanes * nWaves;
+        if (first >= end) break;
+        id = first + lane * nWaves;
+        e = (lane < kSplatLanes && id < nIds) ? table[id] : make_int4(0, 0, 0, VH_FREE_ENTRY);
     }
 }
 
@@ -2152,7 +2152,7 @@
 VHD void rider_done(const CoIntegrate& integ, const uint32_t i, const uint32_t n)
 {
     if (integ.groups == 0u) return;
-    __builtin_amdgcn_fence(__ATOMIC_RELEASE, "workgroup");
+    asm volatile("s_waitcnt vmcnt(0)" ::: "memory");
     __syncthreads();
     if (threadIdx.x < kWave) {
         uint32_t* const words = integ.done;
@@ -2260,8 +2260,8 @@
     const uint32_t nSched = splat.groups - splat.nSplatGroups;
     if (g >= nSched && g - nSched < job.groups) {
         g -= nSched;
-        if (integ.groups != 0u) compactify_group<true>(job.hd, job.hp, job.cp, g * blockDim.x + threadIdx.x, shared.compact, integ.riderTag);
-        else compactify_group<false>(job.hd, job.hp, job.cp, g * blockDim.x + threadIdx.x, shared.compact);
+        if (integ.groups != 0u) compactify_group<true>(job.hd, job.hp, job.cp, g, job.groups, shared.compact, integ.riderTag);
+        else compactify_group<false>(job.hd, job.hp, job.cp, g, job.groups, shared.compact);
         VH_GROUP_STAMP(3u)
         rider_done(integ, g, job.groups);
         return;
@@ -3334,6 +3334,7 @@
             append_heap(hd, (uint32_t)q.w / VH_SDF_BLOCK_VOXELS);
             delete_hash_entry(e);
             bucket_dec(hd, idx);
+            table_clear(hd, hp, q.w);
             emit = true;
         }
         if (emit) {
@@ -3380,6 +3381,7 @@
             append_heap(hd, (uint32_t)q.w / VH_SDF_BLOCK_VOXELS);
             delete_hash_entry(e);
             bucket_dec(hd, idx);
+            table_clear(hd, hp, q.w);
             emit = true;
         }
         if (emit) {
@@ -3458,10 +3460,14 @@
     if (i == 0u && bitMask && chunkBit != 0xffffffffu) atomicAnd(&bitMask[chunkBit >> 5], ~(1u << (chunkBit & 31u)));
     const uint32_t ptr = hd.d_heap[heapCountPrev - i] * VH_SDF_BLOCK_VOXELS;
     const VhSDFBlockDesc dsc = descs[i];
+    uint32_t end = 0u;
     if (!insert_hash_entry(hd, hp, mki3(dsc.pos[0], dsc.pos[1], dsc.pos[2]), (int)ptr, lockToken)) {
         atomicAdd(&hd.d_state[VH_STATE_INSERT_FAILED], 1u);
         failed[1u + atomicAdd(&failed[0], 1u)] = i;
-    }
+    } else {
+        end = ptr / VH_SDF_BLOCK_VOXELS + 1u;
+    }
+    table_raise(hd, hp, end);
 }
 __global__ __launch_bounds__(256) void k_stream_in_pass2_dev(VhHashData hd, uint32_t n, const VhVoxel* blocks)
 {
@@ -3492,10 +3498,14 @@
     if (i >= n) return;
     const uint32_t ptr = hd.d_heap[heapCountPrev - i] * VH_SDF_BLOCK_VOXELS;
     const VhSDFBlockDesc dsc = descs[i];
+    uint32_t end = 0u;
     if (!insert_hash_entry(hd, hp, mki3(dsc.pos[0], dsc.pos[1], dsc.pos[2]), (int)ptr, lockToken)) {
         atomicAdd(&hd.d_state[VH_STATE_INSERT_FAILED], 1u);
         if (failed) failed[1u + atomicAdd(&failed[0], 1u)] = i;
-    }
+    } else {
+        end = ptr / VH_SDF_BLOCK_VOXELS + 1u;
+    }
+    table_raise(hd, hp, end);
 }
 
 __global__ __launch_bounds__(256) void k_stream_in_pass2(VhHashData hd, uint32_t n, uint32_t heapCountPrev, const VhVoxel* blocks)
@@ -3562,14 +3572,19 @@
         const I3 p = mki3(ops[5 * i + 1], ops[5 * i + 2], ops[5 * i + 3]);
         const int32_t arg = ops[5 * i + 4];
         int32_t r = 0;
+        uint32_t end = 0u;
         switch (op) {
-        case VH_OP_ALLOC: r = alloc_block(hd, hp, p, token); break;
+        case VH_OP_ALLOC: r = alloc_block(hd, hp, p, token, end); break;
         case VH_OP_DELETE: r = delete_hash_entry_element(hd, hp, p, token) ? 1 : 0; break;
-        case VH_OP_INSERT: r = insert_hash_entry(hd, hp, p, arg, token) ? 1 : 0; break;
+        case VH_OP_INSERT:
+            r = insert_hash_entry(hd, hp, p, arg, token) ? 1 : 0;
+            if (r) end = (uint32_t)arg / VH_SDF_BLOCK_VOXELS + 1u;
+            break;
         case VH_OP_LOOKUP: r = lookup_ptr(hd, hp, p); break;
         case VH_OP_NEW_PASS: token++; break;
         default: break;
         }
+        table_raise(hd, hp, end);
         __builtin_amdgcn_fence(__ATOMIC_ACQ_REL, "agent");
         results[i] = r;
     }
@@ -3657,7 +3672,29 @@
     k_reset_heap<<<cdiv(nblk, 256), 256, 0, s>>>(hd->d_heap, hd->d_heapCounter, nblk);
     k_reset_hash<<<cdiv(2ull * ne, 256), 256, 0, s>>>(hd->d_hash, hd->d_hashCompactified, ne);
     k_fill_i32<<<cdiv(nb, 256), 256, 0, s>>>(hd->d_hashBucketMutex, VH_FREE_ENTRY, nb);
-    return vh_last_launch_error();
+    k_block_table_clear<<<cdiv(nblk, 256), 256, 0, s>>>(*hd, *hp);
+    return vh_last_launch_error();
+}
+
+int vh_block_table_rebuild(const VhHashData* hd, const VhHashParams* hp, vhStream_t stream)
+{
+    if (!hd || !hp || !hd->d_hash || !hd->d_bucketBits) return VH_ERR_BAD_ARGUMENT;
+    hipStream_t s = (hipStream_t)stream;
+    k_block_table_clear<<<cdiv(hp->m_numSDFBlocks, 256), 256, 0, s>>>(*hd, *hp);
+    k_block_table_from_hash<<<cdiv((uint64_t)hp->m_hashNumBuckets * VH_HASH_BUCKET_SIZE, 256), 256, 0, s>>>(*hd, *hp);
+    return vh_last_launch_error();
+}
+
+int vh_debug_block_table(const VhHashData* hd, const VhHashParams* hp, int32_t* h_table, uint32_t* h_end, vhStream_t stream)
+{
+    if (!hd || !hp || !hd->d_bucketBits) return VH_ERR_BAD_ARGUMENT;
+    hipStream_t s = (hipStream_t)stream;
+    const uint32_t* const words = hd->d_bucketBits;
+    if (h_end) VH_HIP(hipMemcpyAsync(h_end, words + VH_BLOCK_TABLE_END_WORD(hp->m_hashNumBuckets), sizeof(uint32_t), hipMemcpyDeviceToHost, s));
+    if (h_table)
+        VH_HIP(hipMemcpyAsync(h_table, words + VH_BLOCK_TABLE_WORD(hp->m_hashNumBuckets), 16u * (size_t)hp->m_numSDFBlocks, hipMemcpyDeviceToHost, s));
+    VH_HIP(hipStreamSynchronize(s));
+    return VH_OK;
 }
 
 int vh_reset_bucket_mutex(const VhHashData* hd, const VhHashParams* hp, vhStream_t stream)
@@ -3694,8 +3731,7 @@
 {
     if (!job || !job->hashData.d_hash) return VH_ERR_BAD_ARGUMENT;
     job->compactifyLaunched = 1;
-    const uint32_t nWords = (job->hashParams.m_hashNumBuckets + 31) / 32;
-    k_compactify<<<cdiv(nWords, 256), 256, 0, (hipStream_t)stream>>>(job->hashData, job->hashParams, job->cp);
+    k_compactify<<<compact_groups(job->hashParams.m_hashNumBuckets, job->hashParams.m_numSDFBlocks), 256, 0, (hipStream_t)stream>>>(job->hashData, job->hashParams, job->cp);
     return vh_last_launch_error();
 }
 
@@ -3705,8 +3741,7 @@
     if (!hd || !hp || !cp) return VH_ERR_BAD_ARGUMENT;
     hipStream_t s = (hipStream_t)stream;
     if (!(flags & VH_COMPACT_COUNTER_IS_ZERO)) VH_HIP(hipMemsetAsync(hd->d_hashCompactifiedCounter, 0, sizeof(int32_t), s));
-    const uint32_t nWords = (hp->m_hashNumBuckets + 31) / 32;
-    k_compactify<<<cdiv(nWords, 256), 256, 0, s>>>(*hd, *hp, *cp);
+    k_compactify<<<compact_groups(hp->m_hashNumBuckets, hp->m_numSDFBlocks), 256, 0, s>>>(*hd, *hp, *cp);
     int err = vh_last_launch_error();
     if (err) return err;
     if (numOccupied) {
@@ -3867,8 +3902,7 @@
     if (!hd || !hp || !cp || !rp || !d_tileHeads) return VH_ERR_BAD_ARGUMENT;
     if (rp->m_width == 0 || rp->m_height == 0) return VH_OK;
     const uint32_t numCUs = d_schedule ? device_num_cus() : 256u;
-    const uint32_t nWords = (hp->m_hashNumBuckets + 31) / 32;
-    const uint32_t groups = cdiv(nWords, kSplatWordsPerGroup);
+    const uint32_t groups = splat_groups(hp->m_hashNumBuckets);
     const uint32_t nSched = d_schedule ? sched_groups(cdiv(rp->m_width, 8) * cdiv(rp->m_height, 8)) : 0u;
     k_interval_splat<<<groups + nSched, 256, 0, (hipStream_t)stream>>>(*hd, *hp, *cp, *rp, reinterpret_cast<uint4*>(d_tileHeads),
                                                                                  reinterpret_cast<int4*>(d_tileBlocks), d_tileBlocks ? tileCapacity : 0u,
@@ -3889,7 +3923,7 @@
     std::memset(&sp, 0, sizeof(sp));
     if (fj && fj->allocLaunched && !fj->compactifyLaunched && fj->hashData.d_hash) {
         job.hd = fj->hashData; job.hp = fj->hashParams; job.cp = fj->cp;
-        job.groups = cdiv((fj->hashParams.m_hashNumBuckets + 31) / 32, 256);
+        job.groups = compact_groups(fj->hashParams.m_hashNumBuckets, fj->hashParams.m_numSDFBlocks);
         groups += job.groups;
         fj->compactifyLaunched = 1;
         if (nextView && d_tileHeads && nextView->m_width != 0 && nextView->m_height != 0) {
@@ -3900,7 +3934,7 @@
             sp.cap = d_tileBlocks ? tileCapacity : 0u;
             sp.phase = phase;
             sp.numCUs = d_schedule ? device_num_cus() : 256u;
-            sp.nSplatGroups = cdiv((fj->hashParams.m_hashNumBuckets + 31) / 32, kSplatWordsPerGroup);
+            sp.nSplatGroups = splat_groups(fj->hashParams.m_hashNumBuckets);
             sp.groups = sp.nSplatGroups + (d_schedule ? sched_groups(cdiv(nextView->m_width, 8) * cdiv(nextView->m_height, 8)) : 0u);
             groups += sp.groups;
         }
diff --git a/voxelhashing_amd/lib.py b/voxelhashing_amd/lib.py
--- a/voxelhashing_amd/lib.py
+++ b/voxelhashing_amd/lib.py
@@ -33,6 +33,8 @@
     "vh_hash_data_free": (C.c_int, [P(T.HashData)]),
     "vh_reset": (C.c_int, [P(T.HashData), P(T.HashParams), _VP]),
     "vh_reset_bucket_mutex": (C.c_int, [P(T.HashData), P(T.HashParams), _VP]),
+    "vh_block_table_rebuild": (C.c_int, [P(T.HashData), P(T.HashParams), _VP]),
+    "vh_debug_block_table": (C.c_int, [P(T.HashData), P(T.HashParams), _VP, _VP, _VP]),
     "vh_alloc": (C.c_int, [P(T.HashData), P(T.HashParams), P(T.DepthCameraData), P(T.DepthCameraParams), _VP, C.c_int32, _VP]),
     "vh_compactify": (C.c_int, [P(T.HashData), P(T.HashParams), P(T.DepthCameraParams), P(C.c_uint32), C.c_uint32, _VP]),
     "vh_integrate": (C.c_int, [P(T.HashData), P(T.HashParams), P(T.DepthCameraData), P(T.DepthCameraParams), _VP]),
```
